# PreibischLab/SPIM_Registration

Hardware: AMD Instinct MI355X
Metric: Mvoxels/sec per RL iter, 6-view 512³ deconv; 1/2/4/8-GPU scaling (higher is better)
Workload: dtype f32; 1 GPU; 6-view 512^3 per GPU (global 512x512x512), 25^3 PSF, RL INDEPENDENT lambda=0.0; views=6, local_slabs=1, parallelism=z-slab x1 over 1 GPU(s) (device groups in one process, xGMI peer halo pulls), launch=devices, num_devices=1, slabs=1

## Files before the change

### include/spimdecon.h

```cpp
#ifndef SPIMDECON_H
#define SPIMDECON_H

#include <stdint.h>

#ifdef __cplusplus
extern "C" {
#endif

#define SPIMDECON_OK               0
#define SPIMDECON_ERR_ARG         -1
#define SPIMDECON_ERR_DEVICE      -2
#define SPIMDECON_ERR_HIP         -3
#define SPIMDECON_ERR_FFT         -4
#define SPIMDECON_ERR_COMM        -5
#define SPIMDECON_ERR_STATE       -6
#define SPIMDECON_ERR_OOM         -7
#define SPIMDECON_ERR_IO          -8

const char* spimdecon_last_error(void);
const char* spimdecon_version(void);


int convolution3DfftCUDAInPlace(float* im, const int* imDim,
                                const float* kernel, const int* kernelDim,
                                int devCUDA);

float* convolution3DfftCUDA(const float* im, const int* imDim,
                            const float* kernel, const int* kernelDim,
                            int devCUDA);
void spimdecon_free(void* p);

int     getNumDevicesCUDA(void);
void    getNameDeviceCUDA(int devCUDA, char* name);
int64_t getMemDeviceCUDA(int devCUDA);
int64_t getFreeMemDeviceCUDA(int devCUDA);
int     getCUDAcomputeCapabilityMajorVersion(int devCUDA);
int     getCUDAcomputeCapabilityMinorVersion(int devCUDA);

int32_t convolve_7  (float* image, const float* kernelX, const float* kernelY, const float* kernelZ,
                     int imageW, int imageH, int imageD, int32_t convolveX, int32_t convolveY,
                     int32_t convolveZ, int outofbounds, float outofboundsvalue, int devCUDA);
int32_t convolve_15 (float* image, const float* kernelX, const float* kernelY, const float* kernelZ,
                     int imageW, int imageH, int imageD, int32_t convolveX, int32_t convolveY,
                     int32_t convolveZ, int outofbounds, float outofboundsvalue, int devCUDA);
int32_t convolve_31 (float* image, const float* kernelX, const float* kernelY, const float* kernelZ,
                     int imageW, int imageH, int imageD, int32_t convolveX, int32_t convolveY,
                     int32_t convolveZ, int outofbounds, float outofboundsvalue, int devCUDA);
int32_t convolve_63 (float* image, const float* kernelX, const float* kernelY, const float* kernelZ,
                     int imageW, int imageH, int imageD, int32_t convolveX, int32_t convolveY,
                     int32_t convolveZ, int outofbounds, float outofboundsvalue, int devCUDA);
int32_t convolve_127(float* image, const float* kernelX, const float* kernelY, const float* kernelZ,
                     int imageW, int imageH, int imageD, int32_t convolveX, int32_t convolveY,
                     int32_t convolveZ, int outofbounds, float outofboundsvalue, int devCUDA);

int     convolutionCPU(float* image, const float* kernelX, const float* kernelY, const float* kernelZ,
                       int kernelRX, int kernelRY, int kernelRZ, int imageW, int imageH, int imageD,
                       int outofbounds, float outofboundsvalue);

#define MVD_PSF_OPTIMIZATION_II     0
#define MVD_PSF_OPTIMIZATION_I      1
#define MVD_PSF_EFFICIENT_BAYESIAN  2
#define MVD_PSF_INDEPENDENT         3

int mvd_prepare_kernels(int nviews, const float* const* k1_in, const int* kdims,
                        int psftype, int ij_threads,
                        float* const* k1_out, float* const* k2_out, int devCUDA);

int spimdecon_next_value(const float* last, const float* integral, const float* weight, int64_t n,
                         double lambda, float* out);

typedef struct mvd_session mvd_session;

typedef struct mvd_params {
    int64_t dims[3];
    int64_t nz_global;
    int64_t z_offset;
    int     device;
    int     local_slabs;
    int     nranks;
    int     rank;
    const char* comm_id;
    int     storage_fp16;
    int     fft_pad_policy;
    int     halo[3];
    int     ij_threads;
    int     fft_backend;
    int     slab_axis;
    int     reserved[6];
} mvd_params;

void mvd_params_default(mvd_params* p);

int mvd_comm_unique_id(char* out128);

int mvd_slab_range(int64_t nz, int nparts, int idx, int64_t* z0, int64_t* z1);

int mvd_halo_plan(int64_t nz, int64_t Mz, int cz, int64_t plane_elems, int64_t* out5);

int  mvd_create(const mvd_params* params, mvd_session** out);
int  mvd_create_devices(const int* devs, int ndev, const mvd_params* params, mvd_session** out);
void mvd_destroy(mvd_session* h);
int  mvd_num_devices(mvd_session* h, int* ndev);
int  mvd_slab_device(mvd_session* h, int slab, int* dev);
int  mvd_num_slabs(mvd_session* h, int* nslabs);
int  mvd_slab_extent(mvd_session* h, int slab, int64_t* out3);
int  mvd_exchange_stats(mvd_session* h, int64_t* bytes, int64_t* copies);

int mvd_add_view(mvd_session* h, const float* img, const float* weight,
                 const float* kernel1, const int* kdims);
int mvd_add_view_device(mvd_session* h, const float* d_img, const float* d_weight,
                        const float* kernel1, const int* kdims);

int mvd_init(mvd_session* h, int psftype);
int mvd_set_kernels(mvd_session* h, int view, const float* k1, const float* k2);
int mvd_get_kernels(mvd_session* h, int view, float* k1, float* k2);

int mvd_init_psi(mvd_session* h, const float* psi_or_null, double* avg_out);

int mvd_run(mvd_session* h, int iters, double lambda, double* stats);

int mvd_apply_mask(mvd_session* h);

int mvd_get_psi(mvd_session* h, float* out);
float* mvd_psi_device(mvd_session* h, int slab);

int mvd_fft_dims(mvd_session* h, int slab, int64_t* out3);
int mvd_kernel_planes(mvd_session* h, int slab, int* planes);
int mvd_zpass_mode(mvd_session* h, int slab, int* mode);
int mvd_xpass_mode(mvd_session* h, int slab, int* mode);
void* mvd_stream(mvd_session* h);
int mvd_enable_timing(mvd_session* h, int on);
int mvd_timing(mvd_session* h, double* out16);

typedef struct spim_dog_params {
    float   sigma;
    float   threshold;
    int     localization;
    double  image_sigma[3];
    int32_t find_min;
    int32_t find_max;
    double  min_intensity;
    double  max_intensity;
    int     ij_threads;
    int     device;
} spim_dog_params;

typedef struct spim_peak {
    int32_t x, y, z;
    float   intensity;
    int32_t is_min, is_max;
} spim_peak;

typedef struct spim_interest_point {
    double  pos[3];
    float   intensity;
    int32_t is_max;
} spim_interest_point;

void spim_dog_params_default(spim_dog_params* p);

int spim_dog_compute(const float* img, const int64_t* dims, const spim_dog_params* p,
                     float* dog_out, spim_peak* peaks, int64_t max_peaks, int64_t* npeaks);

int spim_dog_interest_points(const float* img, const int64_t* dims, const spim_dog_params* p,
                             float* dog_out, spim_interest_point* out, int64_t max_out,
                             int64_t* nout);

#define SPIM_DOG_EXTEND_MIRROR 0
#define SPIM_DOG_EXTEND_BORDER 1
int spim_dog_compute_ext(const float* img, const int64_t* dims, const spim_dog_params* p, int32_t extension,
                         float* dog_out, spim_peak* peaks, int64_t max_peaks, int64_t* npeaks);
int spim_dog_interest_points_ext(const float* img, const int64_t* dims, const spim_dog_params* p, int32_t extension,
                                 float* dog_out, spim_interest_point* out, int64_t max_out, int64_t* nout);

int spim_dog_release_workspace(int device);

int spim_save_interest_points(const char* base_dir, const char* file, const spim_interest_point* pts,
                              const int32_t* ids, int64_t n);
int spim_load_interest_points(const char* base_dir, const char* file, spim_interest_point* out,
                              int32_t* ids, int64_t max_out, int64_t* nout);
int spim_set_java_version(int jdk);
int spim_java_double_to_string(double d, char* out, int cap);

typedef struct spim_dom_params {
    int     radius1;
    int     radius2;
    float   threshold;
    int     localization;
    double  image_sigma[3];
    int32_t find_min;
    int32_t find_max;
    double  min_intensity;
    double  max_intensity;
    int     ij_threads;
    int     device;
} spim_dom_params;

void spim_dom_params_default(spim_dom_params* p);

int spim_dom_diameters(const spim_dom_params* p, int32_t s1[3], int32_t s2[3]);

int spim_dom_compute(const float* img, const int64_t* dims, const spim_dom_params* p,
                     float* dom_out, spim_peak* peaks, int64_t max_peaks, int64_t* npeaks);
int spim_dom_interest_points(const float* img, const int64_t* dims, const spim_dom_params* p,
                             float* dom_out, spim_interest_point* out, int64_t max_out,
                             int64_t* nout);

typedef struct spim_rgldm_params {
    int32_t num_neighbors;
    int32_t redundancy;
    float   ratio_of_distance;
    float   difference_threshold;
    int32_t b_split;
    int32_t device;
} spim_rgldm_params;

void spim_rgldm_params_default(spim_rgldm_params* p);

void spim_rgldm_tiles(int32_t* a_tile, int32_t* b_tile);

int spim_rgldm_descriptors(const double* pts, int64_t n, const spim_rgldm_params* p,
                           int32_t* neighbors, double* rel);

int spim_rgldm_match(const double* a, int64_t na, const double* b, int64_t nb,
                     const spim_rgldm_params* p, int32_t* best_idx, double* best, double* second,
                     int32_t* cand_a, int32_t* cand_b, int64_t cap, int64_t* count);

typedef struct spim_gh_params {
    double  ratio_of_distance;
    double  difference_threshold;
    int32_t b_split;
    int32_t device;
} spim_gh_params;

void spim_gh_params_default(spim_gh_params* p);

void spim_gh_tiles(int32_t* a_tile, int32_t* b_tile);

int spim_gh_descriptors(const double* pts, int64_t n, const spim_gh_params* p,
                        int32_t* neighbors, float* desc);

int spim_gh_match(const double* a, int64_t na, const double* b, int64_t nb,
                  const spim_gh_params* p, int32_t* best_idx, double* best, double* second,
                  int32_t* cand_a, int32_t* cand_b, int64_t cap, int64_t* count);

typedef struct spim_icp_params {
    float   max_distance;
    int32_t max_iterations;
    int32_t t_split;
    int32_t device;
} spim_icp_params;

void spim_icp_params_default(spim_icp_params* p);

void spim_icp_tiles(int32_t* ref_block, int32_t* target_tile);

int spim_icp_assign(const double* target, int64_t nt, const double* reference, int64_t nr,
                    const double* model, const spim_icp_params* p, int32_t* nearest, float* dist,
                    int32_t* match_t, int32_t* match_r, int64_t cap, int64_t* count,
                    int64_t* ambiguous);

#define SPIM_WEIGHTS_NONE         0
#define SPIM_WEIGHTS_PRECOMPUTED  1
#define SPIM_WEIGHTS_VIRTUAL      2

typedef struct spim_view_source {
    const float* img;
    int64_t      dims[3];
    double       model[12];
} spim_view_source;

typedef struct spim_input_params {
    int64_t bb_min[3];
    int64_t bb_dims[3];
    float   blending_border[3];
    float   blending_range[3];
    int     weight_type;
    int     osem_index;
    double  osem_speedup;
    int     ij_threads;
    int     device;
    int     src_on_device;
    int     out_on_device;
    int     reserved[8];
} spim_input_params;

void spim_input_params_default(spim_input_params* p);

int spim_prepare_inputs(int nviews, const spim_view_source* views, const spim_input_params* p,
                        float* const* img_out, float* const* weight_out, double* osem_used,
                        int* min_overlap, double* avg_overlap);

typedef struct spim_fusion_params {
    int64_t bb_min[3];
    int64_t bb_dims[3];
    float   downsampling;
    int     interpolation;
    int     use_blending;
    int     device;
    int     src_on_device;
    int     out_on_device;
    int     reserved[8];
} spim_fusion_params;

void spim_fusion_params_default(spim_fusion_params* p);

int spim_fuse_weighted_average(int nviews, const spim_view_source* views, const spim_fusion_params* p,
                               const float* blending_borders, const float* blending_ranges, float* out);

int spim_content_based_weights(const float* img, const int64_t dims[3], const double sigma1[3],
                               const double sigma2[3], float* out, int device);

int spim_fuse_weighted_average_content(int nviews, const spim_view_source* views,
                                       const spim_fusion_params* p, const float* blending_borders,
                                       const float* blending_ranges, const double* sigma1,
                                       const double* sigma2, float* out);


int spim_psf_transformed_size(const int64_t psf_size[3], const double model[12], int64_t out_size[3],
                              double offset[3]);

int spim_transform_psf(const float* psf, const int64_t psf_size[3], const double model[12], float* out,
                       int device);

int spim_extract_psf(const float* img, const int64_t dims[3], int img_on_device, const double* locations,
                     int64_t nlocations, const int64_t psf_size[3], const double model[12], float* psf_original,
                     float* psf_transformed, int device);

int spim_extract_psfs(int nviews, const float* const* imgs, const int64_t* dims, int img_on_device,
                      const double* const* locations, const int64_t* nlocations, const int64_t psf_size[3],
                      const double* models, float* const* psf_original, float* const* psf_transformed,
                      int device);

int spim_psf_release_workspace(int device);

int spim_average_transformed_psf(int npsfs, const float* const* psfs, const int64_t* psf_dims, float* avg,
                                 int64_t avg_dims[3], int device);

int spim_max_projection(const float* img, const int64_t dims[3], int min_dim, float* out, int64_t out_dims[2],
                        int* used_dim, int device);

typedef struct lrsim_session lrsim_session;

int  lrsim_create(const int64_t* dims, int device, int nranks, int rank, const char* comm_id,
                  lrsim_session** out);
int  lrsim_create_devices(const int64_t* dims, const int* devs, int ndev, lrsim_session** out);
void lrsim_destroy(lrsim_session* h);
int  lrsim_add_view(lrsim_session* h, const float* img, const float* weight, const float* kernel,
                    const int* kdims);
int  lrsim_owns_view(lrsim_session* h, int view, int* owned);
int  lrsim_view_device(lrsim_session* h, int view, int* device);
int  lrsim_init(lrsim_session* h, double* avg_out);
int  lrsim_run(lrsim_session* h, int iters, int multiplicative, double lambda, double* stats);
int  lrsim_get_psi(lrsim_session* h, float* out);
int  lrsim_fft_dims(lrsim_session* h, int64_t* out3);
int  lrsim_update_rule(const float* psi_in, const double* value, const double* num, int64_t n,
                       int multiplicative, double lambda, float* psi_out, double* stats2);

#ifdef __cplusplus
}
#endif
#endif
```

### spim_registration_amd/_lib.py

```python
from __future__ import annotations

import ctypes as C
import os
from pathlib import Path

import numpy as np

LIB_PATH = Path(os.environ.get("SPIMDECON_LIB") or Path(__file__).resolve().parent / "libspimdecon.so")

_i32, _i64, _f32, _f64 = C.c_int32, C.c_int64, C.c_float, C.c_double
_pf = C.POINTER(C.c_float)
_pi = C.POINTER(C.c_int)
_pi64 = C.POINTER(C.c_int64)
_pd = C.POINTER(C.c_double)


class MvdParams(C.Structure):
    _fields_ = [
        ("dims", C.c_int64 * 3),
        ("nz_global", C.c_int64),
        ("z_offset", C.c_int64),
        ("device", C.c_int),
        ("local_slabs", C.c_int),
        ("nranks", C.c_int),
        ("rank", C.c_int),
        ("comm_id", C.c_char_p),
        ("storage_fp16", C.c_int),
        ("fft_pad_policy", C.c_int),
        ("halo", C.c_int * 3),
        ("ij_threads", C.c_int),
        ("fft_backend", C.c_int),
        ("slab_axis", C.c_int),
        ("reserved", C.c_int * 6),
    ]


class DogParams(C.Structure):
    _fields_ = [
        ("sigma", C.c_float),
        ("threshold", C.c_float),
        ("localization", C.c_int),
        ("image_sigma", C.c_double * 3),
        ("find_min", C.c_int32),
        ("find_max", C.c_int32),
        ("min_intensity", C.c_double),
        ("max_intensity", C.c_double),
        ("ij_threads", C.c_int),
        ("device", C.c_int),
    ]


class DomParams(C.Structure):
    _fields_ = [
        ("radius1", C.c_int),
        ("radius2", C.c_int),
        ("threshold", C.c_float),
        ("localization", C.c_int),
        ("image_sigma", C.c_double * 3),
        ("find_min", C.c_int32),
        ("find_max", C.c_int32),
        ("min_intensity", C.c_double),
        ("max_intensity", C.c_double),
        ("ij_threads", C.c_int),
        ("device", C.c_int),
    ]


class RgldmParams(C.Structure):
    _fields_ = [
        ("num_neighbors", C.c_int32),
        ("redundancy", C.c_int32),
        ("ratio_of_distance", C.c_float),
        ("difference_threshold", C.c_float),
        ("b_split", C.c_int32),
        ("device", C.c_int32),
    ]


class GhParams(C.Structure):
    _fields_ = [
        ("ratio_of_distance", C.c_double),
        ("difference_threshold", C.c_double),
        ("b_split", C.c_int32),
        ("device", C.c_int32),
    ]


class IcpParams(C.Structure):
    _fields_ = [
        ("max_distance", C.c_float),
        ("max_iterations", C.c_int32),
        ("t_split", C.c_int32),
        ("device", C.c_int32),
    ]


class Peak(C.Structure):
    _fields_ = [("x", C.c_int32), ("y", C.c_int32), ("z", C.c_int32),
                ("intensity", C.c_float), ("is_min", C.c_int32), ("is_max", C.c_int32)]


class ViewSource(C.Structure):
    _fields_ = [("img", C.POINTER(C.c_float)), ("dims", C.c_int64 * 3), ("model", C.c_double * 12)]


class InputParams(C.Structure):
    _fields_ = [("bb_min", C.c_int64 * 3), ("bb_dims", C.c_int64 * 3),
                ("blending_border", C.c_float * 3), ("blending_range", C.c_float * 3),
                ("weight_type", C.c_int), ("osem_index", C.c_int), ("osem_speedup", C.c_double),
                ("ij_threads", C.c_int), ("device", C.c_int), ("src_on_device", C.c_int),
                ("out_on_device", C.c_int), ("reserved", C.c_int * 8)]


class FusionParams(C.Structure):
    _fields_ = [("bb_min", C.c_int64 * 3), ("bb_dims", C.c_int64 * 3), ("downsampling", C.c_float),
                ("interpolation", C.c_int), ("use_blending", C.c_int), ("device", C.c_int),
                ("src_on_device", C.c_int), ("out_on_device", C.c_int), ("reserved", C.c_int * 8)]


class InterestPointC(C.Structure):
    _fields_ = [("pos", C.c_double * 3), ("intensity", C.c_float), ("is_max", C.c_int32)]


SIGNATURES = {
    "spimdecon_last_error": (C.c_char_p, []),
    "spimdecon_version": (C.c_char_p, []),
    "convolution3DfftCUDAInPlace": (C.c_int, [_pf, _pi, _pf, _pi, C.c_int]),
    "convolution3DfftCUDA": (_pf, [_pf, _pi, _pf, _pi, C.c_int]),
    "spimdecon_free": (None, [C.c_void_p]),
    "getNumDevicesCUDA": (C.c_int, []),
    "getNameDeviceCUDA": (None, [C.c_int, C.c_char_p]),
    "getMemDeviceCUDA": (_i64, [C.c_int]),
    "getFreeMemDeviceCUDA": (_i64, [C.c_int]),
    "getCUDAcomputeCapabilityMajorVersion": (C.c_int, [C.c_int]),
    "getCUDAcomputeCapabilityMinorVersion": (C.c_int, [C.c_int]),
    "spimdecon_next_value": (C.c_int, [C.c_void_p, C.c_void_p, C.c_void_p, C.c_int64, C.c_double, C.c_void_p]),
    "mvd_prepare_kernels": (C.c_int, [C.c_int, C.POINTER(_pf), _pi, C.c_int, C.c_int,
                                      C.POINTER(_pf), C.POINTER(_pf), C.c_int]),
    "mvd_params_default": (None, [C.POINTER(MvdParams)]),
    "mvd_comm_unique_id": (C.c_int, [C.c_char_p]),
    "mvd_slab_range": (C.c_int, [_i64, C.c_int, C.c_int, _pi64, _pi64]),
    "mvd_halo_plan": (C.c_int, [_i64, _i64, C.c_int, _i64, _pi64]),
    "mvd_create": (C.c_int, [C.POINTER(MvdParams), C.POINTER(C.c_void_p)]),
    "mvd_create_devices": (C.c_int, [_pi, C.c_int, C.POINTER(MvdParams), C.POINTER(C.c_void_p)]),
    "mvd_destroy": (None, [C.c_void_p]),
    "mvd_num_devices": (C.c_int, [C.c_void_p, C.POINTER(C.c_int)]),
    "mvd_slab_device": (C.c_int, [C.c_void_p, C.c_int, C.POINTER(C.c_int)]),
    "mvd_num_slabs": (C.c_int, [C.c_void_p, C.POINTER(C.c_int)]),
    "mvd_slab_extent": (C.c_int, [C.c_void_p, C.c_int, _pi64]),
    "mvd_exchange_stats": (C.c_int, [C.c_void_p, _pi64, _pi64]),
    "mvd_add_view": (C.c_int, [C.c_void_p, _pf, _pf, _pf, _pi]),
    "mvd_add_view_device": (C.c_int, [C.c_void_p, C.c_void_p, C.c_void_p, _pf, _pi]),
    "mvd_init": (C.c_int, [C.c_void_p, C.c_int]),
    "mvd_set_kernels": (C.c_int, [C.c_void_p, C.c_int, _pf, _pf]),
    "mvd_get_kernels": (C.c_int, [C.c_void_p, C.c_int, _pf, _pf]),
    "mvd_init_psi": (C.c_int, [C.c_void_p, _pf, _pd]),
    "mvd_run": (C.c_int, [C.c_void_p, C.c_int, C.c_double, _pd]),
    "mvd_apply_mask": (C.c_int, [C.c_void_p]),
    "mvd_get_psi": (C.c_int, [C.c_void_p, _pf]),
    "mvd_psi_device": (C.c_void_p, [C.c_void_p, C.c_int]),
    "mvd_fft_dims": (C.c_int, [C.c_void_p, C.c_int, _pi64]),
    "mvd_kernel_planes": (C.c_int, [C.c_void_p, C.c_int, C.POINTER(C.c_int)]),
    "mvd_zpass_mode": (C.c_int, [C.c_void_p, C.c_int, C.POINTER(C.c_int)]),
    "mvd_xpass_mode": (C.c_int, [C.c_void_p, C.c_int, C.POINTER(C.c_int)]),
    "mvd_stream": (C.c_void_p, [C.c_void_p]),
    "mvd_enable_timing": (C.c_int, [C.c_void_p, C.c_int]),
    "mvd_timing": (C.c_int, [C.c_void_p, _pd]),
    "convolve_7": (_i32, [_pf, _pf, _pf, _pf, C.c_int, C.c_int, C.c_int, _i32, _i32, _i32,
                          C.c_int, C.c_float, C.c_int]),
    "spim_dog_params_default": (None, [C.POINTER(DogParams)]),
    "spim_dog_compute": (C.c_int, [_pf, _pi64, C.POINTER(DogParams), _pf, C.POINTER(Peak),
                                   _i64, _pi64]),
    "spim_dog_interest_points": (C.c_int, [_pf, _pi64, C.POINTER(DogParams), _pf,
                                           C.POINTER(InterestPointC), _i64, _pi64]),
    "spim_dog_compute_ext": (C.c_int, [_pf, _pi64, C.POINTER(DogParams), _i32, _pf, C.POINTER(Peak),
                                       _i64, _pi64]),
    "spim_dog_interest_points_ext": (C.c_int, [_pf, _pi64, C.POINTER(DogParams), _i32, _pf,
                                               C.POINTER(InterestPointC), _i64, _pi64]),
    "spim_dog_release_workspace": (C.c_int, [C.c_int]),
    "spim_dom_params_default": (None, [C.POINTER(DomParams)]),
    "spim_dom_diameters": (C.c_int, [C.POINTER(DomParams), C.POINTER(_i32), C.POINTER(_i32)]),
    "spim_dom_compute": (C.c_int, [_pf, _pi64, C.POINTER(DomParams), _pf, C.POINTER(Peak), _i64, _pi64]),
    "spim_dom_interest_points": (C.c_int, [_pf, _pi64, C.POINTER(DomParams), _pf,
                                           C.POINTER(InterestPointC), _i64, _pi64]),
    "spim_rgldm_params_default": (None, [C.POINTER(RgldmParams)]),
    "spim_rgldm_tiles": (None, [C.POINTER(_i32), C.POINTER(_i32)]),
    "spim_rgldm_descriptors": (C.c_int, [C.c_void_p, _i64, C.POINTER(RgldmParams), C.c_void_p, C.c_void_p]),
    "spim_rgldm_match": (C.c_int, [C.c_void_p, _i64, C.c_void_p, _i64, C.POINTER(RgldmParams), C.c_void_p,
                                   C.c_void_p, C.c_void_p, C.c_void_p, C.c_void_p, _i64, _pi64]),
    "spim_gh_params_default": (None, [C.POINTER(GhParams)]),
    "spim_gh_tiles": (None, [C.POINTER(_i32), C.POINTER(_i32)]),
    "spim_gh_descriptors": (C.c_int, [C.c_void_p, _i64, C.POINTER(GhParams), C.c_void_p, C.c_void_p]),
    "spim_gh_match": (C.c_int, [C.c_void_p, _i64, C.c_void_p, _i64, C.POINTER(GhParams), C.c_void_p,
                                C.c_void_p, C.c_void_p, C.c_void_p, C.c_void_p, _i64, _pi64]),
    "spim_icp_params_default": (None, [C.POINTER(IcpParams)]),
    "spim_icp_tiles": (None, [C.POINTER(_i32), C.POINTER(_i32)]),
    "spim_icp_assign": (C.c_int, [C.c_void_p, _i64, C.c_void_p, _i64, C.c_void_p, C.POINTER(IcpParams), C.c_void_p,
                                  C.c_void_p, C.c_void_p, C.c_void_p, _i64, _pi64, _pi64]),
    "spim_psf_release_workspace": (C.c_int, [C.c_int]),
    "spim_save_interest_points": (C.c_int, [C.c_char_p, C.c_char_p, C.POINTER(InterestPointC),
                                            C.POINTER(C.c_int32), C.c_int64]),
    "spim_load_interest_points": (C.c_int, [C.c_char_p, C.c_char_p, C.POINTER(InterestPointC),
                                            C.POINTER(C.c_int32), C.c_int64, _pi64]),
    "spim_java_double_to_string": (C.c_int, [C.c_double, C.c_char_p, C.c_int]),
    "spim_set_java_version": (C.c_int, [C.c_int]),
    "convolutionCPU": (C.c_int, [_pf, _pf, _pf, _pf, C.c_int, C.c_int, C.c_int, C.c_int, C.c_int, C.c_int,
                                 C.c_int, C.c_float]),
    "spim_input_params_default": (None, [C.POINTER(InputParams)]),
    "spim_fusion_params_default": (None, [C.POINTER(FusionParams)]),
    "spim_psf_transformed_size": (C.c_int, [_pi64, _pd, _pi64, _pd]),
    "spim_transform_psf": (C.c_int, [_pf, _pi64, _pd, _pf, C.c_int]),
    "spim_extract_psf": (C.c_int, [C.c_void_p, _pi64, C.c_int, _pd, C.c_int64, _pi64, _pd, _pf, _pf, C.c_int]),
    "spim_extract_psfs": (C.c_int, [C.c_int, C.POINTER(C.c_void_p), _pi64, C.c_int, C.POINTER(C.c_void_p), _pi64,
                                    _pi64, _pd, C.POINTER(C.c_void_p), C.POINTER(C.c_void_p), C.c_int]),
    "spim_average_transformed_psf": (C.c_int, [C.c_int, C.POINTER(_pf), _pi64, _pf, _pi64, C.c_int]),
    "spim_max_projection": (C.c_int, [_pf, _pi64, C.c_int, _pf, _pi64, C.POINTER(C.c_int), C.c_int]),
    "spim_fuse_weighted_average": (C.c_int, [C.c_int, C.POINTER(ViewSource), C.POINTER(FusionParams),
                                             _pf, _pf, _pf]),
    "spim_content_based_weights": (C.c_int, [C.c_void_p, _pi64, _pd, _pd, C.c_void_p, C.c_int]),
    "spim_fuse_weighted_average_content": (C.c_int, [C.c_int, C.POINTER(ViewSource), C.POINTER(FusionParams),
                                                     _pf, _pf, _pd, _pd, _pf]),
    "lrsim_create": (C.c_int, [_pi64, C.c_int, C.c_int, C.c_int, C.c_char_p, C.POINTER(C.c_void_p)]),
    "lrsim_create_devices": (C.c_int, [_pi64, _pi, C.c_int, C.POINTER(C.c_void_p)]),
    "lrsim_destroy": (None, [C.c_void_p]),
    "lrsim_view_device": (C.c_int, [C.c_void_p, C.c_int, C.POINTER(C.c_int)]),
    "lrsim_add_view": (C.c_int, [C.c_void_p, C.c_void_p, C.c_void_p, C.c_void_p, _pi]),
    "lrsim_owns_view": (C.c_int, [C.c_void_p, C.c_int, C.POINTER(C.c_int)]),
    "lrsim_init": (C.c_int, [C.c_void_p, _pd]),
    "lrsim_run": (C.c_int, [C.c_void_p, C.c_int, C.c_int, C.c_double, _pd]),
    "lrsim_get_psi": (C.c_int, [C.c_void_p, C.c_void_p]),
    "lrsim_fft_dims": (C.c_int, [C.c_void_p, _pi64]),
    "lrsim_update_rule": (C.c_int, [C.c_void_p, C.c_void_p, C.c_void_p, C.c_int64, C.c_int, C.c_double,
                                    C.c_void_p, _pd]),
    "spim_prepare_inputs": (C.c_int, [C.c_int, C.POINTER(ViewSource), C.POINTER(InputParams),
                                      C.POINTER(_pf), C.POINTER(_pf), C.POINTER(C.c_double),
                                      C.POINTER(C.c_int), C.POINTER(C.c_double)]),
}
for _n in (15, 31, 63, 127):
    SIGNATURES[f"convolve_{_n}"] = SIGNATURES["convolve_7"]

_lib = None


class SpimDeconError(RuntimeError):
    def __init__(self, status, msg):
        super().__init__(f"libspimdecon status {status}: {msg}")
        self.status = status


def load():
    global _lib
    if _lib is not None:
        return _lib
    if not LIB_PATH.exists():
        raise RuntimeError(
            f"{LIB_PATH} not found: build it with `python -m spim_registration_amd.build` "
            "(there is no CPU fallback)")
    if os.environ.get("SPIMDECON_HIP_RUNTIME", "") != "system":
        try:
            import torch
        except ImportError:
            pass
    lib = C.CDLL(str(LIB_PATH), mode=C.RTLD_GLOBAL)
    for name, (res, args) in SIGNATURES.items():
        f = getattr(lib, name)
        f.restype = res
        f.argtypes = args
    _lib = lib
    return lib


def last_error() -> str:
    return load().spimdecon_last_error().decode(errors="replace")


ERR_IO = -8


def check(status: int):
    if status != 0:
        raise SpimDeconError(status, last_error())


def fptr(a: np.ndarray):
    assert a.dtype == np.float32 and a.flags.c_contiguous, (a.dtype, a.flags)
    return a.ctypes.data_as(_pf)


def iptr(a: np.ndarray):
    assert a.dtype == np.int32 and a.flags.c_contiguous
    return a.ctypes.data_as(_pi)


def num_devices() -> int:
    return int(load().getNumDevicesCUDA())
```

### spim_registration_amd/csrc/capi.cpp

```cpp
#include <rccl/rccl.h>
#include <rocfft/rocfft-version.h>

#include <cstdlib>
#include <cstring>
#include <string>

#include "common.hpp"
#include "kernel_prep.hpp"
#include "session.hpp"

namespace spimdecon {

thread_local std::string g_last_error;
void set_last_error(const std::string& msg) { g_last_error = msg; }
void clear_last_error() { g_last_error.clear(); }

void fft_convolve_block(float* im, const int* imDim, const float* kernel, const int* kernelDim,
                        int dev, float* out);
void slab_range(int64_t nz, int nparts, int idx, int64_t* z0, int64_t* z1);

}

using namespace spimdecon;

struct mvd_session {
    Session* s;
};

extern "C" {

const char* spimdecon_last_error(void) { return g_last_error.c_str(); }

const char* spimdecon_version(void) {
    static std::string v = std::string("spimdecon 0.1.0 gfx950 rocfft ") +
                           std::to_string(rocfft_version_major) + "." +
                           std::to_string(rocfft_version_minor) + "." +
                           std::to_string(rocfft_version_patch);
    return v.c_str();
}

int convolution3DfftCUDAInPlace(float* im, const int* imDim, const float* kernel,
                                const int* kernelDim, int devCUDA) {
    return guarded([&] { fft_convolve_block(im, imDim, kernel, kernelDim, devCUDA, im); });
}

float* convolution3DfftCUDA(const float* im, const int* imDim, const float* kernel,
                            const int* kernelDim, int devCUDA) {
    float* out = nullptr;
    int st = guarded([&] {
        SD_CHECK(imDim, SPIMDECON_ERR_ARG, "null imDim");
        const size_t n = size_t(imDim[0]) * imDim[1] * imDim[2];
        out = static_cast<float*>(std::malloc(n * sizeof(float)));
        SD_CHECK(out, SPIMDECON_ERR_OOM, "host out of memory");
        fft_convolve_block(const_cast<float*>(im), imDim, kernel, kernelDim, devCUDA, out);
    });
    if (st != SPIMDECON_OK) {
        std::free(out);
        return nullptr;
    }
    return out;
}

void spimdecon_free(void* p) { std::free(p); }

int getNumDevicesCUDA(void) {
    int n = 0;
    if (hipGetDeviceCount(&n) != hipSuccess) {
        return 0;
    }
    return n;
}

void getNameDeviceCUDA(int devCUDA, char* name) {
    if (!name) return;
    name[0] = 0;
    guarded([&] {
        check_device(devCUDA);
        hipDeviceProp_t prop;
        SD_HIP(hipGetDeviceProperties(&prop, devCUDA));
        std::string s = std::string(prop.name) + " (" + prop.gcnArchName + ")";
        std::strncpy(name, s.c_str(), 255);
        name[255] = 0;
    });
}

int64_t getMemDeviceCUDA(int devCUDA) {
    int64_t r = -1;
    guarded([&] {
        check_device(devCUDA);
        hipDeviceProp_t prop;
        SD_HIP(hipGetDeviceProperties(&prop, devCUDA));
        r = int64_t(prop.totalGlobalMem);
    });
    return r;
}

int64_t getFreeMemDeviceCUDA(int devCUDA) {
    int64_t r = -1;
    guarded([&] {
        check_device(devCUDA);
        DeviceGuard g(devCUDA);
        size_t fr = 0, tot = 0;
        SD_HIP(hipMemGetInfo(&fr, &tot));
        r = int64_t(fr);
    });
    return r;
}

int getCUDAcomputeCapabilityMajorVersion(int devCUDA) {
    int r = -1;
    guarded([&] {
        check_device(devCUDA);
        hipDeviceProp_t prop;
        SD_HIP(hipGetDeviceProperties(&prop, devCUDA));
        r = prop.major;
    });
    return r;
}

int getCUDAcomputeCapabilityMinorVersion(int devCUDA) {
    int r = -1;
    guarded([&] {
        check_device(devCUDA);
        hipDeviceProp_t prop;
        SD_HIP(hipGetDeviceProperties(&prop, devCUDA));
        r = prop.minor;
    });
    return r;
}

int spimdecon_next_value(const float* last, const float* integral, const float* weight, int64_t n, double lambda,
                         float* out) {
    return guarded([&] {
        SD_CHECK(n >= 0, SPIMDECON_ERR_ARG, "n must be >= 0");
        SD_CHECK(n == 0 || (last && integral && weight && out), SPIMDECON_ERR_ARG, "null pointer");
        launch_next_value(last, integral, weight, n, lambda, out, nullptr);
        SD_HIP(hipStreamSynchronize(nullptr));
    });
}

int mvd_prepare_kernels(int nviews, const float* const* k1_in, const int* kdims, int psftype,
                        int ij_threads, float* const* k1_out, float* const* k2_out, int devCUDA) {
    return guarded([&] {
        SD_CHECK(nviews >= 1 && k1_in && kdims && k1_out && k2_out, SPIMDECON_ERR_ARG, "bad arguments");
        std::vector<HostKernel> k1(nviews), k2;
        for (int v = 0; v < nviews; ++v) {
            for (int d = 0; d < 3; ++d) k1[v].dims[d] = kdims[3 * v + d];
            const int64_t n = int64_t(k1[v].dims[0]) * k1[v].dims[1] * k1[v].dims[2];
            SD_CHECK(n > 0 && k1_in[v], SPIMDECON_ERR_ARG, "bad kernel");
            k1[v].data.assign(k1_in[v], k1_in[v] + n);
        }
        prepare_kernels_gpu(k1, k2, psftype, ij_threads, devCUDA);
        for (int v = 0; v < nviews; ++v) {
            std::copy(k1[v].data.begin(), k1[v].data.end(), k1_out[v]);
            std::copy(k2[v].data.begin(), k2[v].data.end(), k2_out[v]);
        }
    });
}

void mvd_params_default(mvd_params* p) {
    if (!p) return;
    std::memset(p, 0, sizeof(*p));
    p->local_slabs = 1;
    p->nranks = 1;
    p->ij_threads = 8;
}

int mvd_comm_unique_id(char* out128) {
    return guarded([&] {
        SD_CHECK(out128, SPIMDECON_ERR_ARG, "null output");
        static_assert(sizeof(ncclUniqueId) == 128, "unexpected ncclUniqueId size");
        ncclUniqueId id;
        ncclResult_t r = ncclGetUniqueId(&id);
        SD_CHECK(r == ncclSuccess, SPIMDECON_ERR_COMM,
                 std::string("ncclGetUniqueId failed: ") + ncclGetErrorString(r));
        std::memcpy(out128, &id, 128);
    });
}

int mvd_slab_range(int64_t nz, int nparts, int idx, int64_t* z0, int64_t* z1) {
    return guarded([&] {
        SD_CHECK(nz >= 1 && nparts >= 1 && idx >= 0 && idx < nparts && z0 && z1, SPIMDECON_ERR_ARG,
                 "bad slab_range arguments");
        slab_range(nz, nparts, idx, z0, z1);
    });
}

int mvd_halo_plan(int64_t nz, int64_t Mz, int cz, int64_t plane_elems, int64_t* out5) {
    return guarded([&] {
        SD_CHECK(out5, SPIMDECON_ERR_ARG, "null argument");
        const HaloPlan h = halo_plan(nz, Mz, cz, plane_elems);
        out5[0] = h.send_lo;
        out5[1] = h.recv_lo;
        out5[2] = h.send_hi;
        out5[3] = h.recv_hi;
        out5[4] = h.count;
    });
}

int mvd_create(const mvd_params* params, mvd_session** out) {
    return guarded([&] {
        SD_CHECK(params && out, SPIMDECON_ERR_ARG, "null argument");
        *out = nullptr;
        auto* h = new mvd_session{nullptr};
        try {
            h->s = new Session(*params);
        } catch (...) {
            delete h;
            throw;
        }
        *out = h;
    });
}

int mvd_create_devices(const int* devs, int ndev, const mvd_params* params, mvd_session** out) {
    return guarded([&] {
        SD_CHECK(devs && ndev >= 1 && params && out, SPIMDECON_ERR_ARG, "null argument");
        *out = nullptr;
        std::vector<int> dl(devs, devs + ndev);
        auto* h = new mvd_session{nullptr};
        try {
            h->s = new Session(*params, dl);
        } catch (...) {
            delete h;
            throw;
        }
        *out = h;
    });
}

void mvd_destroy(mvd_session* h) {
    if (!h) return;
    guarded([&] { delete h->s; });
    delete h;
}

#define SESSION(h) \
    SD_CHECK((h) && (h)->s, SPIMDECON_ERR_ARG, "null session"); \
    Session& S = *(h)->s

int mvd_add_view(mvd_session* h, const float* img, const float* weight, const float* kernel1,
                 const int* kdims) {
    return guarded([&] { SESSION(h); S.add_view(img, weight, kernel1, kdims, false); });
}

int mvd_add_view_device(mvd_session* h, const float* d_img, const float* d_weight,
                        const float* kernel1, const int* kdims) {
    return guarded([&] { SESSION(h); S.add_view(d_img, d_weight, kernel1, kdims, true); });
}

int mvd_init(mvd_session* h, int psftype) {
    return guarded([&] { SESSION(h); S.init(psftype); });
}

int mvd_set_kernels(mvd_session* h, int view, const float* k1, const float* k2) {
    return guarded([&] { SESSION(h); S.set_kernels(view, k1, k2); });
}

int mvd_get_kernels(mvd_session* h, int view, float* k1, float* k2) {
    return guarded([&] { SESSION(h); S.get_kernels(view, k1, k2); });
}

int mvd_init_psi(mvd_session* h, const float* psi_or_null, double* avg_out) {
    return guarded([&] {
        SESSION(h);
        const double a = S.init_psi(psi_or_null);
        if (avg_out) *avg_out = a;
    });
}

int mvd_run(mvd_session* h, int iters, double lambda, double* stats) {
    return guarded([&] { SESSION(h); S.run(iters, lambda, stats); });
}

int mvd_apply_mask(mvd_session* h) {
    return guarded([&] { SESSION(h); S.apply_mask(); });
}

int mvd_get_psi(mvd_session* h, float* out) {
    return guarded([&] { SESSION(h); S.get_psi(out); });
}

float* mvd_psi_device(mvd_session* h, int slab) {
    float* r = nullptr;
    guarded([&] { SESSION(h); r = S.psi_device(slab); });
    return r;
}

int mvd_fft_dims(mvd_session* h, int slab, int64_t* out3) {
    return guarded([&] { SESSION(h); SD_CHECK(out3, SPIMDECON_ERR_ARG, "null"); S.fft_dims(slab, out3); });
}

int mvd_kernel_planes(mvd_session* h, int slab, int* planes) {
    return guarded([&] { SESSION(h); SD_CHECK(planes, SPIMDECON_ERR_ARG, "null"); *planes = S.kernel_planes(slab); });
}

int mvd_zpass_mode(mvd_session* h, int slab, int* mode) {
    return guarded([&] { SESSION(h); SD_CHECK(mode, SPIMDECON_ERR_ARG, "null"); *mode = S.zpass_mode(slab); });
}

int mvd_xpass_mode(mvd_session* h, int slab, int* mode) {
    return guarded([&] { SESSION(h); SD_CHECK(mode, SPIMDECON_ERR_ARG, "null"); *mode = S.xpass_mode(slab); });
}

void* mvd_stream(mvd_session* h) {
    void* r = nullptr;
    guarded([&] { SESSION(h); r = S.stream(); });
    return r;
}

int mvd_num_devices(mvd_session* h, int* ndev) {
    return guarded([&] { SESSION(h); SD_CHECK(ndev, SPIMDECON_ERR_ARG, "null"); *ndev = S.ndevices(); });
}

int mvd_slab_device(mvd_session* h, int slab, int* dev) {
    return guarded([&] { SESSION(h); SD_CHECK(dev, SPIMDECON_ERR_ARG, "null"); *dev = S.slab_device(slab); });
}

int mvd_num_slabs(mvd_session* h, int* nslabs) {
    return guarded([&] { SESSION(h); SD_CHECK(nslabs, SPIMDECON_ERR_ARG, "null"); *nslabs = S.nslabs(); });
}

int mvd_exchange_stats(mvd_session* h, int64_t* bytes, int64_t* copies) {
    return guarded([&] { SESSION(h); S.exchange_stats(bytes, copies); });
}

int mvd_slab_extent(mvd_session* h, int slab, int64_t* out3) {
    return guarded([&] { SESSION(h); SD_CHECK(out3, SPIMDECON_ERR_ARG, "null"); S.slab_extent(slab, out3); });
}

int mvd_enable_timing(mvd_session* h, int on) {
    return guarded([&] { SESSION(h); S.enable_timing(on != 0); });
}

int mvd_timing(mvd_session* h, double* out16) {
    return guarded([&] { SESSION(h); SD_CHECK(out16, SPIMDECON_ERR_ARG, "null"); S.timing(out16); });
}

}
```

### spim_registration_amd/csrc/fftconv.hip

```cpp
#include "fftconv.hpp"

#include <climits>
#include "rl_math.hpp"

#include <cmath>
#include <cstdlib>
#include <type_traits>
#include <cstdio>
#include <cstring>

namespace spimdecon {

namespace {


typedef float sd_v2 __attribute__((ext_vector_type(2)));
__device__ __forceinline__ sd_v2 v2_(float2 a) { return sd_v2{a.x, a.y}; }
__device__ __forceinline__ float2 f2_(sd_v2 a) { return make_float2(a.x, a.y); }
__device__ __forceinline__ float2 cmul(float2 a, float2 b) {
    const sd_v2 A = v2_(a), B = v2_(b);
    const sd_v2 t = A.xx * B;
    return f2_(__builtin_elementwise_fma(A.yy, sd_v2{-B.y, B.x}, t));
}
__device__ __forceinline__ float2 cadd(float2 a, float2 b) {
#pragma clang fp contract(fast)
    return f2_(v2_(a) + v2_(b));
}
__device__ __forceinline__ float2 csub(float2 a, float2 b) {
#pragma clang fp contract(fast)
    return f2_(v2_(a) - v2_(b));
}
__device__ __forceinline__ float2 cscale(float2 a, float s) {
#pragma clang fp contract(fast)
    return f2_(v2_(a) * sd_v2{s, s});
}
template <bool INV>
__device__ __forceinline__ float2 mul_mi(float2 a) {
    return INV ? make_float2(-a.y, a.x) : make_float2(a.y, -a.x);
}
template <bool INV>
__device__ __forceinline__ float2 cadd_mi(float2 a, float2 d) {
    const sd_v2 D = v2_(d);
    return f2_(__builtin_elementwise_fma(D.yx, INV ? sd_v2{-1.0f, 1.0f} : sd_v2{1.0f, -1.0f}, v2_(a)));
}
template <bool INV>
__device__ __forceinline__ float2 csub_mi(float2 a, float2 d) {
    const sd_v2 D = v2_(d);
    return f2_(__builtin_elementwise_fma(D.yx, INV ? sd_v2{1.0f, -1.0f} : sd_v2{-1.0f, 1.0f}, v2_(a)));
}

template <int S>
__device__ __forceinline__ float ldv(const void* p, int64_t i) {
    if constexpr (S == 0) return static_cast<const float*>(p)[i];
    else return __half2float(static_cast<const __half*>(p)[i]);
}


template <int R, bool INV>
__device__ __forceinline__ void dft(float2* a) {
    if constexpr (R == 2) {
        const float2 t = a[0];
        a[0] = cadd(t, a[1]);
        a[1] = csub(t, a[1]);
    } else if constexpr (R == 3) {
        const float2 s = cadd(a[1], a[2]);
        const float2 m = csub(a[0], cscale(s, 0.5f));
        const float2 d = cscale(csub(a[1], a[2]), 0.86602540378443864676f);
        a[0] = cadd(a[0], s);
        a[1] = cadd_mi<INV>(m, d);
        a[2] = csub_mi<INV>(m, d);
    } else if constexpr (R == 4) {
        const float2 s0 = cadd(a[0], a[2]), d0 = csub(a[0], a[2]);
        const float2 s1 = cadd(a[1], a[3]), d1 = csub(a[1], a[3]);
        a[0] = cadd(s0, s1);
        a[2] = csub(s0, s1);
        a[1] = cadd_mi<INV>(d0, d1);
        a[3] = csub_mi<INV>(d0, d1);
    } else if constexpr (R == 5) {
        constexpr float c1 = 0.30901699437494742410f, c2 = -0.80901699437494742410f;
        constexpr float s1 = 0.95105651629515357212f, s2 = 0.58778525229247312917f;
        const float2 b1 = cadd(a[1], a[4]), b2 = cadd(a[2], a[3]);
        const float2 d1 = csub(a[1], a[4]), d2 = csub(a[2], a[3]);
        const float2 m1 = cadd(a[0], cadd(cscale(b1, c1), cscale(b2, c2)));
        const float2 m2 = cadd(a[0], cadd(cscale(b1, c2), cscale(b2, c1)));
        const float2 n1 = cadd(cscale(d1, s1), cscale(d2, s2));
        const float2 n2 = csub(cscale(d1, s2), cscale(d2, s1));
        a[0] = cadd(a[0], cadd(b1, b2));
        a[1] = cadd_mi<INV>(m1, n1);
        a[4] = csub_mi<INV>(m1, n1);
        a[2] = cadd_mi<INV>(m2, n2);
        a[3] = csub_mi<INV>(m2, n2);
    } else {
        static_assert(R == 7, "radix 2, 3, 4, 5, 7 only");
        constexpr float c1 = 0.62348980185873353053f, c2 = -0.22252093395631440429f,
                        c3 = -0.90096886790241912624f;
        constexpr float s1 = 0.78183148246802980871f, s2 = 0.97492791218182360702f,
                        s3 = 0.43388373911755812048f;
        const float2 b1 = cadd(a[1], a[6]), b2 = cadd(a[2], a[5]), b3 = cadd(a[3], a[4]);
        const float2 d1 = csub(a[1], a[6]), d2 = csub(a[2], a[5]), d3 = csub(a[3], a[4]);
        const float2 r1 = cadd(a[0], cadd(cscale(b1, c1), cadd(cscale(b2, c2), cscale(b3, c3))));
        const float2 r2 = cadd(a[0], cadd(cscale(b1, c2), cadd(cscale(b2, c3), cscale(b3, c1))));
        const float2 r3 = cadd(a[0], cadd(cscale(b1, c3), cadd(cscale(b2, c1), cscale(b3, c2))));
        const float2 i1 = cadd(cscale(d1, s1), cadd(cscale(d2, s2), cscale(d3, s3)));
        const float2 i2 = csub(cscale(d1, s2), cadd(cscale(d2, s3), cscale(d3, s1)));
        const float2 i3 = cadd(csub(cscale(d1, s3), cscale(d2, s1)), cscale(d3, s2));
        a[0] = cadd(a[0], cadd(b1, cadd(b2, b3)));
        a[1] = cadd_mi<INV>(r1, i1);
        a[6] = csub_mi<INV>(r1, i1);
        a[2] = cadd_mi<INV>(r2, i2);
        a[5] = csub_mi<INV>(r2, i2);
        a[3] = cadd_mi<INV>(r3, i3);
        a[4] = csub_mi<INV>(r3, i3);
    }
}

template <int R, bool INV>
__device__ __forceinline__ void stage_pp(const float2* __restrict__ src, float2* __restrict__ dst,
                                         const float2* __restrict__ tw, int L, int Ns, int c, int g,
                                         int TPC, int ES, int CS) {
    const int nb = L / R;
    const int step = L / (Ns * R);
    for (int j = g; j < nb; j += TPC) {
        const int k = j % Ns;
        float2 v[R];
#pragma unroll
        for (int t = 0; t < R; ++t) v[t] = src[(j + t * nb) * ES + c * CS];
        if (Ns > 1) {
#pragma unroll
            for (int t = 1; t < R; ++t) {
                float2 w = tw[t * k * step];
                if (INV) w.y = -w.y;
                v[t] = cmul(v[t], w);
            }
        }
        dft<R, INV>(v);
        const int base = (j - k) * R + k;
#pragma unroll
        for (int t = 0; t < R; ++t) dst[(base + t * Ns) * ES + c * CS] = v[t];
    }
}

__device__ __forceinline__ void wave_sync() {
    __builtin_amdgcn_fence(__ATOMIC_RELEASE, "wavefront");
    __builtin_amdgcn_wave_barrier();
    __builtin_amdgcn_fence(__ATOMIC_ACQUIRE, "wavefront");
}

template <bool INV, bool WAVE = false>
__device__ __forceinline__ float2* fft_pp(float2* a, float2* b, const float2* tw, const Fft1D& f, int c, int g,
                          int TPC, int ES, int CS, bool active) {
    int Ns = 1;
    float2* src = a;
    float2* dst = b;
    for (int s = 0; s < f.ns; ++s) {
        const int R = f.radix(s);
        if (active) {
            switch (R) {
                case 2: stage_pp<2, INV>(src, dst, tw, f.L, Ns, c, g, TPC, ES, CS); break;
                case 3: stage_pp<3, INV>(src, dst, tw, f.L, Ns, c, g, TPC, ES, CS); break;
                case 4: stage_pp<4, INV>(src, dst, tw, f.L, Ns, c, g, TPC, ES, CS); break;
                case 5: stage_pp<5, INV>(src, dst, tw, f.L, Ns, c, g, TPC, ES, CS); break;
                default: stage_pp<7, INV>(src, dst, tw, f.L, Ns, c, g, TPC, ES, CS); break;
            }
        }
        if constexpr (WAVE) wave_sync();
        else __syncthreads();
        Ns *= R;
        float2* t = src;
        src = dst;
        dst = t;
    }
    return src;
}


enum XMode { XM_PSI = 0, XM_QUOT = 1, XM_UPDATE = 2, XM_KERNEL = 3 };

struct XArgs {
    SlabGeom g;
    int64_t Hx, Hp;
    Fft1D fx;
    const int* row_mirror;
    const int* row_one;
    const float2* Cin;
    float2* Cout;
    const float* psi_in;
    float* psi_out;
    const void* img;
    const void* w;
    double lambda;
    double* partials;
    const float* kern;
    int kx, ky, kz;
    float kscale;
    uint32_t spec_bytes;
    uint32_t nvox;
    int pb0, pn0, pb1, pn1;
};

__device__ __forceinline__ int x_pair(const XArgs& a, int i) {
    return i < a.pn0 ? a.pb0 + i : (i - a.pn0 < a.pn1 ? a.pb1 + (i - a.pn0) : -1);
}

constexpr int kXThreads = 256;
constexpr int kXPairs = kXThreads / 64;

__host__ __device__ inline int x_wave_elems(int Mx) { return 2 * (Mx + 2); }

template <int MODE, int S>
__global__ __launch_bounds__(kXThreads) void k_xpass(XArgs a) {
    extern __shared__ __attribute__((aligned(16))) float2 smem[];
    const SlabGeom& g = a.g;
    const int Mx = int(g.Mx);
    const int Hx = int(a.Hx);
    const int Hp = int(a.Hp);
    const int nx = int(g.nx);
    const int cx = g.cx;
    float2* tw = smem;
    const int wv = threadIdx.x >> 6;
    const int lane = threadIdx.x & 63;
    float2* A = smem + Mx + wv * x_wave_elems(Mx);
    float2* B = A + Mx + 2;
    for (int i = threadIdx.x; i < Mx; i += kXThreads) tw[i] = a.fx.tw[i];
    const int nrows = int(g.My * g.Mz);
    const int nlin = a.pn0 + a.pn1;
    double ssum = 0.0;
    float smax = -1.0f;
    __syncthreads();
    for (int pg = blockIdx.x; pg * kXPairs < nlin; pg += gridDim.x) {
        const int pair = x_pair(a, pg * kXPairs + wv);
        const bool active = pair >= 0;
        const int r0 = 2 * pair, r1 = 2 * pair + 1;
        const bool valid0 = active && r0 < nrows, valid1 = active && r1 < nrows;
        const int sm0 = valid0 ? a.row_mirror[r0] : -1, sm1 = valid1 ? a.row_mirror[r1] : -1;
        const int so0 = valid0 ? a.row_one[r0] : -1, so1 = valid1 ? a.row_one[r1] : -1;
        float2* Z = A;
        if constexpr (MODE == XM_QUOT || MODE == XM_UPDATE) {
            int p0 = -1, p1 = -1;
            if constexpr (MODE == XM_QUOT) {
                p0 = so0 >= 0 ? r0 : -1;
                p1 = so1 >= 0 ? r1 : -1;
            } else {
                p0 = sm0 >= 0 ? (sm0 / int(g.ny)) * int(g.My) + sm0 % int(g.ny) : -1;
                p1 = sm1 >= 0 ? (sm1 / int(g.ny)) * int(g.My) + sm1 % int(g.ny) : -1;
            }
            const float2* row0 = a.Cin + int64_t(p0) * Hp;
            const float2* row1 = a.Cin + int64_t(p1) * Hp;
            for (int k = lane; k < Hx; k += 64) {
                B[k] = p0 >= 0 ? row0[k] : make_float2(0.f, 0.f);
                B[Hx + k] = p1 >= 0 ? row1[k] : make_float2(0.f, 0.f);
            }
            __syncthreads();
            for (int k = lane; k < Mx; k += 64) {
                float2 xa, xb;
                if (k <= Mx / 2) {
                    xa = B[k];
                    xb = B[Hx + k];
                    if (k == 0 || k == Mx / 2) {
                        xa.y = 0.f;
                        xb.y = 0.f;
                    }
                } else {
                    xa = B[Mx - k];
                    xb = B[Hx + Mx - k];
                    xa.y = -xa.y;
                    xb.y = -xb.y;
                }
                A[k] = make_float2(xa.x - xb.y, xa.y + xb.x);
            }
            __syncthreads();
            Z = fft_pp<true>(A, B, tw, a.fx, 0, lane, 64, 1, 0, active);
        }
        float2* O = (Z == A) ? B : A;
        if constexpr (MODE == XM_PSI) {
            const float* p0 = a.psi_in + int64_t(sm0 < 0 ? 0 : sm0) * nx;
            const float* p1 = a.psi_in + int64_t(sm1 < 0 ? 0 : sm1) * nx;
            for (int qx = lane; qx < Mx; qx += 64) {
                const int sx = qx < nx + cx ? qx : qx - Mx;
                const int lx = int(mirror_idx(sx, nx));
                Z[qx] = make_float2(sm0 >= 0 ? p0[lx] : 0.f, sm1 >= 0 ? p1[lx] : 0.f);
            }
        } else if constexpr (MODE == XM_KERNEL) {
            for (int qx = lane; qx < Mx; qx += 64) {
                float v[2] = {0.f, 0.f};
#pragma unroll
                for (int h = 0; h < 2; ++h) {
                    const int r = h == 0 ? r0 : r1;
                    if (!(h == 0 ? valid0 : valid1)) continue;
                    const int qz = r / int(g.My), qy = r % int(g.My);
                    const int jz = (qz + a.kz / 2) % int(g.Mz), jy = (qy + a.ky / 2) % int(g.My);
                    const int jx = (qx + a.kx / 2) % Mx;
                    if (jz < a.kz && jy < a.ky && jx < a.kx)
                        v[h] = a.kern[(int64_t(jz) * a.ky + jy) * a.kx + jx] * a.kscale;
                }
                Z[qx] = make_float2(v[0], v[1]);
            }
        } else if constexpr (MODE == XM_QUOT) {
            const bool live0 = valid0 && sm0 != -1, live1 = valid1 && sm1 != -1;
            for (int qx = lane; qx < Mx; qx += 64) {
                const float2 bz = Z[qx];
                float q0 = live0 ? 1.0f : 0.0f, q1 = live1 ? 1.0f : 0.0f;
                if (qx < nx) {
                    if (so0 >= 0) {
                        const float iv = ldv<S>(a.img, int64_t(so0) * nx + qx);
                        if (iv > 0.0f) q0 = __fdiv_rn(iv, bz.x);
                    }
                    if (so1 >= 0) {
                        const float iv = ldv<S>(a.img, int64_t(so1) * nx + qx);
                        if (iv > 0.0f) q1 = __fdiv_rn(iv, bz.y);
                    }
                }
                Z[qx] = make_float2(q0, q1);
            }
        } else {
            for (int qx = lane; qx < nx; qx += 64) {
                const float2 iz = Z[qx];
                float o0 = 0.f, o1 = 0.f;
                if (sm0 >= 0) {
                    const int64_t vi = int64_t(sm0) * nx + qx;
                    const float last = a.psi_in[vi];
                    o0 = next_value(last, iz.x, ldv<S>(a.w, vi), a.lambda);
                    if (so0 >= 0) {
                        a.psi_out[vi] = o0;
                        const float ch = fabsf(__fsub_rn(o0, last));
                        ssum += (double)ch;
                        smax = fmaxf(smax, ch);
                    }
                }
                if (sm1 >= 0) {
                    const int64_t vi = int64_t(sm1) * nx + qx;
                    const float last = a.psi_in[vi];
                    o1 = next_value(last, iz.y, ldv<S>(a.w, vi), a.lambda);
                    if (so1 >= 0) {
                        a.psi_out[vi] = o1;
                        const float ch = fabsf(__fsub_rn(o1, last));
                        ssum += (double)ch;
                        smax = fmaxf(smax, ch);
                    }
                }
                Z[qx] = make_float2(o0, o1);
            }
            __syncthreads();
            for (int qx = nx + lane; qx < Mx; qx += 64) {
                const int sx = qx < nx + cx ? qx : qx - Mx;
                Z[qx] = Z[mirror_idx(sx, nx)];
            }
        }
        __syncthreads();
        if (MODE == XM_UPDATE && a.Cout == nullptr) continue;
        float2* F = fft_pp<false>(Z, O, tw, a.fx, 0, lane, 64, 1, 0, active);
        const bool w0 = valid0 && sm0 != -1, w1 = valid1 && sm1 != -1;
        float2* out0 = a.Cout + int64_t(r0) * Hp;
        float2* out1 = a.Cout + int64_t(r1) * Hp;
        for (int k = lane; k < Hp; k += 64) {
            float2 xa = make_float2(0.f, 0.f), xb = make_float2(0.f, 0.f);
            if (k < Hx) {
                const float2 zk = F[k];
                const float2 zm = F[k == 0 ? 0 : Mx - k];
                xa = make_float2(0.5f * (zk.x + zm.x), 0.5f * (zk.y - zm.y));
                xb = make_float2(0.5f * (zk.y + zm.y), -0.5f * (zk.x - zm.x));
            }
            if (w0) out0[k] = xa;
            if (w1) out1[k] = xb;
        }
        __syncthreads();
    }
    if constexpr (MODE == XM_UPDATE) {
        __shared__ double sh_sum[kXThreads / 64];
        __shared__ float sh_max[kXThreads / 64];
        for (int off = 32; off > 0; off >>= 1) {
            ssum += __shfl_xor(ssum, off, 64);
            smax = fmaxf(smax, __shfl_xor(smax, off, 64));
        }
        if (lane == 0) {
            sh_sum[wv] = ssum;
            sh_max[wv] = smax;
        }
        __syncthreads();
        if (threadIdx.x == 0) {
            for (int i = 1; i < kXThreads / 64; ++i) {
                ssum += sh_sum[i];
                smax = fmaxf(smax, sh_max[i]);
            }
            a.partials[2 * blockIdx.x] = ssum;
            a.partials[2 * blockIdx.x + 1] = (double)smax;
        }
    }
}


constexpr int kCThreads = 1024;

#include "fftconv_col.inc"
#include "fft_reg.inc"
#include "fftconv_2f.inc"
#include "fftconv_x.inc"
#include "fftconv_xt.inc"
#include "fftconv_zd.inc"


Fft1D make_fft(int L, bool allow_2f, DBuf<float2>& tw, hipStream_t s) {
    Fft1D f;
    f.L = L;
    int m = L;
    auto push = [&](int r) {
        SD_CHECK(f.ns < kFftMaxStages, SPIMDECON_ERR_ARG, "too many FFT stages");
        f.radix_packed |= uint64_t(r) << (4 * f.ns);
        f.ns++;
        m /= r;
    };
    while (m % 4 == 0) push(4);
    while (m % 2 == 0) push(2);
    while (m % 3 == 0) push(3);
    while (m % 5 == 0) push(5);
    while (m % 7 == 0) push(7);
    SD_CHECK(m == 1, SPIMDECON_ERR_ARG, "FFT length " + std::to_string(L) + " is not 2,3,5,7-smooth");
#define SD_2F_LOOKUP(A, B) \
    if (L == (A) * (B)) { f.n1 = (A); f.n2 = (B); }
    if (allow_2f) { SD_2F_SIZES(SD_2F_LOOKUP) }
#undef SD_2F_LOOKUP
    std::vector<float2> h(L);
    for (int i = 0; i < L; ++i) {
        const double ang = -2.0 * M_PI * double(i) / double(L);
        h[i] = make_float2(float(std::cos(ang)), float(std::sin(ang)));
    }
    tw.alloc(L);
    SD_HIP(hipMemcpyAsync(tw.p, h.data(), L * sizeof(float2), hipMemcpyHostToDevice, s));
    SD_HIP(hipStreamSynchronize(s));
    f.tw = tw.p;
    return f;
}

size_t x_lds(const SpectralPlan& p) {
    return size_t(p.g.Mx + kXPairs * x_wave_elems(int(p.g.Mx))) * sizeof(float2);
}

unsigned x_grid(const XArgs& a) {
    const int64_t b = ceil_div(int64_t(a.pn0) + a.pn1, kXPairs);
    return unsigned(std::max<int64_t>(1, std::min<int64_t>(b, 256 * 8)));
}

XArgs base_args(const SpectralPlan& p) {
    XArgs a{};
    SD_CHECK(p.g.My * p.g.Mz < (int64_t(1) << 30), SPIMDECON_ERR_ARG, "too many rows");
    a.pb0 = 0;
    a.pn0 = int((p.g.My * p.g.Mz + 1) / 2);
    a.pb1 = 0;
    a.pn1 = 0;
    a.g = p.g;
    a.Hx = p.Hx;
    a.Hp = p.Hp;
    a.fx = p.fx;
    a.row_mirror = p.row_mirror.p;
    a.row_one = p.row_one.p;
    return a;
}

#define SD_X2F_SIZES(M) M(16, 16) M(16, 24) M(16, 32) M(20, 27) M(24, 24) M(20, 32) M(25, 32) M(30, 35) M(42, 50)

bool aligned_to(const void* q, size_t n) { return q == nullptr || reinterpret_cast<uintptr_t>(q) % n == 0; }

bool x_buffer_args(const XArgs& a, Store st, const SpectralPlan& p, XArgs& b) {
    const size_t va = st == Store::F32 ? 16 : 8;
    const uint64_t spec_bytes = uint64_t(p.spectrum_elems()) * sizeof(float2);
    const uint64_t nvox = uint64_t(p.g.nx) * p.g.ny * p.g.nz;
    if (p.g.nx % 4 != 0 || !aligned_to(a.img, va) || !aligned_to(a.w, va) || !aligned_to(a.psi_in, 16) ||
        !aligned_to(a.psi_out, 16) || spec_bytes >= kOOB || nvox * 4 >= kOOB)
        return false;
    b = a;
    b.spec_bytes = uint32_t(spec_bytes);
    b.nvox = uint32_t(nvox);
    return true;
}

template <int MODE>
unsigned launch_xtile(const XArgs& a, Store st, const SpectralPlan& p, hipStream_t s) {
    XArgs b;
    if (!p.fx.n1 || !x_buffer_args(a, st, p, b)) return 0;
    const int L = int(p.g.Mx);
    const int NP = xt_np(MODE, L);
    const size_t lds = xt_lds(L, NP, xt_twg(L, NP));
    if (lds > 160 * 1024) return 0;
    const unsigned grid = unsigned(std::max<int64_t>(1, ceil_div(int64_t(a.pn0) + a.pn1, int64_t(NP))));
    const int sv = st == Store::F32 ? 0 : 1;
    bool done = false;
    const bool tik = MODE == XM_UPDATE && a.lambda > 0.0;
#define SD_XT(SV, A, B, TK)                                                                                \
    if (!done && sv == SV && L == (A) * (B) && tik == TK) {                                               \
        constexpr int TRv = SD_2F_TR(A, B);                                                               \
        constexpr int NPv = xt_np(MODE, (A) * (B));                                                       \
        auto kfn = &k_xtile<MODE, SV, A, B, TK, NPv, TRv>;                                                \
        SD_HIP(hipFuncSetAttribute(reinterpret_cast<const void*>(kfn), hipFuncAttributeMaxDynamicSharedMemorySize, \
                                   int(lds)));                                                            \
        hipLaunchKernelGGL(kfn, dim3(grid), dim3(NPv * TRv), lds, s, b);                                  \
        done = true;                                                                                      \
    }
#define SD_XT_S(A, B) \
    SD_XT(0, A, B, false) SD_XT(1, A, B, false) if constexpr (MODE == XM_UPDATE) { SD_XT(0, A, B, true) SD_XT(1, A, B, true) }
    SD_X2F_SIZES(SD_XT_S)
#undef SD_XT_S
#undef SD_XT
    if (!done) return 0;
    SD_HIP(hipGetLastError());
#if SD_XT_STAMPS
    {
        unsigned long long h[3][8];
        SD_HIP(hipStreamSynchronize(s));
        SD_HIP(hipMemcpyFromSymbol(h, HIP_SYMBOL(g_xt_stamp), sizeof(h)));
        const unsigned long long n = std::max(1ull, h[MODE][7]);
        std::fprintf(stderr, "[xt_stamp] L=%d mode=%d fp16=%d tiles=%llu cycles/tile: load %llu inv %llu rl %llu fwd %llu store %llu prologue %llu\n",
                     L, MODE, sv, h[MODE][7], h[MODE][0] / n, h[MODE][1] / n, h[MODE][2] / n, h[MODE][3] / n,
                     h[MODE][4] / n, h[MODE][5] / n);
        std::memset(h, 0, sizeof(h));
        SD_HIP(hipMemcpyToSymbol(HIP_SYMBOL(g_xt_stamp), h, sizeof(h)));
    }
#endif
    return grid;
}

template <int MODE>
unsigned launch_xrows(const XArgs& a, Store st, const SpectralPlan& p, hipStream_t s) {
    const int nx = int(p.g.nx);
    const int U = int(ceil_div(p.Hp / 2, 64));
    const int UV = int(ceil_div(nx / 4, 64));
    XArgs b;
    if (U > 4 || (UV != U && UV != U - 1) || !x_buffer_args(a, st, p, b)) return 0;
    const int Mx = int(p.g.Mx);
    const size_t lds = size_t(Mx + kXPairs * xrows_wave_elems(Mx, false)) * sizeof(float2);
    SD_CHECK(lds <= 160 * 1024, SPIMDECON_ERR_ARG, "x pass LDS too large");
    SD_CHECK(p.g.My * p.g.Mz < (int64_t(1) << 30), SPIMDECON_ERR_ARG, "too many rows");
    const unsigned grid = x_grid(a);
    const int sv = st == Store::F32 ? 0 : 1;
    bool done = false;
#define SD_XR(SV, UU, VV)                                                                               \
    if (!done && sv == SV && U == UU && UV == VV) {                                                     \
        SD_HIP(hipFuncSetAttribute(reinterpret_cast<const void*>(&k_xrows<MODE, SV, UU, VV, 0, 0>),    \
                                   hipFuncAttributeMaxDynamicSharedMemorySize, int(lds)));              \
        hipLaunchKernelGGL((k_xrows<MODE, SV, UU, VV, 0, 0>), dim3(grid), dim3(kXThreads), lds, s, b); \
        done = true;                                                                                    \
    }
#define SD_XR_S(SV) SD_XR(SV, 1, 1) SD_XR(SV, 2, 1) SD_XR(SV, 2, 2) SD_XR(SV, 3, 2) \
                    SD_XR(SV, 3, 3) SD_XR(SV, 4, 3) SD_XR(SV, 4, 4)
    SD_XR_S(0) SD_XR_S(1)
#undef SD_XR_S
#undef SD_XR
    SD_CHECK(done, SPIMDECON_ERR_ARG, "no x-row kernel for this configuration");
    SD_HIP(hipGetLastError());
    return grid;
}

template <int MODE>
unsigned launch_x(const XArgs& a, Store st, const SpectralPlan& p, hipStream_t s) {
    if constexpr (MODE == XM_QUOT || MODE == XM_UPDATE || MODE == XM_PSI) {
        if (const unsigned gt = launch_xtile<MODE>(a, st, p, s)) {
            if (MODE == XM_UPDATE) p.xmode_update = 2;
            return gt;
        }
    }
    if constexpr (MODE == XM_QUOT || MODE == XM_UPDATE) {
        if (const unsigned gr = launch_xrows<MODE>(a, st, p, s)) {
            if (MODE == XM_UPDATE) p.xmode_update = 1;
            return gr;
        }
    }
    if (MODE == XM_UPDATE) p.xmode_update = 0;
    const size_t lds = x_lds(p);
    SD_CHECK(lds <= 160 * 1024, SPIMDECON_ERR_ARG, "x pass LDS too large");
    SD_CHECK(p.g.My * p.g.Mz < (int64_t(1) << 30), SPIMDECON_ERR_ARG, "too many rows");
    const unsigned grid = x_grid(a);
    if (st == Store::F32) {
        SD_HIP(hipFuncSetAttribute(reinterpret_cast<const void*>(&k_xpass<MODE, 0>),
                                   hipFuncAttributeMaxDynamicSharedMemorySize, int(lds)));
        hipLaunchKernelGGL((k_xpass<MODE, 0>), dim3(grid), dim3(kXThreads), lds, s, a);
    } else {
        SD_HIP(hipFuncSetAttribute(reinterpret_cast<const void*>(&k_xpass<MODE, 1>),
                                   hipFuncAttributeMaxDynamicSharedMemorySize, int(lds)));
        hipLaunchKernelGGL((k_xpass<MODE, 1>), dim3(grid), dim3(kXThreads), lds, s, a);
    }
    SD_HIP(hipGetLastError());
    return grid;
}

int col_tx(int L) {
    for (int tx : {16, 8, 4})
        if (size_t(2 * L * tx + L) * sizeof(float2) <= 160 * 1024) return tx;
    fail(SPIMDECON_ERR_ARG, "column FFT length " + std::to_string(L) + " exceeds the LDS tile");
}

constexpr int kColGridRounds = 16;

template <int AXIS, int MODE>
bool launch_col2f(const SpectralPlan& p, const Fft1D& f, float2* C, const float2* K, hipStream_t s,
                  int tx0 = 0, int ntxb = -1, int kc = 0, int nout = -1, int zsplit = INT_MAX, int zskip = 0) {
    if (nout < 0) nout = int(p.g.Mz);
    const int L = f.L;
    const int tr = (f.n1 > 32 || f.n2 > 32) ? 64 : 32;
    const size_t budget = size_t(160) * 1024;
    auto tile_lds = [&](int tx) { return size_t(L * tx + L + (MODE == 5 ? f.n2 * tx : 0)) * sizeof(float2); };
    const int TX = tile_lds(k2fTX) <= budget ? k2fTX : 8;
    const int kplanes = MODE == 5 ? 2 * kc + 1 : 0;
    const size_t lds = tile_lds(TX);
    const uint64_t bytes = uint64_t(p.spectrum_elems()) * sizeof(float2);
    const uint64_t kbytes = MODE == 5 ? uint64_t(kplanes) * p.Hp * p.g.My * sizeof(float2)
                                      : (MODE >= 2 ? bytes : 0);
    if (MODE >= 2 && tr == 64) return false;
    if (lds > budget || (AXIS == 2 && bytes >= (uint64_t(1) << 31))) return false;
    if (MODE == 5 && (AXIS != 2 || kplanes > f.n2)) return false;
    const uint32_t rbytes = AXIS == 1 ? uint32_t(uint64_t(p.g.My * p.Hp) * sizeof(float2)) : uint32_t(bytes);
    if (ntxb < 0) ntxb = int(p.Hp / TX);
    SD_CHECK(tx0 >= 0 && ntxb > 0 && tx0 + ntxb <= p.Hp / TX, SPIMDECON_ERR_ARG, "bad column band");
    const int64_t ntiles = int64_t(ntxb) * (AXIS == 1 ? nout : p.g.My);
    const int64_t per_cu = std::max<int64_t>(1, (160 * 1024) / int64_t(lds));
    const unsigned grid = unsigned(std::min<int64_t>(ntiles, 256 * per_cu * kColGridRounds));
    const int n1 = f.n1, n2 = f.n2;
    const bool pf = p.knobs.ypf && AXIS == 1 && MODE < 2 && tr == 32 && TX == 16 && lds > size_t(80 * 1024);
    bool done = false;
#define SD_2F_L(A, B, T, PFV)                                                                                   \
            constexpr int TRv = SD_2F_TR(A, B);                                                                 \
            SD_HIP(hipFuncSetAttribute(reinterpret_cast<const void*>(&k_col2f<AXIS, A, B, MODE, T, TRv, PFV>), \
                                       hipFuncAttributeMaxDynamicSharedMemorySize, int(lds)));                  \
            hipLaunchKernelGGL((k_col2f<AXIS, A, B, MODE, T, TRv, PFV>), dim3(grid), dim3(T * TRv), lds, s,     \
                               p.g, p.Hp, f.tw, C, K, rbytes, tx0, ntxb, kc, uint32_t(kbytes), nout, zsplit,  \
                               zskip);                                                                       \
            done = true;
#define SD_2F_C1(A, B, T)                                                                                  \
    if constexpr (MODE < 2 || SD_2F_TR(A, B) == 32) {                                                      \
        if (!done && n1 == (A) && n2 == (B) && TX == (T)) {                                                \
            if constexpr (AXIS == 1 && MODE < 2 && (T) == 16 && SD_2F_TR(A, B) == 32 && (A) * (B) >= 512) { \
                if (pf) { SD_2F_L(A, B, T, true) }                                                         \
            }                                                                                              \
            if (!done) { SD_2F_L(A, B, T, false) }                                                         \
        }                                                                                                  \
    }
#define SD_2F_C(A, B) \
    SD_2F_C1(A, B, 16) if constexpr ((A) * (B) > 600) { SD_2F_C1(A, B, 8) }
    SD_2F_SIZES(SD_2F_C)
#undef SD_2F_C
#undef SD_2F_C1
#undef SD_2F_L
    SD_CHECK(done, SPIMDECON_ERR_ARG, "no two-factor column kernel for this length");
    SD_HIP(hipGetLastError());
    return true;
}

template <int AXIS, bool INV, int ZMODE>
void launch_col(const SpectralPlan& p, const Fft1D& f, float2* C, const float2* K, hipStream_t s,
                int nout = -1) {
    if constexpr (ZMODE == 1) {
        if (f.n1 && launch_col2f<AXIS, 4>(p, f, C, K, s, 0, -1, 0, nout)) return;
    }
    if (f.n1 && launch_col2f<AXIS, ZMODE == 1 ? 2 : (INV ? 1 : 0)>(p, f, C, K, s, 0, -1, 0, nout)) return;
    const int tx = col_tx(f.L);
    SD_CHECK(f.L * tx / 2 <= kColMaxU * kCThreads, SPIMDECON_ERR_ARG, "column tile exceeds prefetch registers");
    const size_t lds = size_t(2 * f.L * tx + f.L) * sizeof(float2);
    const int64_t ntiles = (p.Hp / tx) * (AXIS == 1 ? p.g.Mz : p.g.My);
    const unsigned grid = unsigned(std::min<int64_t>(ntiles, 256 * (tx == 16 ? 1 : 2)));
#define CL(TXV)                                                                                    \
    case TXV:                                                                                      \
        SD_HIP(hipFuncSetAttribute(reinterpret_cast<const void*>(&k_colpass<AXIS, TXV, INV, ZMODE>), \
                                   hipFuncAttributeMaxDynamicSharedMemorySize, int(lds)));         \
        hipLaunchKernelGGL((k_colpass<AXIS, TXV, INV, ZMODE>), dim3(grid), dim3(kCThreads), lds, s, \
                           p.g, p.Hp, f, C, K);                                                    \
        break;
    switch (tx) {
        CL(16) CL(8) CL(4)
        default: fail(SPIMDECON_ERR_ARG, "bad TX");
    }
#undef CL
    SD_HIP(hipGetLastError());
}

}

int64_t engine_fast_size(int64_t need, bool even, int policy) {
    need = std::max<int64_t>(need, 1);
    int64_t smooth = 0;
    for (int64_t m = need;; ++m) {
        if (even && (m & 1)) continue;
        int64_t r = m;
        for (int64_t q : {2, 3, 5, 7})
            while (r % q == 0) r /= q;
        if (r == 1) {
            smooth = m;
            break;
        }
    }
    int64_t fast = 0;
#define SD_2F_PICK(A, B) \
    if ((A) * (B) >= need && (fast == 0 || (A) * (B) < fast)) fast = (A) * (B);
    SD_2F_SIZES(SD_2F_PICK)
#undef SD_2F_PICK
    if (policy == 2 || fast == 0) {
        SD_CHECK(policy != 1, SPIMDECON_ERR_ARG, "length " + std::to_string(need) + " beyond the fast-path table");
        return smooth;
    }
    if (policy == 1) return fast;
    return fast * 4 <= smooth * 5 ? fast : smooth;
}

bool engine_slab_fits(int64_t nx, int64_t ny, int64_t nzs, const int halo[3], int policy) {
    const int64_t Mx = engine_fast_size(nx + 2 * halo[0], true, policy);
    const int64_t My = engine_fast_size(ny + 2 * halo[1], false, policy);
    const int64_t Mz = engine_fast_size(nzs + 2 * halo[2], false, policy);
    const int64_t Hp = ceil_div(Mx / 2 + 1, int64_t(16)) * 16;
    return uint64_t(nx) * uint64_t(ny) * uint64_t(nzs) * 4u < kOOB &&
           uint64_t(Hp) * uint64_t(My) * uint64_t(Mz) * sizeof(float2) < kOOB;
}

static bool zdirect_env() {
    const char* e = std::getenv("SPIMDECON_ZDIRECT");
    return !(e && e[0] == '0');
}

EngineKnobs EngineKnobs::from_env() {
    auto off = [](const char* name) {
        const char* e = std::getenv(name);
        return e && e[0] == '0';
    };
    EngineKnobs k;
    k.ypf = !off("SPIMDECON_YPF");
    k.zkd = !off("SPIMDECON_ZKD");
    k.zdirect = zdirect_env();
    return k;
}

void SpectralPlan::create(const SlabGeom& geom, bool allow_2f, bool z_fft, const EngineKnobs& kn) {
    g = geom;
    knobs = kn;
    SD_CHECK(g.Mx % 2 == 0, SPIMDECON_ERR_ARG, "Mx must be even");
    Hx = g.Mx / 2 + 1;
    Hp = ceil_div(Hx, 16) * 16;
    hipStream_t s = nullptr;
    fx = make_fft(int(g.Mx), allow_2f, twx, s);
    fy = make_fft(int(g.My), allow_2f, twy, s);
    if (z_fft) {
        fz = make_fft(int(g.Mz), allow_2f, twz, s);
    } else {
        fz = Fft1D{};
        fz.L = int(g.Mz);
    }
    const int64_t nrows = g.My * g.Mz;
    std::vector<int> rm(nrows), ro(nrows);
    auto mir = [](int64_t sidx, int64_t n) -> int64_t {
        if (n == 1) return 0;
        const int64_t p = 2 * (n - 1);
        int64_t j = sidx % p;
        if (j < 0) j += p;
        return j >= n ? p - j : j;
    };
    for (int64_t qz = 0; qz < g.Mz; ++qz) {
        const int64_t sz = qz < g.nz + g.cz ? qz : qz - g.Mz;
        const int64_t gz = g.z0 + sz;
        const bool gin = gz >= 0 && gz < g.nzg;
        const bool skip = gin && (sz < 0 || sz >= g.nz);
        const int64_t lz = mir(gz, g.nzg) - g.z0;
        for (int64_t qy = 0; qy < g.My; ++qy) {
            const int64_t r = qz * g.My + qy;
            if (skip) {
                rm[r] = ro[r] = -1;
                continue;
            }
            SD_CHECK(lz >= 0 && lz < g.nz, SPIMDECON_ERR_ARG, "slab too thin for its mirror halo");
            const int64_t sy = qy < g.ny + g.cy ? qy : qy - g.My;
            const int64_t ly = mir(sy, g.ny);
            rm[r] = int(lz * g.ny + ly);
            const bool interior = (sz >= 0 && sz < g.nz) && (sy >= 0 && sy < g.ny);
            ro[r] = interior ? int(sz * g.ny + sy) : -2;
        }
    }
    row_mirror.alloc(nrows);
    row_one.alloc(nrows);
    SD_HIP(hipMemcpy(row_mirror.p, rm.data(), nrows * sizeof(int), hipMemcpyHostToDevice));
    SD_HIP(hipMemcpy(row_one.p, ro.data(), nrows * sizeof(int), hipMemcpyHostToDevice));
}

void engine_forward_psi(const SpectralPlan& p, const float* psi, float2* C, hipStream_t s) {
    XArgs a = base_args(p);
    a.psi_in = psi;
    a.Cout = C;
    launch_x<XM_PSI>(a, Store::F32, p, s);
}

void engine_kernel_spectrum(const SpectralPlan& p, const float* d_kernel, int kx, int ky, int kz,
                            float scale, float2* Kspec, hipStream_t s) {
    XArgs a = base_args(p);
    a.Cout = Kspec;
    a.kern = d_kernel;
    a.kx = kx;
    a.ky = ky;
    a.kz = kz;
    a.kscale = scale;
    DBuf<int> all(size_t(p.g.My * p.g.Mz));
    SD_HIP(hipMemsetAsync(all.p, 0, all.bytes(), s));
    a.row_mirror = all.p;
    a.row_one = all.p;
    launch_x<XM_KERNEL>(a, Store::F32, p, s);
    launch_col<1, false, 0>(p, p.fy, Kspec, nullptr, s);
    launch_col<2, false, 0>(p, p.fz, Kspec, nullptr, s);
    SD_HIP(hipStreamSynchronize(s));
}

bool engine_kernel_compact_ok(const SpectralPlan& p) {
    const int kc = p.g.cz;
    return p.fz.n1 && p.fz.n1 <= 32 && p.fz.n2 <= 32 && 2 * kc + 1 <= p.fz.n2 &&
           size_t(p.fz.L * 8 + p.fz.L + p.fz.n2 * 8) * sizeof(float2) <= 80 * 1024 &&
           uint64_t(p.spectrum_elems()) * sizeof(float2) < (uint64_t(1) << 31);
}

int64_t engine_kernel_compact_elems(const SpectralPlan& p) { return int64_t(2 * p.g.cz + 1) * p.g.My * p.Hp; }

void engine_kernel_compact(const SpectralPlan& p, const float* d_kernel, int kx, int ky, int kz, float scale,
                           float2* work, float2* Kc, hipStream_t s) {
    SD_CHECK(engine_kernel_compact_ok(p) || engine_zdirect_ok(p), SPIMDECON_ERR_ARG,
             "compact kernel path not available");
    SD_CHECK(kz / 2 <= p.g.cz, SPIMDECON_ERR_ARG, "kernel z half size exceeds the halo");
    const int kc = p.g.cz;
    const int mzc = 2 * kc + 1;
    XArgs a = base_args(p);
    a.g.Mz = mzc;
    a.pn0 = int((p.g.My * mzc + 1) / 2);
    a.Cout = work;
    a.kern = d_kernel;
    a.kx = kx;
    a.ky = ky;
    a.kz = kz;
    a.kscale = scale;
    DBuf<int> all(size_t(p.g.My * mzc));
    SD_HIP(hipMemsetAsync(all.p, 0, all.bytes(), s));
    a.row_mirror = all.p;
    a.row_one = all.p;
    launch_x<XM_KERNEL>(a, Store::F32, p, s);
    launch_col<1, false, 0>(p, p.fy, work, nullptr, s, mzc);
    const size_t plane = size_t(p.g.My * p.Hp) * sizeof(float2);
    SD_HIP(hipMemcpyAsync(Kc + size_t(kc) * p.g.My * p.Hp, work, size_t(kc + 1) * plane,
                          hipMemcpyDeviceToDevice, s));
    if (kc > 0)
        SD_HIP(hipMemcpyAsync(Kc, work + size_t(mzc - kc) * p.g.My * p.Hp, size_t(kc) * plane,
                              hipMemcpyDeviceToDevice, s));
    SD_HIP(hipStreamSynchronize(s));
}

static int zdirect_kc_bound(int kc) {
    for (int b : {4, 8, 12, 16})
        if (kc <= b) return b;
    return 0;
}

struct ZChunk { int opt = 0, H = 0; };
static ZChunk zdmc_plan(int64_t nz, int KC) {
    ZChunk best;
    if (KC == 0 || nz < 1) return best;
    int64_t bw = -1;
    for (int opt : {KC == 16 ? 15 : 16, 12, 8}) {
        const int64_t cap = int64_t(kZdThreads / 32) * opt;
        const int64_t nch = ceil_div(nz, cap);
        const int64_t waste = nch * cap - nz;
        if (bw < 0 || waste < bw) {
            best = {opt, int(ceil_div(nz, nch))};
            bw = waste;
        }
    }
    return best;
}

bool engine_zdirect_dims_ok(int64_t Mx, int64_t My, int64_t Mz, int cz, bool zdirect_knob) {
    const int KC = zdirect_kc_bound(cz);
    const int64_t Hp = ceil_div(Mx / 2 + 1, int64_t(16)) * 16;
    return zdirect_knob && KC > 0 && Mz >= 2 * cz + 1 && Mz >= KC &&
           uint64_t(Hp) * uint64_t(My) * uint64_t(Mz) * sizeof(float2) <= kOOB;
}

bool engine_zdirect_ok(const SpectralPlan& p) {
    return p.Hp % 16 == 0 && engine_zdirect_dims_ok(p.g.Mx, p.g.My, p.g.Mz, p.g.cz, p.knobs.zdirect);
}

int engine_zpass_mode(const SpectralPlan& p, bool compact) {
    if (!compact) return 0;
    return engine_zdirect_ok(p) ? 3 : 1;
}

void engine_zpass_compact(const SpectralPlan& p, float2* C, const float2* Kc, hipStream_t s) {
    if (!engine_zdirect_ok(p)) {
        const bool ok = launch_col2f<2, 5>(p, p.fz, C, Kc, s, 0, -1, p.g.cz, int(p.g.nz));
        SD_CHECK(ok, SPIMDECON_ERR_ARG, "compact-kernel z pass not available");
        return;
    }
    const int64_t nflat = p.g.My * p.Hp;
    const int KC = zdirect_kc_bound(p.g.cz);
    const ZChunk zc = zdmc_plan(p.g.nz, KC);
    const int64_t ntiles = ceil_div(nflat, int64_t(32));
    const uint32_t bytes = uint32_t(uint64_t(nflat) * p.g.Mz * sizeof(float2));
    const float kscale = float(p.g.Mz);
    const int kd = p.knobs.zkd && (KC == 12 || KC == 16) && KC - p.g.cz == 1 ? 1 : 0;
    bool done = false;
#define SD_ZC(KCV, OPTV, KDV)                                                                                 \
    if (!done && KC == (KCV) && zc.opt == (OPTV) && kd == (KDV)) {                                            \
        constexpr size_t lds = size_t(zdc_lds(KCV, OPTV, 32));                                                \
        SD_HIP(hipFuncSetAttribute(reinterpret_cast<const void*>(&k_zdmc<KCV, OPTV, KDV>),                    \
                                   hipFuncAttributeMaxDynamicSharedMemorySize, int(lds)));                    \
                     \
        static const int per_cu = [] {                                                                        \
            int n = 1;                                                                                        \
            SD_HIP(hipOccupancyMaxActiveBlocksPerMultiprocessor(                                              \
                &n, reinterpret_cast<const void*>(&k_zdmc<KCV, OPTV, KDV>), kZdThreads, lds));                \
            return std::max(1, n);                                                                            \
        }();                                                                                                  \
        const unsigned grid = unsigned(std::min<int64_t>(ntiles, 256 * per_cu));                              \
        hipLaunchKernelGGL((k_zdmc<KCV, OPTV, KDV>), dim3(grid), dim3(kZdThreads), lds, s, p.g, nflat, C, Kc,  \
                           p.g.cz, zc.H, bytes, kscale);                                                      \
        done = true;                                                                                          \
    }
#define SD_ZC3(KCV) SD_ZC(KCV, 16, 0) SD_ZC(KCV, 12, 0) SD_ZC(KCV, 8, 0)
    SD_ZC3(4) SD_ZC3(8) SD_ZC3(12)
    SD_ZC(12, 16, 1) SD_ZC(12, 12, 1) SD_ZC(12, 8, 1)
    SD_ZC(16, 15, 0) SD_ZC(16, 12, 0) SD_ZC(16, 8, 0) SD_ZC(16, 15, 1) SD_ZC(16, 12, 1) SD_ZC(16, 8, 1)
#undef SD_ZC3
#undef SD_ZC
    SD_CHECK(done, SPIMDECON_ERR_ARG, "no z-chunked LDS-DMA z kernel for this kernel size");
    SD_HIP(hipGetLastError());
}

void engine_ypass(const SpectralPlan& p, float2* C, bool inv, hipStream_t s) {
    if (inv) launch_col<1, true, 0>(p, p.fy, C, nullptr, s, int(p.g.nz));
    else launch_col<1, false, 0>(p, p.fy, C, nullptr, s);
}

bool engine_ypass_planes2(const SpectralPlan& p, float2* C, int z0, int z1, int z2, int z3, hipStream_t s) {
    if (!p.fy.n1 || z0 < 0 || z1 < z0 || z2 < z1 || z3 < z2 || z3 > int(p.g.Mz)) return false;
    if (z3 - z2 + z1 - z0 <= 0) return true;
    return launch_col2f<1, 0>(p, p.fy, C + size_t(z0) * size_t(p.g.My) * size_t(p.Hp), nullptr, s, 0, -1, 0,
                              (z1 - z0) + (z3 - z2), z1 - z0, z2 - z1);
}

bool engine_ypass_planes(const SpectralPlan& p, float2* C, int z0, int z1, hipStream_t s) {
    if (!p.fy.n1 || z0 < 0 || z1 > int(p.g.Mz)) return false;
    if (z1 <= z0) return true;
    return launch_col2f<1, 0>(p, p.fy, C + size_t(z0) * size_t(p.g.My) * size_t(p.Hp), nullptr, s, 0, -1, 0,
                              z1 - z0);
}

void engine_zpass(const SpectralPlan& p, float2* C, const float2* K, hipStream_t s) {
    if (K) launch_col<2, false, 1>(p, p.fz, C, K, s, int(p.g.nz));
    else launch_col<2, false, 0>(p, p.fz, C, nullptr, s);
}

PairRanges all_pairs(const SpectralPlan& p) {
    PairRanges r;
    r.n0 = int((p.g.My * p.g.Mz + 1) / 2);
    return r;
}

void engine_quotient(const SpectralPlan& p, Store st, const float2* Cin, const void* img,
                     float2* Cout, const PairRanges& pr, hipStream_t s) {
    XArgs a = base_args(p);
    a.pb0 = pr.b0;
    a.pn0 = pr.n0;
    a.pb1 = pr.b1;
    a.pn1 = pr.n1;
    a.Cin = Cin;
    a.Cout = Cout;
    a.img = img;
    launch_x<XM_QUOT>(a, st, p, s);
}

int64_t engine_update(const SpectralPlan& p, Store st, const float2* Cin, const float* psi_in,
                      const void* w, double lambda, float* psi_out, float2* Cout, double* partials,
                      const PairRanges& pr, hipStream_t s) {
    XArgs a = base_args(p);
    a.pb0 = pr.b0;
    a.pn0 = pr.n0;
    a.pb1 = pr.b1;
    a.pn1 = pr.n1;
    a.Cin = Cin;
    a.Cout = Cout;
    a.psi_in = psi_in;
    a.psi_out = psi_out;
    a.w = w;
    a.lambda = lambda;
    a.partials = partials;
    return launch_x<XM_UPDATE>(a, st, p, s);
}

}
```

### spim_registration_amd/csrc/fftconv.hpp

```cpp
#pragma once

#include <cstdint>
#include <memory>
#include <vector>

#include "common.hpp"
#include "rl_kernels.hpp"

namespace spimdecon {

constexpr int kFftMaxStages = 16;

struct Fft1D {
    int L = 0;
    int ns = 0;
    uint64_t radix_packed = 0;
    const float2* tw = nullptr;
    int n1 = 0, n2 = 0;
    __host__ __device__ int radix(int s) const { return int((radix_packed >> (4 * s)) & 15u); }
};

struct EngineKnobs {
    bool ypf = true, zkd = true, zdirect = true;
    static EngineKnobs from_env();
};

struct SpectralPlan {
    SlabGeom g{};
    int64_t Hx = 0, Hp = 0;
    Fft1D fx, fy, fz;
    DBuf<float2> twx, twy, twz;
    DBuf<int> row_mirror;
    DBuf<int> row_one;
    mutable int xmode_update = -1;
    EngineKnobs knobs;
    int64_t spectrum_elems() const { return Hp * g.My * g.Mz; }
    void create(const SlabGeom& geom, bool allow_2f, bool z_fft, const EngineKnobs& knobs);
};

int64_t engine_fast_size(int64_t need, bool even, int policy = 0);

bool engine_slab_fits(int64_t nx, int64_t ny, int64_t nzs, const int halo[3], int policy);

void engine_forward_psi(const SpectralPlan& p, const float* psi, float2* C, hipStream_t s);
void engine_kernel_spectrum(const SpectralPlan& p, const float* d_kernel, int kx, int ky, int kz,
                            float scale, float2* Kspec, hipStream_t s);
bool engine_kernel_compact_ok(const SpectralPlan& p);
bool engine_zdirect_ok(const SpectralPlan& p);
bool engine_zdirect_dims_ok(int64_t Mx, int64_t My, int64_t Mz, int cz, bool zdirect_knob);
int engine_zpass_mode(const SpectralPlan& p, bool compact);
int64_t engine_kernel_compact_elems(const SpectralPlan& p);
void engine_kernel_compact(const SpectralPlan& p, const float* d_kernel, int kx, int ky, int kz, float scale,
                           float2* work, float2* Kc, hipStream_t s);
void engine_zpass_compact(const SpectralPlan& p, float2* C, const float2* Kc, hipStream_t s);
void engine_ypass(const SpectralPlan& p, float2* C, bool inv, hipStream_t s);
bool engine_ypass_planes(const SpectralPlan& p, float2* C, int z0, int z1, hipStream_t s);
bool engine_ypass_planes2(const SpectralPlan& p, float2* C, int z0, int z1, int z2, int z3, hipStream_t s);
void engine_zpass(const SpectralPlan& p, float2* C, const float2* K, hipStream_t s);
struct PairRanges {
    int b0 = 0, n0 = 0, b1 = 0, n1 = 0;
};
PairRanges all_pairs(const SpectralPlan& p);

void engine_quotient(const SpectralPlan& p, Store st, const float2* Cin, const void* img,
                     float2* Cout, const PairRanges& pr, hipStream_t s);
int64_t engine_update(const SpectralPlan& p, Store st, const float2* Cin, const float* psi_in,
                      const void* w, double lambda, float* psi_out, float2* Cout, double* partials,
                      const PairRanges& pr, hipStream_t s);

}
```

### spim_registration_amd/csrc/fftconv_2f.inc

```

#define SD_2F_SIZES(M)                                                                   \
    M(4, 4) M(4, 8) M(6, 8) M(8, 8) M(8, 12) M(8, 16) M(12, 16) M(16, 16) M(16, 24)     \
    M(16, 32) M(20, 27) M(24, 24) M(20, 32) M(25, 32) M(32, 32) M(30, 35) M(42, 50)

#define SD_2F_TR(A, B) (((A) > 32 || (B) > 32) ? 64 : 32)

constexpr int k2fMaxN = 64;

constexpr int k2fTX = 16;
constexpr int kKChunk = 9;

__device__ __forceinline__ float2 bload2(__amdgpu_buffer_rsrc_t r, int vo, int so) {
    return __builtin_bit_cast(float2, __builtin_amdgcn_raw_buffer_load_b64(r, vo, so, 0));
}
__device__ __forceinline__ void bstore2(__amdgpu_buffer_rsrc_t r, int vo, int so, float2 x) {
    __builtin_amdgcn_raw_buffer_store_b64(__builtin_bit_cast(__attribute__((ext_vector_type(2))) unsigned, x),
                                          r, vo, so, 0);
}

template <bool LDSONLY>
__device__ __forceinline__ void col_barrier() {
    if constexpr (LDSONLY) asm volatile("s_waitcnt lgkmcnt(0)\n\ts_barrier" ::: "memory");
    else __syncthreads();
}

template <int AXIS, int N1, int N2, int MODE, int TX, int TR, bool PF = false>
__global__ __launch_bounds__(TX * TR, (N1 * N2 > 1204 || (PF && N1 * N2 >= 640)) ? 2 : ((MODE >= 2 && N2 >= 32 && TR == 32) ? 3 : 4)) void k_col2f(SlabGeom g, int64_t Hp, const float2* twg,
                                                             float2* C, const float2* K, uint32_t bytes,
                                                             int tx0, int ntx, int kc, uint32_t kbytes,
                                                             int nout, int zsplit, int zskip) {
    constexpr int L = N1 * N2;
    static_assert(N1 <= TR && N2 <= TR, "factor exceeds the threads per column");
    constexpr int kThreads = TX * TR;
    constexpr bool INVA = MODE == 1;
    extern __shared__ __attribute__((aligned(16))) float2 smem[];
    float2* Y = smem;
    float2* tw = smem + L * TX;
    float2* Pk = tw + L;
    for (int i = threadIdx.x; i < L; i += kThreads) tw[i] = twg[i];
    __amdgpu_buffer_rsrc_t rc = __builtin_amdgcn_make_buffer_rsrc(C, 0, bytes, 0x00020000);
    const __amdgpu_buffer_rsrc_t rk =
        __builtin_amdgcn_make_buffer_rsrc(const_cast<float2*>(MODE >= 2 ? K : C), 0, MODE >= 2 ? kbytes : bytes,
                                          0x00020000);
    const int t = threadIdx.x;
    const int ntiles = ntx * (AXIS == 1 ? nout : int(g.My));
    const int es = int(AXIS == 1 ? Hp : g.My * Hp) * 8;
    const int os = AXIS == 1 ? 0 : int(Hp) * 8;
    static_assert(!PF || (AXIS == 1 && MODE < 2), "prefetch: y passes only");
    float2 vn[PF ? N1 : 1];
    auto plane_of = [&](int q) { return q + (q >= zsplit ? zskip : 0); };
    auto load_a = [&](int tl, int vo, float2* dst) {
        const __amdgpu_buffer_rsrc_t rt = __builtin_amdgcn_make_buffer_rsrc(
            C + (int64_t(plane_of(tl / ntx)) * g.My * Hp + int64_t(tx0 + tl % ntx) * TX), 0, bytes, 0x00020000);
        int sk = 0;
        asm volatile("" : "+s"(sk));
#pragma unroll
        for (int n1 = 0; n1 < N1; ++n1) {
            dst[n1] = bload2(rt, vo, sk);
            sk += N2 * es;
            asm volatile("" : "+s"(sk));
        }
    };
    if constexpr (PF) {
        const int r = t / TX;
        if (int(blockIdx.x) < ntiles && r < N2) load_a(int(blockIdx.x), (t % TX) * 8 + r * es, vn);
    }
    __syncthreads();
    for (int tile = blockIdx.x; tile < ntiles; tile += gridDim.x) {
        int tt = t;
        asm volatile("" : "+v"(tt));
        const int c = tt % TX;
        const int r = tt / TX;
        const int voA = c * 8 + r * es;
        const int voB = voA;
        int so;
        if constexpr (AXIS == 1) {
            rc = __builtin_amdgcn_make_buffer_rsrc(C + (int64_t(plane_of(tile / ntx)) * g.My * Hp + int64_t(tx0 + tile % ntx) * TX),
                                                   0, bytes, 0x00020000);
            so = 0;
            asm volatile("" : "+s"(so));
        } else {
            so = (tile / ntx) * os + (tx0 + tile % ntx) * TX * 8;
        }
        constexpr int KE = MODE == 4 ? (L * TX + kThreads - 1) / kThreads : 1;
        if constexpr (MODE == 5) {
            for (int i = tt; i < N2 * TX; i += kThreads) {
                const int n2 = i / TX;
                const bool lo = 2 * n2 < N2;
                const int jc = lo ? n2 + kc : n2 - N2 + kc;
                const bool nz = lo ? n2 <= kc : n2 >= N2 - kc;
                Pk[i] = bload2(rk, nz ? (i % TX) * 8 + jc * es : int(0x80000000), so);
            }
        }
        if (r < N2) {
            float2 v[N1];
            if constexpr (PF) {
#pragma unroll
                for (int n1 = 0; n1 < N1; ++n1) v[n1] = vn[n1];
            } else {
                int sk = so;
#pragma unroll
                for (int n1 = 0; n1 < N1; ++n1) {
                    v[n1] = bload2(rc, voA, sk);
                    sk += N2 * es;
                    asm volatile("" : "+s"(sk));
                }
            }
            fft_reg<N1, INVA>(v);
            __builtin_amdgcn_sched_barrier(0);
#pragma unroll
            for (int k1 = 0; k1 < N1; ++k1) {
                float2 w = tw[r * k1];
                if (INVA) w.y = -w.y;
                Y[(k1 * N2 + r) * TX + c] = k1 == 0 ? v[0] : cmul(v[k1], w);
            }
            if constexpr (PF) {
                const int next = tile + int(gridDim.x);
                if (next < ntiles) load_a(next, voA, vn);
            }
        }
        col_barrier<PF>();
        if constexpr (MODE == 4) {
            if (r < N1) {
                float2 u[N2];
#pragma unroll
                for (int n2 = 0; n2 < N2; ++n2) u[n2] = Y[(r * N2 + n2) * TX + c];
                fft_reg<N2, false>(u);
#pragma unroll
                for (int k2 = 0; k2 < N2; ++k2) Y[(r * N2 + k2) * TX + c] = u[k2];
            }
            float2 kr[KE];
            int vok = c * 8;
            asm volatile("" : "+v"(vok));
#pragma unroll
            for (int e = 0; e < KE; ++e) {
                const int q = r + TR * e;
                const int k = q / N2 + N1 * (q % N2);
                kr[e] = bload2(rk, q < L ? vok + k * es : int(0x80000000), so);
            }
            col_barrier<PF>();
#pragma unroll
            for (int e = 0; e < KE; ++e) {
                const int idx = tt + e * kThreads;
                if ((L * TX) % kThreads == 0 || e < KE - 1 || idx < L * TX) Y[idx] = cmul(Y[idx], kr[e]);
            }
            col_barrier<PF>();
            if (r < N1) {
                float2 u[N2];
#pragma unroll
                for (int k2 = 0; k2 < N2; ++k2) u[k2] = Y[(r * N2 + k2) * TX + c];
                fft_reg<N2, true>(u);
                __builtin_amdgcn_sched_barrier(0);
#pragma unroll
                for (int n2 = 0; n2 < N2; ++n2) {
                    float2 w = tw[n2 * r];
                    w.y = -w.y;
                    Y[(r * N2 + n2) * TX + c] = (n2 == 0 || r == 0) ? u[n2] : cmul(u[n2], w);
                }
            }
        } else if constexpr (MODE == 5) {
            if (r < N1) {
                float2 u[N2];
#pragma unroll
                for (int n2 = 0; n2 < N2; ++n2) u[n2] = Y[(r * N2 + n2) * TX + c];
                fft_reg<N2, false>(u);
#pragma unroll
                for (int k2 = 0; k2 < N2; ++k2) Y[(r * N2 + k2) * TX + c] = u[k2];
                asm volatile("" ::: "memory");
                float2 kk[N2];
#pragma unroll
                for (int n2 = 0; n2 < N2; ++n2) {
                    const int zs = 2 * n2 < N2 ? n2 : n2 - N2;
                    float2 w = tw[(zs < 0 ? -zs : zs) * r];
                    if (zs < 0) w.y = -w.y;
                    kk[n2] = cmul(Pk[n2 * TX + c], w);
                }
                fft_reg<N2, false>(kk);
#pragma unroll
                for (int k2 = 0; k2 < N2; ++k2) kk[k2] = cmul(Y[(r * N2 + k2) * TX + c], kk[k2]);
                fft_reg<N2, true>(kk);
                __builtin_amdgcn_sched_barrier(0);
#pragma unroll
                for (int n2 = 0; n2 < N2; ++n2) {
                    float2 w = tw[n2 * r];
                    w.y = -w.y;
                    Y[(r * N2 + n2) * TX + c] = (n2 == 0 || r == 0) ? kk[n2] : cmul(kk[n2], w);
                }
            }
        } else if (r < N1) {
            float2 u[N2];
#pragma unroll
            for (int n2 = 0; n2 < N2; ++n2) u[n2] = Y[(r * N2 + n2) * TX + c];
            fft_reg<N2, INVA>(u);
            if constexpr (MODE != 2) {
                int sk = so;
#pragma unroll
                for (int k2 = 0; k2 < N2; ++k2) {
                    bstore2(rc, voB, sk, u[k2]);
                    sk += N1 * es;
                    asm volatile("" : "+s"(sk));
                }
            } else {
                int vok = voB;
#pragma unroll
                for (int k0 = 0; k0 < N2; k0 += kKChunk) {
                    asm volatile("" : "+v"(vok));
#pragma unroll
                    for (int k2 = k0; k2 < (k0 + kKChunk < N2 ? k0 + kKChunk : N2); ++k2) {
                        u[k2] = cmul(u[k2], bload2(rk, vok, so + N1 * k2 * es));
                        asm volatile("" : "+v"(u[k2].x), "+v"(u[k2].y));
                    }
                }
                fft_reg<N2, true>(u);
                __builtin_amdgcn_sched_barrier(0);
#pragma unroll
                for (int n2 = 0; n2 < N2; ++n2) {
                    float2 w = tw[n2 * r];
                    w.y = -w.y;
                    Y[(r * N2 + n2) * TX + c] = (n2 == 0 || r == 0) ? u[n2] : cmul(u[n2], w);
                }
            }
        }
        if constexpr (MODE == 2 || MODE == 4 || MODE == 5) {
            col_barrier<PF>();
            if (r < N2) {
                float2 v[N1];
#pragma unroll
                for (int k1 = 0; k1 < N1; ++k1) v[k1] = Y[(k1 * N2 + r) * TX + c];
                fft_reg<N1, true>(v);
                int sk = so;
#pragma unroll
                for (int n1 = 0; n1 < N1; ++n1) {
                    bstore2(rc, N2 * n1 + r < nout ? voA : int(0x80000000), sk, v[n1]);
                    sk += N2 * es;
                    asm volatile("" : "+s"(sk));
                }
            }
        }
        col_barrier<PF>();
    }
}
```

### spim_registration_amd/csrc/fftconv_xt.inc

```

#ifndef SD_XT_VB_TIK64
#define SD_XT_VB_TIK64 2
#endif
#ifndef SD_XT_VB_TIK32
#define SD_XT_VB_TIK32 2
#endif
#ifndef SD_XT_REV
#define SD_XT_REV 1
#endif
#ifndef SD_XT_VB_WAVE
#define SD_XT_VB_WAVE 0
#endif
#ifndef SD_XT_PITCH4
#define SD_XT_PITCH4 1
#endif
#ifndef SD_XT_AMAP
#define SD_XT_AMAP 1
#endif
__host__ __device__ constexpr int xt_amap(int L, int NP) {
    return !SD_XT_AMAP ? 0 : NP == 8 && L == 1050 ? 2 : NP == 4 && (L == 1050 || L == 800) ? 3 : 0;
}
__host__ __device__ constexpr int xt_pitch(int L, int NP) {
    return xt_amap(L, NP) == 2 ? L + 2
         : xt_amap(L, NP) == 3 ? L + (L == 1050 ? 14 : 8)
         : L + 2 + (SD_XT_PITCH4 && (L + 2) % 4 == 0 ? 2 : 0);
}

__host__ __device__ constexpr size_t xt_lds(int L, int NP, bool twg) {
    return size_t((twg ? 0 : L + 2) + NP * xt_pitch(L, NP)) * 8u;
}
__host__ __device__ constexpr bool xt_twg(int L, int NP) {
    return 163840 / xt_lds(L, NP, true) > 163840 / xt_lds(L, NP, false);
}
#ifndef SD_XT_STAMPS
#define SD_XT_STAMPS 0
#endif
#if SD_XT_STAMPS
__device__ unsigned long long g_xt_stamp[3][8];
#define XT_STAMP(i)                                                                              \
    do {                                                                                         \
        __builtin_amdgcn_sched_barrier(0);                                                       \
        unsigned long long t_;                                                                   \
        asm volatile("s_memtime %0\n\ts_waitcnt lgkmcnt(0)" : "=s"(t_)::"memory");            \
        __builtin_amdgcn_sched_barrier(0);                                                       \
        xts[i] = t_;                                                                             \
    } while (0)
#else
#define XT_STAMP(i) do {} while (0)
#endif

#ifndef SD_XT_WAVE
#define SD_XT_WAVE 1
#endif
#ifndef SD_XT_WAVE_W
#define SD_XT_WAVE_W 2
#endif
#ifndef SD_XT_WAVE_QPF
#define SD_XT_WAVE_QPF 1
#endif
__host__ __device__ constexpr bool xt_wave(int L) {
    return (L == 2100 && (SD_XT_WAVE & 1)) || (L == 1050 && (SD_XT_WAVE & 2)) || (L == 800 && (SD_XT_WAVE & 4)) ||
           (L == 540 && (SD_XT_WAVE & 8));
}

__device__ __forceinline__ void xt_barrier() { asm volatile("s_waitcnt lgkmcnt(0)\n\ts_barrier" ::: "memory"); }

__device__ __forceinline__ float4 sel4(int c, float4 a, float4 b) {
    return make_float4(c ? a.x : b.x, c ? a.y : b.y, c ? a.z : b.z, c ? a.w : b.w);
}

struct XtTwGlobal {
    __amdgpu_buffer_rsrc_t r;
    __device__ __forceinline__ float2 operator[](int i) const {
        return __builtin_bit_cast(float2, __builtin_amdgcn_raw_buffer_load_b64(r, i * 8, 0, 0));
    }
};

__host__ __device__ constexpr int xt_np(int mode, int L) {
    return xt_wave(L) ? (L == 1050 || L == 2100 ? 1 : 2)
         : mode == XM_UPDATE && (L == 1050 || L == 800) ? 4 : 8;
}
constexpr int kXtVB = 4;

template <int L, int NP>
__device__ __forceinline__ void xt_cr(int t, int& c, int& r) {
    int tt = t;
    asm volatile("" : "+v"(tt));
    constexpr int AM = xt_amap(L, NP);
    constexpr int LNP = NP == 8 ? 3 : NP == 4 ? 2 : 0;
    static_assert(AM == 0 || (1 << LNP) == NP, "lane map for 4 or 8 row pairs");
    c = AM ? (tt >> AM) & (NP - 1) : tt % NP;
    r = AM ? (tt & ((1 << AM) - 1)) | ((tt >> (AM + LNP)) << AM) : tt / NP;
}

template <int N1, int N2, bool INV, int NP, typename TW>
__device__ __forceinline__ void xt_phaseA(float2* Z, TW tw, int P, int t) {
    int c, r;
    xt_cr<N1 * N2, NP>(t, c, r);
    float2* row = Z + c * P;
    if (r < N2) {
        float2 v[N1];
#pragma unroll
        for (int n1 = 0; n1 < N1; ++n1) v[n1] = row[N2 * n1 + r];
        fft_reg<N1, INV>(v);
        __builtin_amdgcn_sched_barrier(0);
#pragma unroll
        for (int k1 = 0; k1 < N1; ++k1) {
            float2 w = tw[r * k1];
            if (INV) w.y = -w.y;
            row[k1 * N2 + r] = k1 == 0 ? v[0] : cmul(v[k1], w);
        }
    }
    xt_barrier();
}

template <int N1, int N2, bool INV, int NP>
__device__ __forceinline__ void xt_phaseB(float2* Z, int P, int t) {
    int c, r;
    xt_cr<N1 * N2, NP>(t, c, r);
    float2* row = Z + c * P;
    float2 u[N2];
    if (r < N1) {
#pragma unroll
        for (int n2 = 0; n2 < N2; ++n2) u[n2] = row[r * N2 + n2];
    }
    xt_barrier();
    if (r < N1) {
        fft_reg<N2, INV>(u);
#pragma unroll
        for (int k2 = 0; k2 < N2; ++k2) row[r + N1 * k2] = u[k2];
    }
    xt_barrier();
}

template <int N1, int N2, bool INV, int NP, typename TW>
__device__ __forceinline__ void xt_fft(float2* Z, TW tw, int P, int t) {
    xt_phaseA<N1, N2, INV, NP>(Z, tw, P, t);
    xt_phaseB<N1, N2, INV, NP>(Z, P, t);
}

template <int S>
using vraw4 = typename std::conditional<S == 0, float4, uint2>::type;
template <int S>
__device__ __forceinline__ vraw4<S> bloadraw4(__amdgpu_buffer_rsrc_t r, uint32_t vox) {
    if constexpr (S == 0) return bload4(r, vox * 4u);
    else return __builtin_bit_cast(uint2, __builtin_amdgcn_raw_buffer_load_b64(r, int(vox * 2u), 0, 0));
}
template <int S>
__device__ __forceinline__ float4 cvt4(const vraw4<S>& u) {
    if constexpr (S == 0) {
        return u;
    } else {
        const float2 lo = __half22float2(__builtin_bit_cast(__half2, u.x));
        const float2 hi = __half22float2(__builtin_bit_cast(__half2, u.y));
        return make_float4(lo.x, lo.y, hi.x, hi.y);
    }
}


template <int MODE, int S, int N1, int N2, bool TIK, int NP, int TR>
__global__ __launch_bounds__(NP * TR, (NP * TR == 64 && N1 * N2 > 1204) ? SD_XT_WAVE_W : N1 * N2 > 1204 ? 2 : 4)
void k_xtile(XArgs a) {
    static_assert(N1 <= TR && N2 <= TR, "factor exceeds the threads per row pair");
    constexpr int kXtThreads = NP * TR;
    static_assert(MODE == XM_QUOT || MODE == XM_UPDATE || MODE == XM_PSI, "quotient / update / psi rows only");
    constexpr int L = N1 * N2;
    static_assert(L % 2 == 0, "even lengths only");
    constexpr int P = xt_pitch(L, NP);
    constexpr int cHx = L / 2 + 1;
    constexpr int cHp2 = (cHx + 15) / 16 * 8;
    constexpr int KS = (cHp2 + TR - 1) / TR;
    constexpr int KV = (L / 4 + TR - 1) / TR;
    extern __shared__ __attribute__((aligned(16))) float2 smem[];
    constexpr bool TWG = xt_twg(L, NP);
    float2* tw = smem;
    float2* Z = TWG ? smem : smem + L + 2;
    const XtTwGlobal twg{brsrc(a.fx.tw, uint32_t(L) * 8u)};
    const SlabGeom& g = a.g;
    constexpr int Hx = cHx;
    constexpr int Hp = cHp2 * 2;
    constexpr int Hp2 = cHp2;
    const int nx = int(g.nx);
    const int nx4 = nx / 4;
    const int ny = int(g.ny);
    const int My = int(g.My);
    const int cx = g.cx;
    const int t0 = threadIdx.x;
#if SD_XT_STAMPS
    unsigned long long xt_entry;
    asm volatile("s_memtime %0\n\ts_waitcnt lgkmcnt(0)" : "=s"(xt_entry)::"memory");
#endif
    if constexpr (!TWG)
        for (int i = t0; i < L; i += kXtThreads) tw[i] = a.fx.tw[i];
    const int nrows = int(g.My * g.Mz);
    const int nlin = a.pn0 + a.pn1;
    const int ntiles = (nlin + NP - 1) / NP;
    const __amdgpu_buffer_rsrc_t rcin = brsrc(a.Cin, a.spec_bytes);
    const __amdgpu_buffer_rsrc_t rcout = brsrc(a.Cout, a.Cout ? a.spec_bytes : 0u);
    const __amdgpu_buffer_rsrc_t rpsi = brsrc(a.psi_in, a.nvox * 4u);
    const __amdgpu_buffer_rsrc_t rpo = brsrc(a.psi_out, a.nvox * 4u);
    const __amdgpu_buffer_rsrc_t rimg = brsrc(MODE == XM_QUOT ? a.img : a.w, a.nvox * (S == 0 ? 4u : 2u));
    double ssum = 0.0;
    float smax = -1.0f;
    const double inv_lambda = TIK ? 1.0 / a.lambda : 0.0;
    __syncthreads();
#if SD_XT_STAMPS
    unsigned long long xts[8] = {0, 0, 0, 0, 0, 0, xt_entry, 0};
    bool xt_first = true;
#endif
    auto spec_issue = [&](int T, float4 (&xa)[KS], float4 (&xb)[KS]) {
        int tq = t0;
        asm volatile("" : "+v"(tq));
        const int c = tq / TR;
        const int hl = tq % TR;
        const int pr = T < ntiles ? x_pair(a, T * NP + c) : -1;
        const int r0 = pr >= 0 ? 2 * pr : nrows, r1 = r0 + 1;
        const bool v0 = r0 < nrows, v1 = r1 < nrows;
        int q0, q1;
        if constexpr (MODE == XM_QUOT) {
            q0 = v0 && a.row_one[r0] >= 0 ? r0 : -1;
            q1 = v1 && a.row_one[r1] >= 0 ? r1 : -1;
        } else {
            const int sm0 = v0 ? a.row_mirror[r0] : -1, sm1 = v1 ? a.row_mirror[r1] : -1;
            q0 = sm0 >= 0 ? (sm0 / ny) * My + sm0 % ny : -1;
            q1 = sm1 >= 0 ? (sm1 / ny) * My + sm1 % ny : -1;
        }
        const uint32_t o0 = q0 >= 0 ? uint32_t(q0) * uint32_t(Hp) * 8u : kOOB;
        const uint32_t o1 = q1 >= 0 ? uint32_t(q1) * uint32_t(Hp) * 8u : kOOB;
#pragma unroll
        for (int i = 0; i < KS; ++i) {
            const uint32_t jo = uint32_t(min(hl + TR * i, Hp2 - 1)) * 16u;
            xa[i] = bload4(rcin, o0 + jo);
            xb[i] = bload4(rcin, o1 + jo);
        }
    };
    for (int tile_ = blockIdx.x; tile_ < ntiles; tile_ += gridDim.x) {
        const int tile = SD_XT_REV ? ntiles - 1 - tile_ : tile_;
        XT_STAMP(0);
#define SD_XT_ROWS                                                                   \
    int tt_ = t0;                                                                    \
    asm volatile("" : "+v"(tt_));                                                    \
    const int c = tt_ / TR;                                                          \
    const int hl = tt_ % TR;                                                         \
    float2* zr = Z + c * P;                                                          \
     \
     \
                          \
    const int sw = ((hl >> 2) ^ (hl >> 3)) & 1;                                      \
    const int pr_ = x_pair(a, tile * NP + c);                                        \
    const int r0 = pr_ >= 0 ? 2 * pr_ : nrows, r1 = r0 + 1;                          \
    const bool v0 = r0 < nrows, v1 = r1 < nrows;                                     \
    const int sm0 = v0 ? a.row_mirror[r0] : -1, sm1 = v1 ? a.row_mirror[r1] : -1;   \
    const int so0 = v0 ? a.row_one[r0] : -1, so1 = v1 ? a.row_one[r1] : -1;         \
    (void)so0; (void)so1; (void)sm0; (void)sm1; (void)sw;
        constexpr bool QPF = MODE == XM_QUOT && (KV <= 5 || (SD_XT_WAVE_QPF && NP * TR == 64 && S == 1 && KV <= 9));
        vraw4<S> ia[MODE == XM_QUOT ? KV : 1], ib[MODE == XM_QUOT ? KV : 1];
        if constexpr (MODE != XM_PSI) {
        {
            SD_XT_ROWS
            float4 sa[KS], sb[KS];
            spec_issue(tile, sa, sb);
            if constexpr (QPF) {
                const uint32_t b0 = so0 >= 0 ? uint32_t(so0) * uint32_t(nx) : kOOBV;
                const uint32_t b1 = so1 >= 0 ? uint32_t(so1) * uint32_t(nx) : kOOBV;
#pragma unroll
                for (int i = 0; i < KV; ++i) {
                    const uint32_t jo = uint32_t(min(hl + TR * i, nx4 - 1)) * 4u;
                    ia[i] = bloadraw4<S>(rimg, b0 + jo);
                    ib[i] = bloadraw4<S>(rimg, b1 + jo);
                }
            }
#pragma unroll
            for (int i = 0; i < KS; ++i) {
                const int j = hl + TR * i;
                if (j >= Hp2) break;
                const float4 s0 = sa[i], s1 = sb[i];
                float2 zo[2];
#pragma unroll
                for (int h = 0; h < 2; ++h) {
                    const int k = 2 * j + h;
                    float2 xa = h ? make_float2(s0.z, s0.w) : make_float2(s0.x, s0.y);
                    float2 xb = h ? make_float2(s1.z, s1.w) : make_float2(s1.x, s1.y);
                    if (k == 0 || 2 * k == L) {
                        xa.y = 0.f;
                        xb.y = 0.f;
                    }
                    zo[h] = make_float2(xa.x - xb.y, xa.y + xb.x);
                    if (k < Hx && k > 0 && 2 * k < L) zr[L - k] = make_float2(xa.x + xb.y, xb.x - xa.y);
                }
                if (2 * j + 1 < Hx) *reinterpret_cast<float4*>(zr + 2 * j) = make_float4(zo[0].x, zo[0].y, zo[1].x, zo[1].y);
                else if (2 * j < Hx) zr[2 * j] = zo[0];
            }
        }
        xt_barrier();
        XT_STAMP(1);
        if constexpr (TWG) xt_fft<N1, N2, true, NP>(Z, twg, P, t0);
        else xt_fft<N1, N2, true, NP>(Z, (const float2*)tw, P, t0);
        XT_STAMP(2);
        }
        {
        SD_XT_ROWS
        if constexpr (MODE == XM_PSI) {
            const uint32_t b0 = sm0 >= 0 ? uint32_t(sm0) * uint32_t(nx) : kOOBV;
            const uint32_t b1 = sm1 >= 0 ? uint32_t(sm1) * uint32_t(nx) : kOOBV;
            float4 pa[KV], pb[KV];
#pragma unroll
            for (int i = 0; i < KV; ++i) {
                const uint32_t jo = uint32_t(min(hl + TR * i, nx4 - 1)) * 4u;
                pa[i] = bload4(rpsi, (b0 + jo) * 4u);
                pb[i] = bload4(rpsi, (b1 + jo) * 4u);
            }
#pragma unroll
            for (int i = 0; i < KV; ++i) {
                const int j = hl + TR * i;
                if (j >= nx4) break;
                float4* zq = reinterpret_cast<float4*>(zr + 4 * j);
                const float4 p0 = pa[i], p1 = pb[i];
                const float4 o01 = make_float4(p0.x, p1.x, p0.y, p1.y), o23 = make_float4(p0.z, p1.z, p0.w, p1.w);
                zq[sw] = sel4(sw, o23, o01);
                zq[sw ^ 1] = sel4(sw, o01, o23);
            }
            xt_barrier();
            for (int qx = nx + hl; qx < L; qx += TR) {
                const int sx = qx < nx + cx ? qx : qx - L;
                zr[qx] = zr[mirror_idx(sx, nx)];
            }
        } else if constexpr (MODE == XM_QUOT) {
            const float one0 = sm0 != -1 ? 1.0f : 0.0f;
            const float one1 = v1 && sm1 != -1 ? 1.0f : 0.0f;
            if constexpr (!QPF) {
                const uint32_t b0 = so0 >= 0 ? uint32_t(so0) * uint32_t(nx) : kOOBV;
                const uint32_t b1 = so1 >= 0 ? uint32_t(so1) * uint32_t(nx) : kOOBV;
#pragma unroll
                for (int i = 0; i < KV; ++i) {
                    const uint32_t jo = uint32_t(min(hl + TR * i, nx4 - 1)) * 4u;
                    ia[i] = bloadraw4<S>(rimg, b0 + jo);
                    ib[i] = bloadraw4<S>(rimg, b1 + jo);
                }
            }
#pragma unroll
            for (int i = 0; i < KV; ++i) {
                const int j = hl + TR * i;
                if (j >= nx4) break;
                const float4 i0 = cvt4<S>(ia[i]), i1 = cvt4<S>(ib[i]);
                float4* zq = reinterpret_cast<float4*>(zr + 4 * j);
                const float4 za = zq[sw], zb = zq[sw ^ 1];
                const float4 z01 = sel4(sw, zb, za), z23 = sel4(sw, za, zb);
                float qa[4], qb[4];
#pragma unroll
                for (int e = 0; e < 4; ++e) {
                    const float2 bz = e == 0 ? make_float2(z01.x, z01.y) : e == 1 ? make_float2(z01.z, z01.w)
                                    : e == 2 ? make_float2(z23.x, z23.y) : make_float2(z23.z, z23.w);
                    const float a0 = f4c(i0, e), a1 = f4c(i1, e);
                    qa[e] = (so0 >= 0 && a0 > 0.0f) ? __fdiv_rn(a0, bz.x) : one0;
                    qb[e] = (so1 >= 0 && a1 > 0.0f) ? __fdiv_rn(a1, bz.y) : one1;
                }
                const float4 o01 = make_float4(qa[0], qb[0], qa[1], qb[1]), o23 = make_float4(qa[2], qb[2], qa[3], qb[3]);
                zq[sw] = sel4(sw, o23, o01);
                zq[sw ^ 1] = sel4(sw, o01, o23);
            }
            for (int qx = nx + hl; qx < L; qx += TR) zr[qx] = make_float2(one0, one1);
        } else {
            const uint32_t b0 = sm0 >= 0 ? uint32_t(sm0) * uint32_t(nx) : kOOBV;
            const uint32_t b1 = sm1 >= 0 ? uint32_t(sm1) * uint32_t(nx) : kOOBV;
            const uint32_t w0o = so0 >= 0 ? b0 * 4u : kOOB, w1o = so1 >= 0 ? b1 * 4u : kOOB;
            auto upd4 = [&](int j, const float4& p0, const float4& p1, const float4& w0, const float4& w1) {
                const uint32_t jo = uint32_t(j) * 4u;
                float o0[4], o1[4];
                float4* zq = reinterpret_cast<float4*>(zr + 4 * j);
                const float4 za = zq[sw], zb = zq[sw ^ 1];
                const float4 z01 = sel4(sw, zb, za), z23 = sel4(sw, za, zb);
#pragma unroll
                for (int e = 0; e < 4; ++e) {
                    const float2 iz = e == 0 ? make_float2(z01.x, z01.y) : e == 1 ? make_float2(z01.z, z01.w)
                                    : e == 2 ? make_float2(z23.x, z23.y) : make_float2(z23.z, z23.w);
                    const float l0 = f4c(p0, e), l1 = f4c(p1, e);
                    const float n0 = next_value_t<TIK>(l0, iz.x, f4c(w0, e), a.lambda, inv_lambda);
                    const float n1 = next_value_t<TIK>(l1, iz.y, f4c(w1, e), a.lambda, inv_lambda);
                    o0[e] = sm0 >= 0 ? n0 : 0.f;
                    o1[e] = sm1 >= 0 ? n1 : 0.f;
                    const float c0 = so0 >= 0 ? fabsf(__fsub_rn(n0, l0)) : 0.f;
                    const float c1 = so1 >= 0 ? fabsf(__fsub_rn(n1, l1)) : 0.f;
                    ssum += (double)c0;
                    ssum += (double)c1;
                    smax = fmaxf(smax, fmaxf(c0, c1));
                }
                const float4 o01 = make_float4(o0[0], o1[0], o0[1], o1[1]), o23 = make_float4(o0[2], o1[2], o0[3], o1[3]);
                zq[sw] = sel4(sw, o23, o01);
                zq[sw ^ 1] = sel4(sw, o01, o23);
                __builtin_amdgcn_raw_buffer_store_b128(
                    __builtin_bit_cast(__attribute__((ext_vector_type(4))) unsigned,
                                       make_float4(o0[0], o0[1], o0[2], o0[3])),
                    rpo, int(w0o + jo * 4u), 0, 0);
                __builtin_amdgcn_raw_buffer_store_b128(
                    __builtin_bit_cast(__attribute__((ext_vector_type(4))) unsigned,
                                       make_float4(o1[0], o1[1], o1[2], o1[3])),
                    rpo, int(w1o + jo * 4u), 0, 0);
            };
            {
            constexpr int VBT = TR == 64 ? SD_XT_VB_TIK64 : (KV <= 5 ? SD_XT_VB_TIK32 : 0);
            constexpr int VB0 = (TIK && VBT > 0) ? (VBT < KV ? VBT : KV) : (KV <= 5 ? KV : kXtVB);
            constexpr bool WAVE = NP * TR == 64 && N1 * N2 > 1204;
            constexpr int VBW = SD_XT_VB_WAVE > 0 ? SD_XT_VB_WAVE : (S == 1 ? KV : 0);
            constexpr int VB = (WAVE && VBW > 0) ? (VBW < KV ? VBW : KV) : VB0;
            int hb = hl;
            for (int i0 = 0; i0 < KV; i0 += VB) {
            asm volatile("" : "+v"(hb));
            float4 pa[VB], pb[VB];
            vraw4<S> wa[VB], wb[VB];
#pragma unroll
            for (int i = 0; i < VB; ++i) {
                const uint32_t jo = uint32_t(min(hb + TR * (i0 + i), nx4 - 1)) * 4u;
                pa[i] = bload4(rpsi, (b0 + jo) * 4u);
                pb[i] = bload4(rpsi, (b1 + jo) * 4u);
                wa[i] = bloadraw4<S>(rimg, b0 + jo);
                wb[i] = bloadraw4<S>(rimg, b1 + jo);
            }
#pragma unroll
            for (int i = 0; i < VB; ++i) {
                const int j = hb + TR * (i0 + i);
                if (j < nx4) upd4(j, pa[i], pb[i], cvt4<S>(wa[i]), cvt4<S>(wb[i]));
            }
            }
            }
            xt_barrier();
            for (int qx = nx + hl; qx < L; qx += TR) {
                const int sx = qx < nx + cx ? qx : qx - L;
                zr[qx] = zr[mirror_idx(sx, nx)];
            }
        }
        }
        xt_barrier();
        XT_STAMP(3);
        if (!(MODE == XM_UPDATE && a.Cout == nullptr)) {
        if constexpr (TWG) xt_fft<N1, N2, false, NP>(Z, twg, P, t0);
        else xt_fft<N1, N2, false, NP>(Z, (const float2*)tw, P, t0);
        XT_STAMP(4);
        {
            SD_XT_ROWS
            const uint32_t o0 = v0 && sm0 != -1 ? uint32_t(r0) * uint32_t(Hp) * 8u : kOOB;
            const uint32_t o1 = v1 && sm1 != -1 ? uint32_t(r1) * uint32_t(Hp) * 8u : kOOB;
#pragma unroll
            for (int i = 0; i < KS; ++i) {
                const int j = hl + TR * i;
                if (j >= Hp2) break;
                float o[2][4];
                const float4 zkk = *reinterpret_cast<const float4*>(zr + 2 * j);
#pragma unroll
                for (int h = 0; h < 2; ++h) {
                    const int k = 2 * j + h;
                    float2 xa = make_float2(0.f, 0.f), xb = make_float2(0.f, 0.f);
                    if (k < Hx) {
                        const float2 zk = h ? make_float2(zkk.z, zkk.w) : make_float2(zkk.x, zkk.y);
                        const float2 zm = zr[k == 0 ? 0 : L - k];
                        xa = make_float2(0.5f * (zk.x + zm.x), 0.5f * (zk.y - zm.y));
                        xb = make_float2(0.5f * (zk.y + zm.y), -0.5f * (zk.x - zm.x));
                    }
                    o[0][2 * h] = xa.x;
                    o[0][2 * h + 1] = xa.y;
                    o[1][2 * h] = xb.x;
                    o[1][2 * h + 1] = xb.y;
                }
                __builtin_amdgcn_raw_buffer_store_b128(
                    __builtin_bit_cast(__attribute__((ext_vector_type(4))) unsigned,
                                       make_float4(o[0][0], o[0][1], o[0][2], o[0][3])),
                    rcout, int(o0 + uint32_t(j) * 16u), 0, 0);
                __builtin_amdgcn_raw_buffer_store_b128(
                    __builtin_bit_cast(__attribute__((ext_vector_type(4))) unsigned,
                                       make_float4(o[1][0], o[1][1], o[1][2], o[1][3])),
                    rcout, int(o1 + uint32_t(j) * 16u), 0, 0);
            }
        }
        xt_barrier();
#if SD_XT_STAMPS
        XT_STAMP(5);
        if (t0 == 0 && (tile & 63) == 0 && MODE >= 0 && MODE < 3) {
            for (int i = 0; i < 5; ++i) atomicAdd(&g_xt_stamp[MODE][i], xts[i + 1] - xts[i]);
            if (xt_first) atomicAdd(&g_xt_stamp[MODE][5], xts[0] - xts[6]);
            atomicAdd(&g_xt_stamp[MODE][7], 1ull);
        }
        xt_first = false;
#endif
        }
        break;
    }
#undef SD_XT_ROWS
    if constexpr (MODE == XM_UPDATE) {
        __shared__ double sh_sum[kXtThreads / 64];
        __shared__ float sh_max[kXtThreads / 64];
        for (int off = 32; off > 0; off >>= 1) {
            ssum += __shfl_xor(ssum, off, 64);
            smax = fmaxf(smax, __shfl_xor(smax, off, 64));
        }
        if ((t0 & 63) == 0) {
            sh_sum[t0 >> 6] = ssum;
            sh_max[t0 >> 6] = smax;
        }
        __syncthreads();
        if (t0 == 0) {
            for (int i = 1; i < kXtThreads / 64; ++i) {
                ssum += sh_sum[i];
                smax = fmaxf(smax, sh_max[i]);
            }
            a.partials[2 * blockIdx.x] = ssum;
            a.partials[2 * blockIdx.x + 1] = (double)smax;
        }
    }
}
```

### spim_registration_amd/csrc/session.cpp

```cpp
#include "session.hpp"

#include <algorithm>
#include <cmath>
#include <cstdio>
#include <cstdlib>
#include <cstring>
#include <chrono>
#include <exception>
#include <thread>

namespace spimdecon {

#define SD_NCCL(expr)                                                                          \
    do {                                                                                       \
        ncclResult_t _r = (expr);                                                              \
        if (_r != ncclSuccess)                                                                 \
            ::spimdecon::fail(SPIMDECON_ERR_COMM,                                              \
                              std::string(#expr " failed: ") + ncclGetErrorString(_r));        \
    } while (0)

void slab_range(int64_t nz, int nparts, int idx, int64_t* z0, int64_t* z1) {
    const int64_t base = nz / nparts, rem = nz % nparts;
    *z0 = int64_t(idx) * base + std::min<int64_t>(idx, rem);
    *z1 = *z0 + base + (idx < rem ? 1 : 0);
// ... 710 lines not shown

void Session::allreduce_max(double* host, int n) {
    if (!comm_) return;
    DeviceGuard guard(p_.device);
    DBuf<double> d(n);
    SD_HIP(hipMemcpyAsync(d.p, host, n * 8, hipMemcpyHostToDevice, stream_));
    SD_NCCL(ncclAllReduce(d.p, d.p, n, ncclDouble, ncclMax, comm_, stream_));
    SD_HIP(hipMemcpyAsync(host, d.p, n * 8, hipMemcpyDeviceToHost, stream_));
    wait_stream(stream_);
}

void Session::record_progress(hipStream_t st) {
    if (!comm_ || groups_.size() > 1) return;
    if (nprogress_ == progress_.size()) {
        hipEvent_t e;
        SD_HIP(hipEventCreateWithFlags(&e, hipEventDisableTiming));
        progress_.push_back(e);
    }
    SD_HIP(hipEventRecord(progress_[nprogress_++], st));
}

void Session::wait_stream(hipStream_t st) {
    if (!comm_) {
        SD_HIP(hipStreamSynchronize(st));
        return;
    }
    using clk = std::chrono::steady_clock;
    auto last = clk::now();
    size_t done = 0;
    int spins = 0;
    for (;;) {
        const hipError_t e = hipStreamQuery(st);
        if (e == hipSuccess) break;
        if (e != hipErrorNotReady) SD_HIP(e);
        while (done < nprogress_ && hipEventQuery(progress_[done]) == hipSuccess) {
            ++done;
            last = clk::now();
        }
        ncclResult_t ar = ncclSuccess;
        (void)ncclCommGetAsyncError(comm_, &ar);
        const double idle = std::chrono::duration<double>(clk::now() - last).count();
        if ((ar != ncclSuccess && ar != ncclInProgress) || idle > rccl_timeout_s_) {
            const std::string why = ar != ncclSuccess && ar != ncclInProgress
                                        ? std::string("RCCL asynchronous error: ") + ncclGetErrorString(ar)
                                        : "no progress for " + std::to_string(int(idle)) +
                                              " s (SPIMDECON_RCCL_TIMEOUT): mismatched halo exchanges across ranks?";
            (void)ncclCommAbort(comm_);
            comm_ = nullptr;
            rccl_dead_ = true;
            poisoned_ = true;
            fail(SPIMDECON_ERR_COMM, "rank " + std::to_string(p_.rank) + ": " + why + "; communicator aborted");
        }
        if (++spins > 2000) std::this_thread::sleep_for(std::chrono::microseconds(200));
    }
    if (st == stream_) nprogress_ = 0;
}

void Session::verify_ranks() {
    if (!comm_) return;
    constexpr int K = 12;
    int64_t ext = 0;
    for (auto& sl : slabs_) ext += sl.g.nz;
    const int64_t mine[K] = {0x5350494d44454301LL, p_.nranks, p_.rank, p_.nz_global, p_.z_offset, ext,
                             int64_t(axis_), int64_t(store_ == Store::F16), int64_t(backend_), int64_t(nviews_),
                             int64_t(halo_[2]), int64_t(plane_floats())};
    DeviceGuard guard(p_.device);
    const int R = p_.nranks;
    DBuf<int64_t> d(size_t(K) * R);
    std::vector<int64_t> all(size_t(K) * R, 0);
    SD_HIP(hipMemcpyAsync(d.p + size_t(K) * p_.rank, mine, sizeof(mine), hipMemcpyHostToDevice, stream_));
    SD_NCCL(ncclAllGather(d.p + size_t(K) * p_.rank, d.p, K, ncclInt64, comm_, stream_));
    SD_HIP(hipMemcpyAsync(all.data(), d.p, all.size() * 8, hipMemcpyDeviceToHost, stream_));
    wait_stream(stream_);
    static const char* names[K] = {"build", "nranks", "rank", "nz_global", "z_offset", "extent", "slab_axis",
                                   "storage_fp16", "fft_backend", "views", "halo planes", "plane floats"};
    std::string bad;
    for (int r = 0; r < R && bad.empty(); ++r) {
        const int64_t* q = all.data() + size_t(K) * r;
        for (int k = 0; k < K; ++k) {
            const bool must_equal = k != 2 && k != 4 && k != 5;
            if ((must_equal && q[k] != mine[k]) || (k == 2 && q[k] != r)) {
                bad = std::string(names[k]) + ": rank " + std::to_string(r) + " has " + std::to_string(q[k]) +
                      ", rank " + std::to_string(p_.rank) + " has " + std::to_string(mine[k]);
                break;
            }
        }
        if (bad.empty() && r + 1 < R) {
            const int64_t* n = q + K;
            if (q[4] + q[5] != n[4])
                bad = "rank " + std::to_string(r) + " owns [" + std::to_string(q[4]) + ", " +
                      std::to_string(q[4] + q[5]) + ") but rank " + std::to_string(r + 1) + " starts at " +
                      std::to_string(n[4]);
        }
    }
    if (bad.empty()) {
        const int64_t* l = all.data() + size_t(K) * (R - 1);
        if (all[4] != 0 || l[4] + l[5] != p_.nz_global)
            bad = "the ranks' ranges do not cover [0, nz_global)";
    }
    SD_CHECK(bad.empty(), SPIMDECON_ERR_ARG, "ranks disagree on the exchange geometry (" + bad + ")");
}

void Session::run(int iters, double lambda, double* stats) {
    SD_CHECK(!poisoned_, SPIMDECON_ERR_STATE, "an earlier multi-device run failed mid-iteration; destroy the session");
    SD_CHECK(iters >= 0, SPIMDECON_ERR_ARG, "iters must be >= 0");
    SD_CHECK(spectra_ready_, SPIMDECON_ERR_STATE, "call mvd_init (or mvd_set_kernels) first");
    SD_CHECK(psi_ready_, SPIMDECON_ERR_STATE, "call mvd_init_psi first");
    if (iters == 0) return;
    const int V = nviews_;
    nprogress_ = 0;
    for (auto& gr : groups_) {
        DeviceGuard guard(gr.dev);
        gr.stats.alloc(size_t(iters) * V * 2);
    }
    try {
        if (backend_ == 1) {
            DeviceGuard guard(p_.device);
            run_rocfft(iters, lambda);
        } else if (groups_.size() == 1) {
            DeviceGuard guard(p_.device);
            run_engine(0, iters, lambda, nullptr);
        } else {
            run_groups(iters, lambda);
        }
    } catch (...) {
        if (slabs_.size() > 1 || p_.nranks > 1) poisoned_ = true;
        throw;
    }
    static const bool quiet = [] {
        const char* e = std::getenv("SPIMDECON_WARN_FALLBACK");
        return e && e[0] == '0';
    }();
    if (backend_ == 0 && !quiet && !warned_fallback_) {
        for (int s = 0; s < int(slabs_.size()); ++s) {
            const int xm = slabs_[s].sp.xmode_update, zm = zpass_mode(s);
            if (xm != 2 || zm != 3) {
                std::fprintf(stderr,
                             "[spimdecon] warning: slab %d (%lld x %lld x %lld, padded %lld x %lld x %lld) runs "
                             "outside the fast engine passes (x pass %d, z pass %d; fast = 2 and 3): same "
                             "results, lower throughput\n",
                             s, (long long)slabs_[s].g.nx, (long long)slabs_[s].g.ny, (long long)slabs_[s].g.nz,
                             (long long)slabs_[s].g.Mx, (long long)slabs_[s].g.My, (long long)slabs_[s].g.Mz, xm,
                             zm);
                warned_fallback_ = true;
                break;
            }
        }
    }
    std::vector<double> st(size_t(iters) * V * 2, 0.0), part(st.size());
    for (size_t gi = 0; gi < groups_.size(); ++gi) {
        DevGroup& gr = groups_[gi];
        DeviceGuard guard(gr.dev);
        SD_HIP(hipMemcpyAsync(part.data(), gr.stats.p, part.size() * 8, hipMemcpyDeviceToHost, gr.stream));
        wait_stream(gr.stream);
        for (size_t i = 0; i < st.size(); i += 2) {
            st[i] = gi == 0 ? part[i] : st[i] + part[i];
            st[i + 1] = gi == 0 ? part[i + 1] : std::max(st[i + 1], part[i + 1]);
        }
    }
    if (comm_) {
        DeviceGuard guard(p_.device);
        std::vector<double> sums(size_t(iters) * V), maxs(size_t(iters) * V);
        for (size_t i = 0; i < sums.size(); ++i) {
            sums[i] = st[2 * i];
            maxs[i] = st[2 * i + 1];
        }
        allreduce_sum(sums.data(), int(sums.size()));
        allreduce_max(maxs.data(), int(maxs.size()));
        for (size_t i = 0; i < sums.size(); ++i) {
            st[2 * i] = sums[i];
            st[2 * i + 1] = maxs[i];
        }
    }
    if (stats) std::copy(st.begin(), st.end(), stats);
    if (timing_on_) {
        DeviceGuard guard(p_.device);
        for (auto& r : trecs_) {
            float ms = 0.f;
            SD_HIP(hipEventElapsedTime(&ms, r.a, r.b));
            tacc_[r.cls] += ms;
            tacc_[8 + r.cls] += double(r.weight);
            event_pool_.push_back(r.a);
            event_pool_.push_back(r.b);
        }
        trecs_.clear();
    }
}

void Session::run_groups(int iters, double lambda) {
    const int G = int(groups_.size());
    HostBarrier bar(G);
    std::vector<std::exception_ptr> errs(G);
    std::vector<std::thread> th;
    th.reserve(G);
    for (int gi = 0; gi < G; ++gi) {
        th.emplace_back([&, gi] {
            try {
                SD_HIP(hipSetDevice(groups_[gi].dev));
                run_engine(gi, iters, lambda, &bar);
            } catch (...) {
                errs[gi] = std::current_exception();
                bar.abort();
            }
        });
    }
    for (auto& t : th) t.join();
    for (auto& e : errs)
        if (e) poisoned_ = true;
    for (auto& e : errs)
        if (e) {
            try {
                std::rethrow_exception(e);
            } catch (const Error& x) {
                if (std::string(x.what()) != "device group aborted") throw;
            }
        }
    for (auto& e : errs)
        if (e) std::rethrow_exception(e);
    sync_all();
}

void Session::run_rocfft(int iters, double lambda) {
    const int V = nviews_;
    for (auto& sl : slabs_) {
        tstart(0);
        launch_pad_mirror(sl.g, sl.psi, sl.Ra.p, stream_);
        tstop();
    }
    exchange(true, stream_);
    for (int it = 0; it < iters; ++it) {
        for (int v = 0; v < V; ++v) {
            const bool last = (it == iters - 1) && (v == V - 1);
            for (auto& sl : slabs_) {
                tstart(2); sl.fft->forward(sl.Ra.p); tstop();
                tstart(3); launch_spec_mul(sl.Ra.p, sl.k1spec[v].p, sl.pd.complex_count(), stream_); tstop();
                tstart(4); sl.fft->inverse(sl.Ra.p); tstop();
                tstart(1); launch_quotient_pad(sl.g, store_, sl.img[v].p, sl.Ra.p, sl.Rb.p, stream_); tstop();
            }
            exchange(false, stream_);
            for (size_t s = 0; s < slabs_.size(); ++s) {
                SlabState& sl = slabs_[s];
                tstart(2); sl.fft->forward(sl.Rb.p); tstop();
                tstart(3); launch_spec_mul(sl.Rb.p, sl.k2spec[v].p, sl.pd.complex_count(), stream_); tstop();
                tstart(4); sl.fft->inverse(sl.Rb.p); tstop();
                tstart(0);
                const int64_t nb = launch_update_pad(sl.g, store_, sl.psi, sl.Rb.p, sl.w[v].p, lambda,
                                                     sl.psi_next, sl.Ra.p, sl.partials.p, !last, stream_);
                tstop();
                tstart(6);
                launch_reduce_partials(sl.partials.p, nb, groups_[0].stats.p + (size_t(it) * V + v) * 2,
                                       s > 0 ? 1 : 0, stream_);
                tstop();
                std::swap(sl.psi, sl.psi_next);
            }
            if (!last) exchange(true, stream_);
        }
        record_progress(stream_);
    }
}

void Session::run_engine(int gi, int iters, double lambda, HostBarrier* bar) {
    const int V = nviews_;
    DevGroup& gr = groups_[gi];
    hipStream_t st = gr.stream;
    const int s0 = gr.s0, s1 = gr.s1;
    const bool tm = gi == 0;
    auto T0 = [&](int cls) { if (tm) tstart(cls, st); };
    auto T1 = [&]() { if (tm) tstop(st); };
    const bool halo = slabs_.size() > 1 || p_.nranks > 1;
    std::vector<PairRanges> bnd(slabs_.size()), rest(slabs_.size());
    bool overlap = halo;
    for (int s = s0; s < s1; ++s) overlap = overlap && split_pairs(slabs_[s], bnd[s], rest[s]);
    auto xbegin = [&](bool buffer_a, bool window = true) {
        if (bar) {
            group_exchange_begin(gi, buffer_a, *bar);
        } else {
            SD_HIP(hipEventRecord(gr.ev_bnd, st));
            SD_HIP(hipStreamWaitEvent(gr.xstream, gr.ev_bnd, 0));
            exchange(buffer_a, gr.xstream);
            SD_HIP(hipEventRecord(gr.ev_x, gr.xstream));
        }
        if (tm && window) wstart(st);
    };
    const bool cb = cbnd_ && !bar;
    auto xbegin_cb = [&](bool buffer_a) {
        exchange(buffer_a, gr.xstream);
        SD_HIP(hipEventRecord(gr.ev_x, gr.xstream));
        if (tm) wstart(st);
    };
    auto xend = [&]() {
        if (tm) wstop(st);
        if (bar) group_exchange_end(gi);
        else SD_HIP(hipStreamWaitEvent(st, gr.ev_x, 0));
    };
    auto xfull = [&](bool buffer_a) {
        if (!halo) return;
        if (bar) {
            xbegin(buffer_a, false);
            xend();
        } else {
            exchange(buffer_a, st);
        }
    };
    auto convolve = [&](SlabState& sl, float2* Cb, const float2* K, bool fwd_done) {
        if (!fwd_done) { T0(2); engine_ypass(sl.sp, Cb, false, st); T1(); }
        T0(3);
        if (sl.kcompact) engine_zpass_compact(sl.sp, Cb, K, st);
        else engine_zpass(sl.sp, Cb, K, st);
        T1();
        T0(2); engine_ypass(sl.sp, Cb, true, st); T1();
    };
    const int czx = halo_[2];
    auto convolve_all = [&](bool buffer_a, int v, bool pending) {
        auto buf = [&](SlabState& sl) { return buffer_a ? sl.C1.p : sl.C2.p; };
        auto ker = [&](SlabState& sl) { return buffer_a ? sl.e1spec[v].p : sl.e2spec[v].p; };
        bool split = pending;
        for (int s = s0; s < s1 && split; ++s)
            split = slabs_[s].sp.fy.n1 != 0 && int(slabs_[s].g.nz) > 2 * czx;
        if (split) {
            for (int s = s0; s < s1; ++s) {
                SlabState& sl = slabs_[s];
                T0(2);
                SD_CHECK(engine_ypass_planes(sl.sp, buf(sl), czx, int(sl.g.nz) - czx, st), SPIMDECON_ERR_STATE,
                         "y pass of a plane range not available");
                T1();
            }
            xend();
            for (int s = s0; s < s1; ++s) {
                SlabState& sl = slabs_[s];
                T0(2);
                SD_CHECK(engine_ypass_planes2(sl.sp, buf(sl), 0, czx, int(sl.g.nz) - czx, int(sl.g.Mz), st),
                         SPIMDECON_ERR_STATE, "y pass of a plane range not available");
                T1();
            }
            for (int s = s0; s < s1; ++s) convolve(slabs_[s], buf(slabs_[s]), ker(slabs_[s]), true);
            return;
        }
        if (pending) xend();
        for (int s = s0; s < s1; ++s) convolve(slabs_[s], buf(slabs_[s]), ker(slabs_[s]), false);
    };

    for (int s = s0; s < s1; ++s) {
        T0(4);
        engine_forward_psi(slabs_[s].sp, slabs_[s].psi, slabs_[s].C1.p, st);
        T1();
    }
    xfull(true);
    bool pending = false;
    for (int it = 0; it < iters; ++it) {
        for (int v = 0; v < V; ++v) {
            const bool last = (it == iters - 1) && (v == V - 1);
            convolve_all(true, v, pending);
            pending = false;
            auto qin = [&](SlabState& sl) { return sl.C1.p; };
            auto qout = [&](SlabState& sl) { return sl.C2.p; };
            if (overlap && cb) {
                const int rq = tm ? rstart(1, st, s1 - s0) : -1;
                SD_HIP(hipEventRecord(gr.ev_pre, st));
                SD_HIP(hipStreamWaitEvent(gr.xstream, gr.ev_pre, 0));
                for (int s = s0; s < s1; ++s) {
                    SlabState& sl = slabs_[s];
                    engine_quotient(sl.sp, store_, qin(sl), sl.img[v].p, qout(sl), bnd[s], gr.xstream);
                }
                SD_HIP(hipEventRecord(gr.ev_bu, gr.xstream));
                xbegin_cb(false);
                for (int s = s0; s < s1; ++s) {
                    SlabState& sl = slabs_[s];
                    engine_quotient(sl.sp, store_, qin(sl), sl.img[v].p, qout(sl), rest[s], st);
                }
                if (rq >= 0) {
                    SD_HIP(hipStreamWaitEvent(st, gr.ev_bu, 0));
                    rstop(rq, st);
                }
            } else if (overlap) {
                for (int s = s0; s < s1; ++s) {
                    SlabState& sl = slabs_[s];
                    T0(1); engine_quotient(sl.sp, store_, qin(sl), sl.img[v].p, qout(sl), bnd[s], st); T1();
                }
                xbegin(false);
                for (int s = s0; s < s1; ++s) {
                    SlabState& sl = slabs_[s];
                    T0(1); engine_quotient(sl.sp, store_, qin(sl), sl.img[v].p, qout(sl), rest[s], st); T1();
                }
            } else {
                for (int s = s0; s < s1; ++s) {
                    SlabState& sl = slabs_[s];
                    T0(1);
                    engine_quotient(sl.sp, store_, qin(sl), sl.img[v].p, qout(sl), all_pairs(sl.sp), st);
                    T1();
                }
                xfull(false);
            }
            convolve_all(false, v, overlap);
            const bool ov = overlap && !last;
            std::vector<int64_t> nb(slabs_.size(), 0);
            const bool ovc = ov && cb;
            int ru = -1;
            if (ovc) {
                ru = tm ? rstart(0, st, s1 - s0) : -1;
                SD_HIP(hipEventRecord(gr.ev_pre, st));
                SD_HIP(hipStreamWaitEvent(gr.xstream, gr.ev_pre, 0));
            }
            for (int s = s0; s < s1; ++s) {
                SlabState& sl = slabs_[s];
                if (!ovc) T0(0);
                nb[s] = engine_update(sl.sp, store_, sl.C2.p, sl.psi, sl.w[v].p, lambda, sl.psi_next,
                                      last ? nullptr : sl.C1.p, sl.partials.p, ov ? bnd[s] : all_pairs(sl.sp),
                                      ovc ? gr.xstream : st);
                if (!ovc) T1();
            }
            if (ovc) SD_HIP(hipEventRecord(gr.ev_bu, gr.xstream));
            if (ov) {
                if (ovc) xbegin_cb(true);
                else xbegin(true);
                for (int s = s0; s < s1; ++s) {
                    SlabState& sl = slabs_[s];
                    if (!ovc) T0(0);
                    nb[s] += engine_update(sl.sp, store_, sl.C2.p, sl.psi, sl.w[v].p, lambda, sl.psi_next,
                                           sl.C1.p, sl.partials.p + 2 * nb[s], rest[s], st);
                    if (!ovc) T1();
                }
            }
            if (ovc) {
                SD_HIP(hipStreamWaitEvent(st, gr.ev_bu, 0));
                rstop(ru, st);
            }
            for (int s = s0; s < s1; ++s) {
                SlabState& sl = slabs_[s];
                T0(6);
                launch_reduce_partials(sl.partials.p, nb[s], gr.stats.p + (size_t(it) * V + v) * 2,
                                       s > s0 ? 1 : 0, st);
                T1();
                std::swap(sl.psi, sl.psi_next);
            }
            if (ov) pending = true;
            else if (!last) xfull(true);
        }
        record_progress(st);
    }
}

void Session::apply_mask() {
    SD_CHECK(!poisoned_, SPIMDECON_ERR_STATE, "an earlier multi-device run failed mid-iteration; psi is inconsistent");
    SD_CHECK(psi_ready_, SPIMDECON_ERR_STATE, "psi not initialised");
    for (auto& sl : slabs_) {
        DeviceGuard guard(groups_[sl.grp].dev);
        launch_mask(sl.psi, sl.n, nviews_, store_, sl.img_ptrs.p, groups_[sl.grp].stream);
    }
    sync_all();
}

void Session::get_psi(float* out) {
    SD_CHECK(!poisoned_, SPIMDECON_ERR_STATE, "an earlier multi-device run failed mid-iteration; psi is inconsistent");
    SD_CHECK(psi_ready_, SPIMDECON_ERR_STATE, "psi not initialised");
    SD_CHECK(out, SPIMDECON_ERR_ARG, "null output");
    for (auto& sl : slabs_) {
        DeviceGuard guard(groups_[sl.grp].dev);
        DBuf<float> tmp;
        store_slab(sl, sl.psi, out, tmp, groups_[sl.grp].stream);
        wait_stream(groups_[sl.grp].stream);
    }
}

float* Session::psi_device(int slab) {
    SD_CHECK(slab >= 0 && slab < int(slabs_.size()), SPIMDECON_ERR_ARG, "bad slab");
    return slabs_[slab].psi;
}

void Session::fft_dims(int slab, int64_t* out3) const {
    SD_CHECK(slab >= 0 && slab < int(slabs_.size()), SPIMDECON_ERR_ARG, "bad slab");
    SD_CHECK(spectra_ready_, SPIMDECON_ERR_STATE, "not initialised");
    for (int d = 0; d < 3; ++d) out3[d] = slabs_[slab].pd.M[d];
}

int Session::zpass_mode(int slab) const {
    SD_CHECK(slab >= 0 && slab < int(slabs_.size()), SPIMDECON_ERR_ARG, "bad slab");
    SD_CHECK(spectra_ready_, SPIMDECON_ERR_STATE, "not initialised");
    if (backend_ != 0) return -1;
    return engine_zpass_mode(slabs_[slab].sp, slabs_[slab].kcompact);
}

int Session::xpass_mode(int slab) const {
    SD_CHECK(slab >= 0 && slab < int(slabs_.size()), SPIMDECON_ERR_ARG, "bad slab");
    SD_CHECK(spectra_ready_, SPIMDECON_ERR_STATE, "not initialised");
    if (backend_ != 0) return -2;
    return slabs_[slab].sp.xmode_update;
}

int Session::kernel_planes(int slab) const {
    SD_CHECK(slab >= 0 && slab < int(slabs_.size()), SPIMDECON_ERR_ARG, "bad slab");
    SD_CHECK(spectra_ready_, SPIMDECON_ERR_STATE, "not initialised");
    const SlabState& sl = slabs_[slab];
    if (backend_ != 0) return int(sl.pd.M[2]);
    return sl.kcompact ? int(2 * sl.sp.g.cz + 1) : int(sl.sp.g.Mz);
}

}
```

### spim_registration_amd/csrc/session.hpp

```cpp
#pragma once

#include <rccl/rccl.h>

#include <atomic>
#include <condition_variable>
#include <memory>
#include <mutex>
#include <vector>

#include "common.hpp"
#include "fft.hpp"
#include "fftconv.hpp"
#include "kernel_prep.hpp"
#include "rl_kernels.hpp"

namespace spimdecon {

struct SlabState {
    int grp = 0;
    SlabGeom g{};
    PadDims pd;
    int64_t local_z0 = 0;
    int64_t n = 0;
    DBuf<float> psi_a, psi_b;
    float* psi = nullptr;
    float* psi_next = nullptr;
    std::vector<DBuf<char>> img, w;
    std::vector<DBuf<float>> k1spec, k2spec;
    DBuf<float> Ra, Rb;
    SpectralPlan sp;
    DBuf<float2> C1, C2;
    std::vector<DBuf<float2>> e1spec, e2spec;
    bool kcompact = false;
    bool zexact = false;
    DBuf<double> partials;
    DBuf<const void*> img_ptrs;
    std::unique_ptr<FftPlan3D> fft;
};

struct TimingRec {
    int cls;
    hipEvent_t a, b;
    int weight = 1;
};

struct DevGroup {
    int dev = 0;
    int s0 = 0, s1 = 0;
    hipStream_t stream = nullptr;
    hipStream_t xstream = nullptr;
    hipEvent_t ev_bnd = nullptr, ev_x = nullptr;
    hipEvent_t ev_pre = nullptr, ev_bu = nullptr;
    DBuf<double> stats;
};

struct HaloPlan {
    int64_t send_lo, recv_lo, send_hi, recv_hi, count;
};
HaloPlan halo_plan(int64_t nz, int64_t Mz, int64_t cz, int64_t plane);

class HostBarrier {
public:
    explicit HostBarrier(int n) : n_(n) {}
    void wait();
    void abort();

private:
    std::mutex mu_;
    std::condition_variable cv_;
    int n_, count_ = 0;
    uint64_t gen_ = 0;
    bool aborted_ = false;
};

class Session {
public:
    explicit Session(const mvd_params& p, const std::vector<int>& devs = {});
    ~Session();

    void add_view(const float* img, const float* weight, const float* k1, const int* kdims,
                  bool device_ptrs);
    void init(int psftype);
    void set_kernels(int view, const float* k1, const float* k2);
    void get_kernels(int view, float* k1, float* k2) const;
    double init_psi(const float* psi_or_null);
    void run(int iters, double lambda, double* stats);
    void apply_mask();
    void get_psi(float* out);
    float* psi_device(int slab);
    void fft_dims(int slab, int64_t* out3) const;
    int kernel_planes(int slab) const;
    int zpass_mode(int slab) const;
    int xpass_mode(int slab) const;
    hipStream_t stream() const { return groups_[0].stream; }
    int ndevices() const { return int(groups_.size()); }
    int nslabs() const { return int(slabs_.size()); }
    void slab_extent(int slab, int64_t* out3) const;
    void exchange_stats(int64_t* bytes, int64_t* copies) const;
    int slab_device(int slab) const;
    void enable_timing(bool on) { timing_on_ = on; }
    void timing(double* out16);

private:
    void build_spectra();
    void load_slab(const float* src, hipMemcpyKind kind, const SlabState& sl, float* dst, DBuf<float>& tmp,
                   hipStream_t st) const;
    void store_slab(const SlabState& sl, const float* src, float* out, DBuf<float>& tmp, hipStream_t st) const;
    HostKernel internal_kernel(const HostKernel& k) const;
    static float* buf_ptr(SlabState& sl, bool a, int backend);
    size_t plane_floats() const;
    void exchange(bool buffer_a, hipStream_t st);
    void group_exchange_begin(int gi, bool buffer_a, HostBarrier& bar);
    void group_exchange_end(int gi);
    bool split_pairs(const SlabState& sl, PairRanges& bnd, PairRanges& rest) const;
    void run_rocfft(int iters, double lambda);
    void run_engine(int gi, int iters, double lambda, HostBarrier* bar);
    void run_groups(int iters, double lambda);
    void sync_all();
    void allreduce_sum(double* host, int n);
    void allreduce_max(double* host, int n);
    void tstart(int cls, hipStream_t st = nullptr);
    void tstop(hipStream_t st = nullptr);
    void wstart(hipStream_t st);
    void wstop(hipStream_t st);
    int rstart(int cls, hipStream_t st, int weight);
    void rstop(int rec, hipStream_t st);
    int wcur_ = -1;

    mvd_params p_{};
    int64_t odims_[3] = {0, 0, 0};
    int axis_ = 0;
    int backend_ = 0;
    Store store_ = Store::F32;
    std::vector<DevGroup> groups_;
    hipStream_t stream_ = nullptr;
    ncclComm_t comm_ = nullptr;
    std::vector<SlabState> slabs_;
    std::vector<HostKernel> k1_, k2_;
    int nviews_ = 0;
    int halo_[3] = {0, 0, 0};
    bool kernels_ready_ = false;
    bool spectra_ready_ = false;
    bool psi_ready_ = false;
    bool poisoned_ = false;
    bool warned_fallback_ = false;
    bool cbnd_ = true;
    bool pull_kernel_ = false;
    void copy_halo(float* dst, const float* src, size_t bytes, hipStream_t st, bool peer);
    std::atomic<int64_t> xbytes_{0}, xcopies_{0};
    bool timing_on_ = false;
    std::vector<TimingRec> trecs_;
    int tcur_ = -1;
    double tacc_[16] = {0};
    std::vector<hipEvent_t> event_pool_;
    hipEvent_t get_event();

    double rccl_timeout_s_ = 300.0;
    bool rccl_dead_ = false;
    std::vector<hipEvent_t> progress_;
    size_t nprogress_ = 0;
    void wait_stream(hipStream_t st);
    void record_progress(hipStream_t st);
    void verify_ranks();
};

}
```

### spim_registration_amd/decon.py

```python
from __future__ import annotations

import atexit
import ctypes as C
import weakref
from enum import IntEnum

import numpy as np

from . import _lib
from ._lib import check, fptr

MIN_VALUE = np.float32(0.0001)


class PSFTYPE(IntEnum):
    OPTIMIZATION_II = 0
    OPTIMIZATION_I = 1
    EFFICIENT_BAYESIAN = 2
    INDEPENDENT = 3


def _as_volume(a, name):
    a = np.ascontiguousarray(a, dtype=np.float32)
    if a.ndim != 3:
        raise ValueError(f"{name} must be a 3D [z, y, x] array, got shape {a.shape}")
    return a


def _kdims(k):
    kz, ky, kx = k.shape
    if kx % 2 == 0 or ky % 2 == 0 or kz % 2 == 0:
        raise ValueError(f"kernel dims must be odd (EfficientBayesianBased.java:792-799), got {k.shape}")
    return np.array([kx, ky, kz], np.int32)


class MVDeconFFT:

    def __init__(self, image, weight, kernel, block_factory=None, device_list=(0,),
                 use_blocks=False, block_size=None, save_memory=False):
        self.image = _as_volume(image, "image")
        self.weight = _as_volume(weight, "weight")
        if self.weight.shape != self.image.shape:
            raise ValueError("image and weight dims differ")
        self.kernel1 = _as_volume(kernel, "kernel")
        _kdims(self.kernel1)
        self.kernel2 = None
        self.device_list = list(device_list)
        if not self.device_list or any(d < 0 for d in self.device_list):
            raise ValueError("device_list must hold GPU ids >= 0 (no CPU path in this framework)")
        self.use_blocks = use_blocks
        self.block_size = block_size
        self.save_memory = save_memory
        self.num_views = 0

    def set_num_views(self, n):
        self.num_views = n

    def get_image(self):
        return self.image

    def get_weight(self):
        return self.weight

    def get_kernel1(self):
        return self.kernel1

    def get_kernel2(self):
        return self.kernel2


class MVDeconInput:
    min_value = MIN_VALUE

    def __init__(self, img_factory=None):
        self.views: list[MVDeconFFT] = []
        self.img_factory = img_factory

    def add(self, view: MVDeconFFT):
        self.views.append(view)
        for v in self.views:
            v.set_num_views(len(self.views))

    def get_views(self):
        return self.views

    def get_num_views(self):
        return len(self.views)

    def init(self, iteration_type: PSFTYPE, ij_threads: int = 8):
        prepare_kernels(self.views, iteration_type, ij_threads)
        return self


def prepare_kernels(views, iteration_type, ij_threads=8, device=None):
    lib = _lib.load()
    V = len(views)
    k1_in = [np.ascontiguousarray(v.kernel1, np.float32) for v in views]
    k1_out = [np.empty_like(k) for k in k1_in]
    k2_out = [np.empty_like(k) for k in k1_in]
    kd = np.concatenate([_kdims(k) for k in k1_in]).astype(np.int32)
    PF = C.POINTER(C.c_float)
    arr_in = (PF * V)(*[fptr(k) for k in k1_in])
    arr_o1 = (PF * V)(*[fptr(k) for k in k1_out])
    arr_o2 = (PF * V)(*[fptr(k) for k in k2_out])
    dev = views[0].device_list[0] if device is None else device
    check(lib.mvd_prepare_kernels(V, arr_in, _lib.iptr(kd), int(iteration_type), int(ij_threads),
                                  arr_o1, arr_o2, int(dev)))
    for v, a, b in zip(views, k1_out, k2_out):
        v.kernel1, v.kernel2 = a, b
    return k1_out, k2_out


_open_sessions: "weakref.WeakSet[Session]" = weakref.WeakSet()


@atexit.register
def _close_open_sessions() -> None:
    for s in list(_open_sessions):
        s.close()


class Session:

    def __init__(self, dims_xyz, device=0, local_slabs=1, nranks=1, rank=0, comm_id=None,
                 nz_global=None, z_offset=0, storage_fp16=False, ij_threads=8, halo=None,
                 fft_backend="engine", fft_pad_policy="auto", devices=None, slab_axis="auto"):
        self.lib = _lib.load()
        p = _lib.MvdParams()
        self.lib.mvd_params_default(C.byref(p))
        for d in range(3):
            p.dims[d] = int(dims_xyz[d])
        p.nz_global = int(nz_global) if nz_global is not None else 0
        p.z_offset = int(z_offset)
        p.device = int(device)
        p.local_slabs = int(local_slabs)
        p.nranks = int(nranks)
        p.rank = int(rank)
        self._comm_id = comm_id
        p.comm_id = comm_id
        p.storage_fp16 = int(bool(storage_fp16))
        p.ij_threads = int(ij_threads)
        p.fft_backend = {"engine": 0, "rocfft": 1}[fft_backend]
        p.fft_pad_policy = {"auto": 0, "fast": 1, "smooth": 2}[fft_pad_policy]
        p.slab_axis = {"z": 0, "y": 1, "auto": -1}[slab_axis]
        if halo is not None:
            for d in range(3):
                p.halo[d] = int(halo[d])
        h = C.c_void_p()
        if devices is not None and len(devices) > 1:
            devs = np.ascontiguousarray(devices, np.int32)
            check(self.lib.mvd_create_devices(_lib.iptr(devs), len(devs), C.byref(p), C.byref(h)))
        else:
            if devices:
                p.device = int(devices[0])
            check(self.lib.mvd_create(C.byref(p), C.byref(h)))
        self.h = h
        _open_sessions.add(self)
        self.params = p
        self.nviews = 0
        self.shape = (int(dims_xyz[2]), int(dims_xyz[1]), int(dims_xyz[0]))

    def close(self):
        if getattr(self, "h", None):
            self.lib.mvd_destroy(self.h)
            self.h = None
            _open_sessions.discard(self)

    def __del__(self):
        self.close()

    def __enter__(self):
        return self

    def __exit__(self, *a):
        self.close()

    def add_view(self, img, weight, kernel1):
        img = _as_volume(img, "img")
        weight = _as_volume(weight, "weight")
        if img.shape != self.shape or weight.shape != self.shape:
            raise ValueError(f"view dims {img.shape} != session dims {self.shape}")
        k = _as_volume(kernel1, "kernel1")
        check(self.lib.mvd_add_view(self.h, fptr(img), fptr(weight), fptr(k), _lib.iptr(_kdims(k))))
        self.nviews += 1

    def add_view_device(self, d_img_ptr, d_weight_ptr, kernel1):
        k = _as_volume(kernel1, "kernel1")
        check(self.lib.mvd_add_view_device(self.h, C.c_void_p(d_img_ptr), C.c_void_p(d_weight_ptr),
                                           fptr(k), _lib.iptr(_kdims(k))))
        self.nviews += 1

    def init(self, psftype):
        check(self.lib.mvd_init(self.h, int(psftype)))

    def set_kernels(self, view, k1, k2):
        k1 = np.ascontiguousarray(k1, np.float32)
        k2 = np.ascontiguousarray(k2, np.float32)
        check(self.lib.mvd_set_kernels(self.h, int(view), fptr(k1), fptr(k2)))

    def get_kernels(self, view, kshape):
        k1 = np.empty(kshape, np.float32)
        k2 = np.empty(kshape, np.float32)
        check(self.lib.mvd_get_kernels(self.h, int(view), fptr(k1), fptr(k2)))
        return k1, k2

    def init_psi(self, psi=None):
        avg = C.c_double(0.0)
        if psi is None:
            check(self.lib.mvd_init_psi(self.h, None, C.byref(avg)))
        else:
            psi = _as_volume(psi, "psi")
            check(self.lib.mvd_init_psi(self.h, fptr(psi), C.byref(avg)))
        return avg.value

    def run(self, iters, lam):
        stats = np.zeros((max(iters, 1), max(self.nviews, 1), 2), np.float64)
        check(self.lib.mvd_run(self.h, int(iters), float(lam),
                               stats.ctypes.data_as(C.POINTER(C.c_double))))
        return stats[:iters]

    def apply_mask(self):
        check(self.lib.mvd_apply_mask(self.h))

    def get_psi(self):
        out = np.empty(self.shape, np.float32)
        check(self.lib.mvd_get_psi(self.h, fptr(out)))
        return out

    def fft_dims(self, slab=0):
        out = (C.c_int64 * 3)()
        check(self.lib.mvd_fft_dims(self.h, int(slab), out))
        return tuple(out)

    def kernel_planes(self, slab=0):
        out = C.c_int()
        check(self.lib.mvd_kernel_planes(self.h, int(slab), C.byref(out)))
        return out.value

    def zpass_mode(self, slab=0):
        out = C.c_int()
        check(self.lib.mvd_zpass_mode(self.h, int(slab), C.byref(out)))
        return out.value

    def xpass_mode(self, slab=0):
        out = C.c_int()
        check(self.lib.mvd_xpass_mode(self.h, int(slab), C.byref(out)))
        return out.value

    def num_devices(self):
        out = C.c_int()
        check(self.lib.mvd_num_devices(self.h, C.byref(out)))
        return out.value

    def slab_device(self, slab):
        out = C.c_int()
        check(self.lib.mvd_slab_device(self.h, int(slab), C.byref(out)))
        return out.value

    def num_slabs(self):
        out = C.c_int()
        check(self.lib.mvd_num_slabs(self.h, C.byref(out)))
        return out.value

    def exchange_stats(self):
        b, c = C.c_int64(), C.c_int64()
        check(self.lib.mvd_exchange_stats(self.h, C.byref(b), C.byref(c)))
        return b.value, c.value

    def slab_extent(self, slab=0):
        out = (C.c_int64 * 3)()
        check(self.lib.mvd_slab_extent(self.h, int(slab), out))
        return tuple(out)

    def enable_timing(self, on=True):
        check(self.lib.mvd_enable_timing(self.h, int(on)))

    def timing(self):
        out = (C.c_double * 16)()
        check(self.lib.mvd_timing(self.h, out))
        return list(out)

    def stream(self):
        return self.lib.mvd_stream(self.h)


class MVDeconvolution:

    min_value = MIN_VALUE

    def __init__(self, views: MVDeconInput, iteration_type: PSFTYPE, num_iterations: int,
                 lam: float, osem_speedup: float = 1.0, osem_speedup_index: int = 0,
                 name: str = "deconvolved", *, ij_threads: int = 8, initial_image=None,
                 local_slabs: int = 1, storage_fp16: bool = False, run: bool = True):
        self.views = views
        self.name = name
        self.num_iterations = int(num_iterations)
        self.lam = float(lam)
        data = views.get_views()
        if not data:
            raise ValueError("no views")
        shape = data[0].get_image().shape
        devs = list(data[0].device_list)
        self.session = Session((shape[2], shape[1], shape[0]), devices=devs, local_slabs=local_slabs,
                               storage_fp16=storage_fp16, ij_threads=ij_threads)
        for v in data:
            self.session.add_view(v.get_image(), v.get_weight(), v.kernel1)
        self.session.init(iteration_type)
        for i, v in enumerate(data):
            v.kernel1, v.kernel2 = self.session.get_kernels(i, v.kernel1.shape)
        self.avg = self.session.init_psi(initial_image)
        self.stats = np.zeros((0, len(data), 2))
        self.i = 0
        if run:
            self.run_iterations(self.num_iterations)
            self.session.apply_mask()

    def run_iterations(self, n):
        st = self.session.run(n, self.lam)
        self.stats = np.concatenate([self.stats, st]) if self.stats.size else st
        self.i += n

    def run_iteration(self):
        self.run_iterations(1)

    def get_psi(self):
        return self.session.get_psi()

    def get_current_iteration(self):
        return self.i

    def get_data(self):
        return self.views

    def get_name(self):
        return self.name
```

Before: 9970 Mvoxels/s per RL iteration.

## Skip x-pass on z-extension planes and rebuild them from mirror images during y-FFT

Planes in the z-padding region are exact mirror copies, or constant-one planes, of interior planes. The x-transform now processes only interior half-rows through a compacted pair index. The forward y two-factor kernel then writes the transformed result of each source plane to all of its mirror destination planes, and for the second buffer loads a precomputed transformed one-plane. This removes the redundant x and y FFT work on the padding planes at the cost of extra scattered stores, new lookup tables, a new kernel parameter and more register and branch pressure in the y kernel. An environment knob can turn it off, and it falls back when the geometry conditions are not met.

```diff
diff --git a/include/spimdecon.h b/include/spimdecon.h
--- a/include/spimdecon.h
+++ b/include/spimdecon.h
@@ -128,6 +128,7 @@
 int mvd_kernel_planes(mvd_session* h, int slab, int* planes);
 int mvd_zpass_mode(mvd_session* h, int slab, int* mode);
 int mvd_xpass_mode(mvd_session* h, int slab, int* mode);
+int mvd_padrows_mode(mvd_session* h, int slab, int* mode);
 void* mvd_stream(mvd_session* h);
 int mvd_enable_timing(mvd_session* h, int on);
 int mvd_timing(mvd_session* h, double* out16);
diff --git a/spim_registration_amd/_lib.py b/spim_registration_amd/_lib.py
--- a/spim_registration_amd/_lib.py
+++ b/spim_registration_amd/_lib.py
@@ -163,6 +163,7 @@
     "mvd_kernel_planes": (C.c_int, [C.c_void_p, C.c_int, C.POINTER(C.c_int)]),
     "mvd_zpass_mode": (C.c_int, [C.c_void_p, C.c_int, C.POINTER(C.c_int)]),
     "mvd_xpass_mode": (C.c_int, [C.c_void_p, C.c_int, C.POINTER(C.c_int)]),
+    "mvd_padrows_mode": (C.c_int, [C.c_void_p, C.c_int, C.POINTER(C.c_int)]),
     "mvd_stream": (C.c_void_p, [C.c_void_p]),
     "mvd_enable_timing": (C.c_int, [C.c_void_p, C.c_int]),
     "mvd_timing": (C.c_int, [C.c_void_p, _pd]),
diff --git a/spim_registration_amd/csrc/capi.cpp b/spim_registration_amd/csrc/capi.cpp
--- a/spim_registration_amd/csrc/capi.cpp
+++ b/spim_registration_amd/csrc/capi.cpp
@@ -299,6 +299,10 @@
     return guarded([&] { SESSION(h); SD_CHECK(mode, SPIMDECON_ERR_ARG, "null"); *mode = S.zpass_mode(slab); });
 }
 
+int mvd_padrows_mode(mvd_session* h, int slab, int* mode) {
+    return guarded([&] { SESSION(h); SD_CHECK(mode, SPIMDECON_ERR_ARG, "null"); *mode = S.padrows_mode(slab); });
+}
+
 int mvd_xpass_mode(mvd_session* h, int slab, int* mode) {
     return guarded([&] { SESSION(h); SD_CHECK(mode, SPIMDECON_ERR_ARG, "null"); *mode = S.xpass_mode(slab); });
 }
diff --git a/spim_registration_amd/csrc/fftconv.hip b/spim_registration_amd/csrc/fftconv.hip
--- a/spim_registration_amd/csrc/fftconv.hip
+++ b/spim_registration_amd/csrc/fftconv.hip
@@ -196,10 +196,17 @@
     uint32_t spec_bytes;
     uint32_t nvox;
     int pb0, pn0, pb1, pn1;
+    int hp, hy;
 };
 
 __device__ __forceinline__ int x_pair(const XArgs& a, int i) {
     return i < a.pn0 ? a.pb0 + i : (i - a.pn0 < a.pn1 ? a.pb1 + (i - a.pn0) : -1);
+}
+__device__ __forceinline__ int xt_pair(const XArgs& a, int i) {
+    const int ci = x_pair(a, i);
+    if (a.hp <= 0 || ci < 0) return ci;
+    const int pl = ci / a.hp;
+    return pl * a.hy + (ci - pl * a.hp);
 }
 
 constexpr int kXThreads = 256;
@@ -473,6 +480,30 @@
     return true;
 }
 
+void xt_compact(const SpectralPlan& p, XArgs& b) {
+    b.hp = b.hy = 0;
+    if (!p.padrows || b.g.Mz != p.g.Mz) return;
+    SD_CHECK(p.ext0 >= p.g.nz, SPIMDECON_ERR_STATE, "extension planes inside the slab");
+    const int64_t hy = p.g.My / 2, hp = (p.g.ny + 1) / 2, nz = p.g.nz;
+    auto conv = [&](int& pb, int& pn) {
+        if (pn <= 0) {
+            pb = pn = 0;
+            return true;
+        }
+        const int64_t e = int64_t(pb) + pn;
+        if (pb % hy != 0 || e % hy != 0) return false;
+        const int64_t z0 = std::min<int64_t>(pb / hy, nz), z1 = std::min<int64_t>(e / hy, nz);
+        pb = int(z0 * hp);
+        pn = int((z1 - z0) * hp);
+        return true;
+    };
+    XArgs c = b;
+    if (!conv(c.pb0, c.pn0) || !conv(c.pb1, c.pn1)) return;
+    c.hp = int(hp);
+    c.hy = int(hy);
+    b = c;
+}
+
 template <int MODE>
 unsigned launch_xtile(const XArgs& a, Store st, const SpectralPlan& p, hipStream_t s) {
     XArgs b;
@@ -481,7 +512,8 @@
     const int NP = xt_np(MODE, L);
     const size_t lds = xt_lds(L, NP, xt_twg(L, NP));
     if (lds > 160 * 1024) return 0;
-    const unsigned grid = unsigned(std::max<int64_t>(1, ceil_div(int64_t(a.pn0) + a.pn1, int64_t(NP))));
+    xt_compact(p, b);
+    const unsigned grid = unsigned(std::max<int64_t>(1, ceil_div(int64_t(b.pn0) + b.pn1, int64_t(NP))));
     const int sv = st == Store::F32 ? 0 : 1;
     bool done = false;
     const bool tik = MODE == XM_UPDATE && a.lambda > 0.0;
@@ -591,7 +623,8 @@
 
 template <int AXIS, int MODE>
 bool launch_col2f(const SpectralPlan& p, const Fft1D& f, float2* C, const float2* K, hipStream_t s,
-                  int tx0 = 0, int ntxb = -1, int kc = 0, int nout = -1, int zsplit = INT_MAX, int zskip = 0) {
+                  int tx0 = 0, int ntxb = -1, int kc = 0, int nout = -1, int zsplit = INT_MAX, int zskip = 0,
+                  const YPad& yp = YPad{}) {
     if (nout < 0) nout = int(p.g.Mz);
     const int L = f.L;
     const int tr = (f.n1 > 32 || f.n2 > 32) ? 64 : 32;
@@ -614,6 +647,8 @@
     const unsigned grid = unsigned(std::min<int64_t>(ntiles, 256 * per_cu * kColGridRounds));
     const int n1 = f.n1, n2 = f.n2;
     const bool pf = p.knobs.ypf && AXIS == 1 && MODE < 2 && tr == 32 && TX == 16 && lds > size_t(80 * 1024);
+    SD_CHECK(yp.mode == 0 || (AXIS == 1 && MODE == 0 && tr == 32 && TX == k2fTX && !pf && yext_len(L)),
+             SPIMDECON_ERR_STATE, "extension rebuild asked of a y kernel without it");
     bool done = false;
 #define SD_2F_L(A, B, T, PFV)                                                                                   \
             constexpr int TRv = SD_2F_TR(A, B);                                                                 \
@@ -621,7 +656,7 @@
                                        hipFuncAttributeMaxDynamicSharedMemorySize, int(lds)));                  \
             hipLaunchKernelGGL((k_col2f<AXIS, A, B, MODE, T, TRv, PFV>), dim3(grid), dim3(T * TRv), lds, s,     \
                                p.g, p.Hp, f.tw, C, K, rbytes, tx0, ntxb, kc, uint32_t(kbytes), nout, zsplit,  \
-                               zskip);                                                                       \
+                               zskip, yp);                                                                   \
             done = true;
 #define SD_2F_C1(A, B, T)                                                                                  \
     if constexpr (MODE < 2 || SD_2F_TR(A, B) == 32) {                                                      \
@@ -721,6 +756,7 @@
     k.ypf = !off("SPIMDECON_YPF");
     k.zkd = !off("SPIMDECON_ZKD");
     k.zdirect = zdirect_env();
+    k.padrows = !off("SPIMDECON_PADROWS");
     return k;
 }
 
@@ -772,6 +808,72 @@
     row_one.alloc(nrows);
     SD_HIP(hipMemcpy(row_mirror.p, rm.data(), nrows * sizeof(int), hipMemcpyHostToDevice));
     SD_HIP(hipMemcpy(row_one.p, ro.data(), nrows * sizeof(int), hipMemcpyHostToDevice));
+    create_padrows();
+}
+
+void SpectralPlan::create_padrows() {
+    padrows = false;
+    ext0 = ext1 = int(g.Mz);
+    if (!knobs.padrows || g.My % 2 != 0 || !fx.n1 || !fy.n1) return;
+    if (fy.n1 > 32 || fy.n2 > 32 || !yext_len(fy.L)) return;
+    if (g.cy > g.ny - 1 || g.My - g.ny - g.cy > g.ny - 1) return;
+    auto mir = [](int64_t sidx, int64_t n) -> int64_t {
+        if (n == 1) return 0;
+        const int64_t p = 2 * (n - 1);
+        int64_t j = sidx % p;
+        if (j < 0) j += p;
+        return j >= n ? p - j : j;
+    };
+    const int Mz = int(g.Mz);
+    std::vector<int> src(Mz, -1);
+    int first = -1, last = -1, count = 0;
+    for (int qz = 0; qz < Mz; ++qz) {
+        const int64_t sz = qz < g.nz + g.cz ? qz : qz - g.Mz;
+        const int64_t gz = g.z0 + sz;
+        if (gz >= 0 && gz < g.nzg) continue;
+        src[qz] = int(mir(gz, g.nzg) - g.z0);
+        if (first < 0) first = qz;
+        last = qz;
+        ++count;
+    }
+    if (count > 0 && (last - first + 1 != count || first < g.nz)) return;
+    if (count > 0) {
+        ext0 = first;
+        ext1 = last + 1;
+    }
+    std::vector<int> start(Mz + 1, 0), list(std::max(count, 1), 0);
+    for (int qz = ext0; qz < ext1; ++qz) start[src[qz] + 1]++;
+    for (int z = 0; z < Mz; ++z) start[z + 1] += start[z];
+    {
+        std::vector<int> fill(start.begin(), start.end() - 1);
+        for (int qz = ext0; qz < ext1; ++qz) list[fill[src[qz]]++] = qz;
+    }
+    img_start.alloc(start.size());
+    img_list.alloc(list.size());
+    SD_HIP(hipMemcpy(img_start.p, start.data(), start.size() * sizeof(int), hipMemcpyHostToDevice));
+    SD_HIP(hipMemcpy(img_list.p, list.data(), list.size() * sizeof(int), hipMemcpyHostToDevice));
+    hipStream_t s = nullptr;
+    const size_t My = size_t(g.My);
+    one_plane.alloc(My * size_t(Hp));
+    one_row.alloc(size_t(Hp));
+    std::vector<int> live(My, 0), ones(My, -2);
+    DBuf<int> dlive(My), dones(My);
+    SD_HIP(hipMemcpy(dlive.p, live.data(), My * sizeof(int), hipMemcpyHostToDevice));
+    SD_HIP(hipMemcpy(dones.p, ones.data(), My * sizeof(int), hipMemcpyHostToDevice));
+    XArgs a = base_args(*this);
+    a.g.Mz = 1;
+    a.pn0 = int((g.My + 1) / 2);
+    a.row_mirror = dlive.p;
+    a.row_one = dones.p;
+    a.Cout = one_plane.p;
+    launch_x<XM_QUOT>(a, Store::F32, *this, s);
+    SD_HIP(hipMemcpyAsync(one_row.p, one_plane.p, size_t(Hp) * sizeof(float2), hipMemcpyDeviceToDevice, s));
+    const bool ok = launch_col2f<1, 0>(*this, fy, one_plane.p, nullptr, s, 0, -1, 0, 1);
+    SD_HIP(hipStreamSynchronize(s));
+    const YPadTables tb{img_start.p, img_list.p, one_row.p, one_plane.p, g.cy};
+    pad_tables.alloc(1);
+    SD_HIP(hipMemcpy(pad_tables.p, &tb, sizeof(tb), hipMemcpyHostToDevice));
+    padrows = ok;
 }
 
 void engine_forward_psi(const SpectralPlan& p, const float* psi, float2* C, hipStream_t s) {
@@ -920,21 +1022,71 @@
     SD_HIP(hipGetLastError());
 }
 
-void engine_ypass(const SpectralPlan& p, float2* C, bool inv, hipStream_t s) {
+static YPad ypad_of(const SpectralPlan& p, YExt ext) {
+    YPad y;
+    if (!p.padrows || ext == YExt::Full) return y;
+    y.mode = int(ext);
+    y.ny = int(p.g.ny);
+    y.tab = p.pad_tables.p;
+    return y;
+}
+
+static void launch_yfwd_ext(const SpectralPlan& p, float2* C, int z0, int z1, int z2, int z3, YPad y,
+                            hipStream_t s) {
+    int r[3][2];
+    int n = 0;
+    auto add = [&](int a, int b) {
+        if (b <= a) return;
+        if (n > 0 && r[n - 1][1] == a) {
+            r[n - 1][1] = b;
+            return;
+        }
+        r[n][0] = a;
+        r[n][1] = b;
+        ++n;
+    };
+    for (const auto& q : {std::pair<int, int>(z0, z1), std::pair<int, int>(z2, z3)}) {
+        add(q.first, std::min(q.second, p.ext0));
+        add(std::max(q.first, p.ext1), q.second);
+    }
+    if (n == 0) return;
+    const int len0 = r[0][1] - r[0][0], len1 = n > 1 ? r[1][1] - r[1][0] : 0, len2 = n > 2 ? r[2][1] - r[2][0] : 0;
+    y.zbase = r[0][0];
+    if (n > 2) {
+        y.zsplit2 = len0 + len1;
+        y.zskip2 = r[2][0] - r[1][1];
+    }
+    const bool ok = launch_col2f<1, 0>(p, p.fy, C, nullptr, s, 0, -1, 0, len0 + len1 + len2, n > 1 ? len0 : INT_MAX,
+                                       n > 1 ? r[1][0] - r[0][1] : 0, y);
+    SD_CHECK(ok, SPIMDECON_ERR_STATE, "two-factor y pass not available under the extension skip");
+}
+
+void engine_ypass(const SpectralPlan& p, float2* C, bool inv, hipStream_t s, YExt ext) {
+    const YPad y = ypad_of(p, ext);
+    if (y.mode != 0 && !inv) return launch_yfwd_ext(p, C, 0, int(p.g.Mz), 0, 0, y, s);
     if (inv) launch_col<1, true, 0>(p, p.fy, C, nullptr, s, int(p.g.nz));
     else launch_col<1, false, 0>(p, p.fy, C, nullptr, s);
 }
 
-bool engine_ypass_planes2(const SpectralPlan& p, float2* C, int z0, int z1, int z2, int z3, hipStream_t s) {
+bool engine_ypass_planes2(const SpectralPlan& p, float2* C, int z0, int z1, int z2, int z3, hipStream_t s,
+                          YExt ext) {
     if (!p.fy.n1 || z0 < 0 || z1 < z0 || z2 < z1 || z3 < z2 || z3 > int(p.g.Mz)) return false;
     if (z3 - z2 + z1 - z0 <= 0) return true;
+    if (const YPad y = ypad_of(p, ext); y.mode != 0) {
+        launch_yfwd_ext(p, C, z0, z1, z2, z3, y, s);
+        return true;
+    }
     return launch_col2f<1, 0>(p, p.fy, C + size_t(z0) * size_t(p.g.My) * size_t(p.Hp), nullptr, s, 0, -1, 0,
                               (z1 - z0) + (z3 - z2), z1 - z0, z2 - z1);
 }
 
-bool engine_ypass_planes(const SpectralPlan& p, float2* C, int z0, int z1, hipStream_t s) {
+bool engine_ypass_planes(const SpectralPlan& p, float2* C, int z0, int z1, hipStream_t s, YExt ext) {
     if (!p.fy.n1 || z0 < 0 || z1 > int(p.g.Mz)) return false;
     if (z1 <= z0) return true;
+    if (const YPad y = ypad_of(p, ext); y.mode != 0) {
+        launch_yfwd_ext(p, C, z0, z1, z1, z1, y, s);
+        return true;
+    }
     return launch_col2f<1, 0>(p, p.fy, C + size_t(z0) * size_t(p.g.My) * size_t(p.Hp), nullptr, s, 0, -1, 0,
                               z1 - z0);
 }
diff --git a/spim_registration_amd/csrc/fftconv.hpp b/spim_registration_amd/csrc/fftconv.hpp
--- a/spim_registration_amd/csrc/fftconv.hpp
+++ b/spim_registration_amd/csrc/fftconv.hpp
@@ -21,8 +21,16 @@
 };
 
 struct EngineKnobs {
-    bool ypf = true, zkd = true, zdirect = true;
+    bool ypf = true, zkd = true, zdirect = true, padrows = true;
     static EngineKnobs from_env();
+};
+
+struct YPadTables {
+    const int* img_start;
+    const int* img_list;
+    const float2* one_row;
+    const float2* one_plane;
+    int cy;
 };
 
 struct SpectralPlan {
@@ -34,8 +42,16 @@
     DBuf<int> row_one;
     mutable int xmode_update = -1;
     EngineKnobs knobs;
+    bool padrows = false;
+    int ext0 = 0, ext1 = 0;
+    DBuf<int> img_start, img_list;
+    DBuf<float2> one_row, one_plane;
+    DBuf<YPadTables> pad_tables;
     int64_t spectrum_elems() const { return Hp * g.My * g.Mz; }
     void create(const SlabGeom& geom, bool allow_2f, bool z_fft, const EngineKnobs& knobs);
+
+private:
+    void create_padrows();
 };
 
 int64_t engine_fast_size(int64_t need, bool even, int policy = 0);
@@ -53,9 +69,11 @@
 void engine_kernel_compact(const SpectralPlan& p, const float* d_kernel, int kx, int ky, int kz, float scale,
                            float2* work, float2* Kc, hipStream_t s);
 void engine_zpass_compact(const SpectralPlan& p, float2* C, const float2* Kc, hipStream_t s);
-void engine_ypass(const SpectralPlan& p, float2* C, bool inv, hipStream_t s);
-bool engine_ypass_planes(const SpectralPlan& p, float2* C, int z0, int z1, hipStream_t s);
-bool engine_ypass_planes2(const SpectralPlan& p, float2* C, int z0, int z1, int z2, int z3, hipStream_t s);
+enum class YExt { Full = 0, Mirror = 1, One = 2 };
+void engine_ypass(const SpectralPlan& p, float2* C, bool inv, hipStream_t s, YExt ext = YExt::Full);
+bool engine_ypass_planes(const SpectralPlan& p, float2* C, int z0, int z1, hipStream_t s, YExt ext = YExt::Full);
+bool engine_ypass_planes2(const SpectralPlan& p, float2* C, int z0, int z1, int z2, int z3, hipStream_t s,
+                          YExt ext = YExt::Full);
 void engine_zpass(const SpectralPlan& p, float2* C, const float2* K, hipStream_t s);
 struct PairRanges {
     int b0 = 0, n0 = 0, b1 = 0, n1 = 0;
diff --git a/spim_registration_amd/csrc/fftconv_2f.inc b/spim_registration_amd/csrc/fftconv_2f.inc
--- a/spim_registration_amd/csrc/fftconv_2f.inc
+++ b/spim_registration_amd/csrc/fftconv_2f.inc
@@ -24,11 +24,21 @@
     else __syncthreads();
 }
 
+struct YPad {
+    int mode = 0;
+    int ny = 0;
+    int zbase = 0;
+    int zsplit2 = INT_MAX, zskip2 = 0;
+    const YPadTables* tab = nullptr;
+};
+typedef const __attribute__((address_space(4))) YPadTables* YPadTabPtr;
+__host__ __device__ constexpr bool yext_len(int L) { return size_t(L * k2fTX + L) * 8u <= size_t(80) * 1024; }
+
 template <int AXIS, int N1, int N2, int MODE, int TX, int TR, bool PF = false>
 __global__ __launch_bounds__(TX * TR, (N1 * N2 > 1204 || (PF && N1 * N2 >= 640)) ? 2 : ((MODE >= 2 && N2 >= 32 && TR == 32) ? 3 : 4)) void k_col2f(SlabGeom g, int64_t Hp, const float2* twg,
                                                              float2* C, const float2* K, uint32_t bytes,
                                                              int tx0, int ntx, int kc, uint32_t kbytes,
-                                                             int nout, int zsplit, int zskip) {
+                                                             int nout, int zsplit, int zskip, YPad yp) {
     constexpr int L = N1 * N2;
     static_assert(N1 <= TR && N2 <= TR, "factor exceeds the threads per column");
     constexpr int kThreads = TX * TR;
@@ -48,12 +58,41 @@
     const int os = AXIS == 1 ? 0 : int(Hp) * 8;
     static_assert(!PF || (AXIS == 1 && MODE < 2), "prefetch: y passes only");
     float2 vn[PF ? N1 : 1];
-    auto plane_of = [&](int q) { return q + (q >= zsplit ? zskip : 0); };
-    auto load_a = [&](int tl, int vo, float2* dst) {
-        const __amdgpu_buffer_rsrc_t rt = __builtin_amdgcn_make_buffer_rsrc(
-            C + (int64_t(plane_of(tl / ntx)) * g.My * Hp + int64_t(tx0 + tl % ntx) * TX), 0, bytes, 0x00020000);
-        int sk = 0;
-        asm volatile("" : "+s"(sk));
+    constexpr bool YEXT = AXIS == 1 && MODE == 0 && TR == 32 && !PF && yext_len(N1 * N2);
+    auto plane_of = [&](int q) {
+        const int pl = q + (q >= zsplit ? zskip : 0);
+        if constexpr (YEXT) return yp.zbase + pl + (q >= yp.zsplit2 ? yp.zskip2 : 0);
+        else return pl;
+    };
+    auto load_col = [&](const __amdgpu_buffer_rsrc_t& rt, int64_t col, int c, int r, int s0, float2* dst) {
+        if constexpr (YEXT) {
+            if (yp.mode != 0) {
+                const YPadTabPtr tb = (YPadTabPtr)(yp.tab);
+                const bool one = yp.mode == 2;
+                float2 onev = make_float2(0.f, 0.f);
+                if (one) onev = tb->one_row[col + c];
+                const int nyc = yp.ny + tb->cy, m2 = 2 * (yp.ny - 1);
+#pragma unroll
+                for (int n1 = 0; n1 < N1; ++n1) {
+                    const int e = N2 * n1 + r;
+                    const bool ext = e >= yp.ny;
+                    const int row = ext ? (e < nyc ? m2 : L) - e : e;
+                    dst[n1] = bload2(rt, ext && one ? int(0x80000000) : c * 8 + row * es, s0);
+                }
+                if (one) {
+                    int rr = r;
+                    asm volatile("" : "+v"(rr));
+#pragma unroll
+                    for (int n1 = 0; n1 < N1; ++n1) {
+                        const bool ext = N2 * n1 + rr >= yp.ny;
+                        dst[n1] = make_float2(ext ? onev.x : dst[n1].x, ext ? onev.y : dst[n1].y);
+                    }
+                }
+                return;
+            }
+        }
+        const int vo = c * 8 + r * es;
+        int sk = s0;
 #pragma unroll
         for (int n1 = 0; n1 < N1; ++n1) {
             dst[n1] = bload2(rt, vo, sk);
@@ -61,9 +100,17 @@
             asm volatile("" : "+s"(sk));
         }
     };
+    auto load_a = [&](int tl, int c, int r, float2* dst) {
+        const int64_t col = int64_t(tx0 + tl % ntx) * TX;
+        const __amdgpu_buffer_rsrc_t rt = __builtin_amdgcn_make_buffer_rsrc(
+            C + (int64_t(plane_of(tl / ntx)) * g.My * Hp + col), 0, bytes, 0x00020000);
+        int s0 = 0;
+        asm volatile("" : "+s"(s0));
+        load_col(rt, col, c, r, s0, dst);
+    };
     if constexpr (PF) {
         const int r = t / TX;
-        if (int(blockIdx.x) < ntiles && r < N2) load_a(int(blockIdx.x), (t % TX) * 8 + r * es, vn);
+        if (int(blockIdx.x) < ntiles && r < N2) load_a(int(blockIdx.x), t % TX, r, vn);
     }
     __syncthreads();
     for (int tile = blockIdx.x; tile < ntiles; tile += gridDim.x) {
@@ -98,13 +145,7 @@
 #pragma unroll
                 for (int n1 = 0; n1 < N1; ++n1) v[n1] = vn[n1];
             } else {
-                int sk = so;
-#pragma unroll
-                for (int n1 = 0; n1 < N1; ++n1) {
-                    v[n1] = bload2(rc, voA, sk);
-                    sk += N2 * es;
-                    asm volatile("" : "+s"(sk));
-                }
+                load_col(rc, int64_t(tx0 + tile % ntx) * TX, c, r, so, v);
             }
             fft_reg<N1, INVA>(v);
             __builtin_amdgcn_sched_barrier(0);
@@ -116,7 +157,7 @@
             }
             if constexpr (PF) {
                 const int next = tile + int(gridDim.x);
-                if (next < ntiles) load_a(next, voA, vn);
+                if (next < ntiles) load_a(next, c, r, vn);
             }
         }
         col_barrier<PF>();
@@ -200,6 +241,38 @@
                     sk += N1 * es;
                     asm volatile("" : "+s"(sk));
                 }
+                if constexpr (YEXT) {
+                    if (yp.mode != 0) {
+                        const YPadTabPtr tb = (YPadTabPtr)(yp.tab);
+                        const int pl = plane_of(tile / ntx);
+                        const int64_t col = int64_t(tx0 + tile % ntx) * TX;
+                        const int i0 = tb->img_start[pl], i1 = tb->img_start[pl + 1];
+                        if (yp.mode == 2 && i0 < i1) {
+                            const __amdgpu_buffer_rsrc_t rp = __builtin_amdgcn_make_buffer_rsrc(
+                                const_cast<float2*>(tb->one_plane) + col, 0, bytes, 0x00020000);
+                            int sp = 0;
+                            asm volatile("" : "+s"(sp));
+#pragma unroll
+                            for (int k2 = 0; k2 < N2; ++k2) {
+                                u[k2] = bload2(rp, voB, sp);
+                                sp += N1 * es;
+                                asm volatile("" : "+s"(sp));
+                            }
+                        }
+                        for (int i = i0; i < i1; ++i) {
+                            const __amdgpu_buffer_rsrc_t ri = __builtin_amdgcn_make_buffer_rsrc(
+                                C + (int64_t(tb->img_list[i]) * g.My * Hp + col), 0, bytes, 0x00020000);
+                            int sp = 0;
+                            asm volatile("" : "+s"(sp));
+#pragma unroll
+                            for (int k2 = 0; k2 < N2; ++k2) {
+                                bstore2(ri, voB, sp, u[k2]);
+                                sp += N1 * es;
+                                asm volatile("" : "+s"(sp));
+                            }
+                        }
+                    }
+                }
             } else {
                 int vok = voB;
 #pragma unroll
diff --git a/spim_registration_amd/csrc/fftconv_xt.inc b/spim_registration_amd/csrc/fftconv_xt.inc
--- a/spim_registration_amd/csrc/fftconv_xt.inc
+++ b/spim_registration_amd/csrc/fftconv_xt.inc
@@ -213,7 +213,7 @@
         asm volatile("" : "+v"(tq));
         const int c = tq / TR;
         const int hl = tq % TR;
-        const int pr = T < ntiles ? x_pair(a, T * NP + c) : -1;
+        const int pr = T < ntiles ? xt_pair(a, T * NP + c) : -1;
         const int r0 = pr >= 0 ? 2 * pr : nrows, r1 = r0 + 1;
         const bool v0 = r0 < nrows, v1 = r1 < nrows;
         int q0, q1;
@@ -247,7 +247,7 @@
      \
                           \
     const int sw = ((hl >> 2) ^ (hl >> 3)) & 1;                                      \
-    const int pr_ = x_pair(a, tile * NP + c);                                        \
+    const int pr_ = xt_pair(a, tile * NP + c);                                       \
     const int r0 = pr_ >= 0 ? 2 * pr_ : nrows, r1 = r0 + 1;                          \
     const bool v0 = r0 < nrows, v1 = r1 < nrows;                                     \
     const int sm0 = v0 ? a.row_mirror[r0] : -1, sm1 = v1 ? a.row_mirror[r1] : -1;   \
diff --git a/spim_registration_amd/csrc/session.cpp b/spim_registration_amd/csrc/session.cpp
--- a/spim_registration_amd/csrc/session.cpp
+++ b/spim_registration_amd/csrc/session.cpp
@@ -1036,18 +1036,19 @@
             exchange(buffer_a, st);
         }
     };
-    auto convolve = [&](SlabState& sl, float2* Cb, const float2* K, bool fwd_done) {
-        if (!fwd_done) { T0(2); engine_ypass(sl.sp, Cb, false, st); T1(); }
+    auto convolve = [&](SlabState& sl, float2* Cb, const float2* K, bool fwd_done, YExt ext) {
+        if (!fwd_done) { T0(2); engine_ypass(sl.sp, Cb, false, st, ext); T1(); }
         T0(3);
         if (sl.kcompact) engine_zpass_compact(sl.sp, Cb, K, st);
         else engine_zpass(sl.sp, Cb, K, st);
         T1();
-        T0(2); engine_ypass(sl.sp, Cb, true, st); T1();
+        T0(2); engine_ypass(sl.sp, Cb, true, st, ext); T1();
     };
     const int czx = halo_[2];
     auto convolve_all = [&](bool buffer_a, int v, bool pending) {
         auto buf = [&](SlabState& sl) { return buffer_a ? sl.C1.p : sl.C2.p; };
         auto ker = [&](SlabState& sl) { return buffer_a ? sl.e1spec[v].p : sl.e2spec[v].p; };
+        const YExt ext = buffer_a ? YExt::Mirror : YExt::One;
         bool split = pending;
         for (int s = s0; s < s1 && split; ++s)
             split = slabs_[s].sp.fy.n1 != 0 && int(slabs_[s].g.nz) > 2 * czx;
@@ -1055,7 +1056,7 @@
             for (int s = s0; s < s1; ++s) {
                 SlabState& sl = slabs_[s];
                 T0(2);
-                SD_CHECK(engine_ypass_planes(sl.sp, buf(sl), czx, int(sl.g.nz) - czx, st), SPIMDECON_ERR_STATE,
+                SD_CHECK(engine_ypass_planes(sl.sp, buf(sl), czx, int(sl.g.nz) - czx, st, ext), SPIMDECON_ERR_STATE,
                          "y pass of a plane range not available");
                 T1();
             }
@@ -1063,15 +1064,15 @@
             for (int s = s0; s < s1; ++s) {
                 SlabState& sl = slabs_[s];
                 T0(2);
-                SD_CHECK(engine_ypass_planes2(sl.sp, buf(sl), 0, czx, int(sl.g.nz) - czx, int(sl.g.Mz), st),
+                SD_CHECK(engine_ypass_planes2(sl.sp, buf(sl), 0, czx, int(sl.g.nz) - czx, int(sl.g.Mz), st, ext),
                          SPIMDECON_ERR_STATE, "y pass of a plane range not available");
                 T1();
             }
-            for (int s = s0; s < s1; ++s) convolve(slabs_[s], buf(slabs_[s]), ker(slabs_[s]), true);
+            for (int s = s0; s < s1; ++s) convolve(slabs_[s], buf(slabs_[s]), ker(slabs_[s]), true, ext);
             return;
         }
         if (pending) xend();
-        for (int s = s0; s < s1; ++s) convolve(slabs_[s], buf(slabs_[s]), ker(slabs_[s]), false);
+        for (int s = s0; s < s1; ++s) convolve(slabs_[s], buf(slabs_[s]), ker(slabs_[s]), false, ext);
     };
 
     for (int s = s0; s < s1; ++s) {
@@ -1214,6 +1215,13 @@
     return engine_zpass_mode(slabs_[slab].sp, slabs_[slab].kcompact);
 }
 
+int Session::padrows_mode(int slab) const {
+    SD_CHECK(slab >= 0 && slab < int(slabs_.size()), SPIMDECON_ERR_ARG, "bad slab");
+    SD_CHECK(spectra_ready_, SPIMDECON_ERR_STATE, "not initialised");
+    if (backend_ != 0) return -1;
+    return slabs_[slab].sp.padrows ? 1 : 0;
+}
+
 int Session::xpass_mode(int slab) const {
     SD_CHECK(slab >= 0 && slab < int(slabs_.size()), SPIMDECON_ERR_ARG, "bad slab");
     SD_CHECK(spectra_ready_, SPIMDECON_ERR_STATE, "not initialised");
diff --git a/spim_registration_amd/csrc/session.hpp b/spim_registration_amd/csrc/session.hpp
--- a/spim_registration_amd/csrc/session.hpp
+++ b/spim_registration_amd/csrc/session.hpp
@@ -92,6 +92,7 @@
     int kernel_planes(int slab) const;
     int zpass_mode(int slab) const;
     int xpass_mode(int slab) const;
+    int padrows_mode(int slab) const;
     hipStream_t stream() const { return groups_[0].stream; }
     int ndevices() const { return int(groups_.size()); }
     int nslabs() const { return int(slabs_.size()); }
diff --git a/spim_registration_amd/decon.py b/spim_registration_amd/decon.py
--- a/spim_registration_amd/decon.py
+++ b/spim_registration_amd/decon.py
@@ -247,6 +247,11 @@
         check(self.lib.mvd_xpass_mode(self.h, int(slab), C.byref(out)))
         return out.value
 
+    def padrows_mode(self, slab=0):
+        out = C.c_int()
+        check(self.lib.mvd_padrows_mode(self.h, int(slab), C.byref(out)))
+        return out.value
+
     def num_devices(self):
         out = C.c_int()
         check(self.lib.mvd_num_devices(self.h, C.byref(out)))
```

Measured after the change: 10080 Mvoxels/s per RL iteration, median of 6. 1.01x the previous value.
